# Quantco/tabmat

Measured on AMD Instinct MI355X. Metric: SplitMatrix.sandwich GFLOP/s + effective HBM GB/s, 10M×1k mixed, higher is better.
Workload: dtype f64; 1 GPU; SplitMatrix.sandwich: dense128 + csr512@5% + cats(256,96,32), 10000000 rows/GPU, p=1024, float64 (BASELINE configs[3]); rows_per_gpu=10000000, p=1024, launch=eager, collective=none

## Files before the change

include/tabmat_hip.h:

```cpp
#ifndef TABMAT_HIP_H
#define TABMAT_HIP_H

#include <stddef.h>
#include <stdint.h>

#ifdef __cplusplus
extern "C" {
#endif

#define TM_OK 0
#define TM_EINVAL (-1)
#define TM_ENOMEM (-2)
#define TM_EUNSUPPORTED (-3)

int tm_version(void);
const char *tm_last_error(void);
int tm_device_count(int *count);
int tm_set_device(int device);
int tm_device_info(char *name, int name_len, int *compute_units, int64_t *hbm_bytes);
int tm_malloc(void **ptr, size_t bytes);
int tm_free(void *ptr);
int tm_memcpy_h2d(void *dst, const void *h_src, size_t bytes, void *stream);
int tm_memcpy_d2h(void *h_dst, const void *src, size_t bytes, void *stream);
int tm_memset(void *dst, int value, size_t bytes, void *stream);
// ... 60 lines not shown

int tm_dense_sandwich_matvec_f32(const float *X, int64_t n, int64_t m, const float *u, const float *dm,
                                 const float *t_add, const float *center, const float *shift, float *g, float *w,
                                 void *stream);
int tm_dense_sandwich_matvec_f64(const double *X, int64_t n, int64_t m, const double *u, const double *dm,
                                 const double *t_add, const double *center, const double *shift, double *g,
                                 double *w, void *stream);

int tm_dense_sandwich_bf16x3_f32(const float *X, int64_t n, int64_t m, const float *d, float *out,
                                 void *stream);

int tm_dense_matvec_f32(const float *X, int64_t n, int64_t m, int order_f, const float *v,
                        const int32_t *rows, int64_t n_rows, const int32_t *cols,
                        int64_t n_cols, float *out, void *stream);
int tm_dense_matvec_f64(const double *X, int64_t n, int64_t m, int order_f, const double *v,
                        const int32_t *rows, int64_t n_rows, const int32_t *cols,
                        int64_t n_cols, double *out, void *stream);

int tm_dense_rmatvec_f32(const float *X, int64_t n, int64_t m, int order_f, const float *v,
                         const int32_t *rows, int64_t n_rows, const int32_t *cols,
                         int64_t n_cols, float *out, void *stream);
int tm_dense_rmatvec_f64(const double *X, int64_t n, int64_t m, int order_f, const double *v,
                         const int32_t *rows, int64_t n_rows, const int32_t *cols,
                         int64_t n_cols, double *out, void *stream);

int tm_dense_col_sq_dev_f32(const float *X, int64_t n, int64_t m, int order_f, const float *w,
                            const float *shift, float *out, void *stream);
int tm_dense_col_sq_dev_f64(const double *X, int64_t n, int64_t m, int order_f, const double *w,
                            const double *shift, double *out, void *stream);


int tm_sparse_sandwich_f32(const float *csr_data, const int32_t *csr_indices,
                           const int64_t *csr_indptr, int64_t n, int64_t m, const float *d,
                           const int32_t *rows, int64_t n_rows, const int32_t *cols,
                           int64_t n_cols, float *out, void *stream);
int tm_sparse_sandwich_f64(const double *csr_data, const int32_t *csr_indices,
                           const int64_t *csr_indptr, int64_t n, int64_t m, const double *d,
                           const int32_t *rows, int64_t n_rows, const int32_t *cols,
                           int64_t n_cols, double *out, void *stream);

int tm_sparse_chunk_cols(void);
int tm_sparse_sandwich_chunked_f32(const float *cm_data, const int32_t *cm_indices,
                                   const int32_t *cptr, int64_t n, int64_t m, int64_t nnz,
                                   const float *d, float *out, void *stream);
int tm_sparse_sandwich_chunked_f64(const double *cm_data, const int32_t *cm_indices,
                                   const int32_t *cptr, int64_t n, int64_t m, int64_t nnz,
                                   const double *d, double *out, void *stream);

int tm_sparse_sandwich_pairs_f32(const int32_t *cm_rec, const int32_t *cptr, int64_t n, int64_t m, int64_t nnz,
                                 const float *d, float *out, void *stream);
int tm_sparse_sandwich_pairs_f64(const int32_t *cm_rec, const int32_t *cptr, int64_t n, int64_t m, int64_t nnz,
                                 const double *d, double *out, void *stream);

int tm_sparse_sandwich_pairs_pk_f32(const int32_t *cm_rec_pk, const int32_t *cptr, int64_t n, int64_t m, int64_t nnz,
                                    const float *d, float *out, void *stream);
int tm_sparse_sandwich_pairs_pk_f64(const int32_t *cm_rec_pk, const int32_t *cptr, int64_t n, int64_t m, int64_t nnz,
                                    const double *d, double *out, void *stream);

int tm_sparse_sandwich_blocks_f32(const float *cm_data, const int32_t *cm_indices, const int32_t *cptr,
                                  int64_t n, int64_t m, int64_t nnz, const int32_t *blocks,
                                  const int32_t *wg_tab, int n_wg, int max_nb, const float *d, float *out,
                                  void *stream);
int tm_sparse_sandwich_blocks_f64(const double *cm_data, const int32_t *cm_indices, const int32_t *cptr,
                                  int64_t n, int64_t m, int64_t nnz, const int32_t *blocks,
                                  const int32_t *wg_tab, int n_wg, int max_nb, const double *d, double *out,
                                  void *stream);

int tm_sparse_sandwich_blocks_u8_f32(const float *cm_data, const uint8_t *cm_col8, const int32_t *cptr,
                                     int64_t n, int64_t m, int64_t nnz, const int32_t *blocks,
                                     const int32_t *wg_tab, int n_wg, int max_nb, const float *d, float *out,
                                     void *stream);
int tm_sparse_sandwich_blocks_u8_f64(const double *cm_data, const uint8_t *cm_col8, const int32_t *cptr,
                                     int64_t n, int64_t m, int64_t nnz, const int32_t *blocks,
                                     const int32_t *wg_tab, int n_wg, int max_nb, const double *d, double *out,
                                     void *stream);
int tm_sparse_sandwich_blocks_p12_f32(const float *cm_data, const uint8_t *cm_col8, const int32_t *cptr,
                                      int64_t n, int64_t m, int64_t nnz, const int32_t *blocks12,
                                      const int32_t *wg_tab, int n_wg, int max_nb, const float *d, float *out,
                                      void *stream);
int tm_sparse_sandwich_blocks_p12_f64(const double *cm_data, const uint8_t *cm_col8, const int32_t *cptr,
                                      int64_t n, int64_t m, int64_t nnz, const int32_t *blocks12,
                                      const int32_t *wg_tab, int n_wg, int max_nb, const double *d, double *out,
                                      void *stream);

int tm_csr_dense_sandwich_f32(const float *csr_data, const int32_t *csr_indices,
                              const int64_t *csr_indptr, int64_t n, int64_t m, const float *B,
                              int64_t r, int order_f, const float *d, const int32_t *rows,
                              int64_t n_rows, const int32_t *A_cols, int64_t nA,
                              const int32_t *B_cols, int64_t nB, float *out, void *stream);
int tm_csr_dense_sandwich_f64(const double *csr_data, const int32_t *csr_indices,
                              const int64_t *csr_indptr, int64_t n, int64_t m, const double *B,
                              int64_t r, int order_f, const double *d, const int32_t *rows,
                              int64_t n_rows, const int32_t *A_cols, int64_t nA,
                              const int32_t *B_cols, int64_t nB, double *out, void *stream);

int tm_slab_rows(void);
int tm_slab_group_cols(void);
int tm_csr_dense_sandwich_slab_f32(const float *vals, const uint32_t *koff, const uint16_t *cnt,
                                   const int64_t *gptr, int64_t n, int64_t m, const float *B,
                                   int64_t r, int order_f, const float *d, float *out, void *stream);
int tm_csr_dense_sandwich_slab_f64(const double *vals, const uint32_t *koff, const uint16_t *cnt,
                                   const int64_t *gptr, int64_t n, int64_t m, const double *B,
                                   int64_t r, int order_f, const double *d, double *out, void *stream);

int tm_csr_dense_sandwich_ell_f32(const float *vals, const uint32_t *koff, const int64_t *gptr,
                                  int64_t n, int64_t m, const float *B, int64_t r, const float *d,
                                  float *out, void *stream);
int tm_csr_dense_sandwich_ell_f64(const double *vals, const uint32_t *koff, const int64_t *gptr,
                                  int64_t n, int64_t m, const double *B, int64_t r, const double *d,
                                  double *out, void *stream);

int tm_ellw_rows(void);
int tm_ellw_group_cols(void);
int tm_csr_dense_sandwich_ellw_f32(const float *vals, const uint32_t *koff, const int64_t *gptr,
                                   int64_t n, int64_t m, const float *B, int64_t r, const float *d,
                                   float *out, void *stream);
int tm_csr_dense_sandwich_ellw_f64(const double *vals, const uint32_t *koff, const int64_t *gptr,
                                   int64_t n, int64_t m, const double *B, int64_t r, const double *d,
                                   double *out, void *stream);

int tm_lg_rows(void);
int tm_lg_group_cols(void);
int tm_lg_row_bytes(int elem_size);
int tm_csr_dense_sandwich_lg_f32(const float *vals, const uint32_t *koff, const int64_t *xptr,
                                 const float *xvals, const uint32_t *xkoff, int64_t n, int64_t m,
                                 const float *B, int64_t r, const float *d, int unconditional,
                                 float *out, void *stream);
int tm_csr_dense_sandwich_lg_f64(const double *vals, const uint32_t *koff, const int64_t *xptr,
                                 const double *xvals, const uint32_t *xkoff, int64_t n, int64_t m,
                                 const double *B, int64_t r, const double *d, int unconditional,
                                 double *out, void *stream);

int tm_csr_dense_sandwich_lg_xtd_f32(const float *vals, const uint32_t *koff, const int64_t *xptr,
                                     const float *xvals, const uint32_t *xkoff, int64_t n, int64_t m,
                                     const float *B, int64_t r, const float *d, int unconditional,
                                     float *out, float *colsum, void *stream);
int tm_csr_dense_sandwich_lg_xtd_f64(const double *vals, const uint32_t *koff, const int64_t *xptr,
                                     const double *xvals, const uint32_t *xkoff, int64_t n, int64_t m,
                                     const double *B, int64_t r, const double *d, int unconditional,
                                     double *out, double *colsum, void *stream);

int tm_csr_dense_sandwich_lgc_f32(const float *cvals, const uint32_t *cmap, const int64_t *crec,
                                  const uint32_t *xkoff, int64_t n, int64_t m, const float *B, int64_t r,
                                  const float *d, int unconditional, float *out, float *colsum, void *stream);
int tm_csr_dense_sandwich_lgc_f64(const double *cvals, const uint32_t *cmap, const int64_t *crec,
                                  const uint32_t *xkoff, int64_t n, int64_t m, const double *B, int64_t r,
                                  const double *d, int unconditional, double *out, double *colsum,
                                  void *stream);

int tm_ent_rows(void);
int tm_ent_group_cols(void);
int tm_ent_batch_slots(void);
int tm_csr_dense_sandwich_ent_f32(const float *vals, const uint16_t *meta, const uint32_t *bstart, int64_t n,
                                  int64_t m, const float *B, int64_t r, const float *d, float *out,
                                  float *colsum, void *stream);
int tm_csr_dense_sandwich_ent_f64(const double *vals, const uint16_t *meta, const uint32_t *bstart, int64_t n,
                                  int64_t m, const double *B, int64_t r, const double *d, double *out,
                                  double *colsum, void *stream);


int tm_index_narrow_i64(const int64_t *src, int64_t count, int64_t limit, int32_t *dst, int32_t *bad, void *stream);
int tm_index_widen_i32(const int32_t *src, int64_t count, int64_t *dst, void *stream);

int tm_csr_matvec_f32(const float *csr_data, const int32_t *csr_indices,
                      const int64_t *csr_indptr, int64_t n, int64_t m, const float *v,
                      const int32_t *rows, int64_t n_rows, const int32_t *cols, int64_t n_cols,
                      float *out, void *stream);
int tm_csr_matvec_f64(const double *csr_data, const int32_t *csr_indices,
                      const int64_t *csr_indptr, int64_t n, int64_t m, const double *v,
                      const int32_t *rows, int64_t n_rows, const int32_t *cols, int64_t n_cols,
                      double *out, void *stream);

int tm_csr_matvec_u16_f32(const float *csr_data, const uint16_t *csr_indices16, const int64_t *csr_indptr,
                          int64_t n, int64_t m, const float *v, float *out, void *stream);
int tm_csr_matvec_u16_f64(const double *csr_data, const uint16_t *csr_indices16, const int64_t *csr_indptr,
                          int64_t n, int64_t m, const double *v, double *out, void *stream);

int tm_csr_rmatvec_u16_f32(const float *csr_data, const uint16_t *csr_indices16, const int64_t *csr_indptr,
                           int64_t n, int64_t m, const float *v, float *out, void *stream);
int tm_csr_rmatvec_u16_f64(const double *csr_data, const uint16_t *csr_indices16, const int64_t *csr_indptr,
                           int64_t n, int64_t m, const double *v, double *out, void *stream);

int tm_csr_rmatvec_f32(const float *csr_data, const int32_t *csr_indices,
                       const int64_t *csr_indptr, int64_t n, int64_t m, const float *v,
                       const int32_t *rows, int64_t n_rows, const int32_t *cols, int64_t n_cols,
                       float *out, void *stream);
int tm_csr_rmatvec_f64(const double *csr_data, const int32_t *csr_indices,
                       const int64_t *csr_indptr, int64_t n, int64_t m, const double *v,
                       const int32_t *rows, int64_t n_rows, const int32_t *cols, int64_t n_cols,
                       double *out, void *stream);

int tm_csr_col_sq_f32(const float *csr_data, const int32_t *csr_indices, const int64_t *csr_indptr,
                      int64_t n, int64_t m, const float *w, float *out, void *stream);
int tm_csr_col_sq_f64(const double *csr_data, const int32_t *csr_indices,
                      const int64_t *csr_indptr, int64_t n, int64_t m, const double *w,
                      double *out, void *stream);

int tm_index_check_i64(void *stream, int32_t *h_bad);
int tm_sparse_sandwich_i64_f32(const float *csr_data, const int64_t *csr_indices, const int64_t *csr_indptr,
                               int64_t n, int64_t m, int64_t nnz, const float *d, const int32_t *rows,
                               int64_t n_rows, const int32_t *cols, int64_t n_cols, float *out, void *stream);
int tm_sparse_sandwich_i64_f64(const double *csr_data, const int64_t *csr_indices, const int64_t *csr_indptr,
                               int64_t n, int64_t m, int64_t nnz, const double *d, const int32_t *rows,
                               int64_t n_rows, const int32_t *cols, int64_t n_cols, double *out, void *stream);
int tm_csr_dense_sandwich_i64_f32(const float *csr_data, const int64_t *csr_indices, const int64_t *csr_indptr,
                                  int64_t n, int64_t m, int64_t nnz, const float *B, int64_t r, int order_f,
                                  const float *d, const int32_t *rows, int64_t n_rows, const int32_t *A_cols,
                                  int64_t nA, const int32_t *B_cols, int64_t nB, float *out, void *stream);
int tm_csr_dense_sandwich_i64_f64(const double *csr_data, const int64_t *csr_indices, const int64_t *csr_indptr,
                                  int64_t n, int64_t m, int64_t nnz, const double *B, int64_t r, int order_f,
                                  const double *d, const int32_t *rows, int64_t n_rows, const int32_t *A_cols,
                                  int64_t nA, const int32_t *B_cols, int64_t nB, double *out, void *stream);
int tm_csr_matvec_i64_f32(const float *csr_data, const int64_t *csr_indices, const int64_t *csr_indptr, int64_t n,
                          int64_t m, int64_t nnz, const float *v, const int32_t *rows, int64_t n_rows,
                          const int32_t *cols, int64_t n_cols, float *out, void *stream);
int tm_csr_matvec_i64_f64(const double *csr_data, const int64_t *csr_indices, const int64_t *csr_indptr, int64_t n,
                          int64_t m, int64_t nnz, const double *v, const int32_t *rows, int64_t n_rows,
                          const int32_t *cols, int64_t n_cols, double *out, void *stream);
int tm_csr_rmatvec_i64_f32(const float *csr_data, const int64_t *csr_indices, const int64_t *csr_indptr, int64_t n,
                           int64_t m, int64_t nnz, const float *v, const int32_t *rows, int64_t n_rows,
                           const int32_t *cols, int64_t n_cols, float *out, void *stream);
int tm_csr_rmatvec_i64_f64(const double *csr_data, const int64_t *csr_indices, const int64_t *csr_indptr, int64_t n,
                           int64_t m, int64_t nnz, const double *v, const int32_t *rows, int64_t n_rows,
                           const int32_t *cols, int64_t n_cols, double *out, void *stream);
int tm_csr_col_sq_i64_f32(const float *csr_data, const int64_t *csr_indices, const int64_t *csr_indptr, int64_t n,
                          int64_t m, int64_t nnz, const float *w, float *out, void *stream);
int tm_csr_col_sq_i64_f64(const double *csr_data, const int64_t *csr_indices, const int64_t *csr_indptr, int64_t n,
                          int64_t m, int64_t nnz, const double *w, double *out, void *stream);


int tm_cat_transpose_matvec_f32(const int32_t *codes, int64_t n, int64_t n_cols, int drop_first,
                                const float *v, const int32_t *rows, int64_t n_rows,
                                const int32_t *cols, int64_t n_cols_sel, float *out,
                                void *stream);
int tm_cat_transpose_matvec_f64(const int32_t *codes, int64_t n, int64_t n_cols, int drop_first,
                                const double *v, const int32_t *rows, int64_t n_rows,
                                const int32_t *cols, int64_t n_cols_sel, double *out,
                                void *stream);

int tm_cat_matvec_f32(const int32_t *codes, int64_t n, int64_t n_cols, int drop_first,
                      const float *v, const int32_t *cols, int64_t n_cols_sel, float *out,
                      void *stream);
int tm_cat_matvec_f64(const int32_t *codes, int64_t n, int64_t n_cols, int drop_first,
                      const double *v, const int32_t *cols, int64_t n_cols_sel, double *out,
                      void *stream);

int tm_cat_matvec_assign_f32(const int32_t *codes, int64_t n, int64_t n_cols, int drop_first,
                             const float *v, const int32_t *cols, int64_t n_cols_sel, float *out,
                             void *stream);
int tm_cat_matvec_assign_f64(const int32_t *codes, int64_t n, int64_t n_cols, int drop_first,
                             const double *v, const int32_t *cols, int64_t n_cols_sel, double *out,
                             void *stream);

int tm_cat_cat_sandwich_f32(const int32_t *i_codes, const int32_t *j_codes, int64_t n,
                            const float *d, const int32_t *rows, int64_t n_rows, int64_t i_ncol,
                            int64_t j_ncol, int i_drop_first, int j_drop_first, float *out,
                            void *stream);
int tm_cat_cat_sandwich_f64(const int32_t *i_codes, const int32_t *j_codes, int64_t n,
                            const double *d, const int32_t *rows, int64_t n_rows, int64_t i_ncol,
                            int64_t j_ncol, int i_drop_first, int j_drop_first, double *out,
                            void *stream);

int tm_cat_cat_sandwich_atomic_f32(const int32_t *i_codes, const int32_t *j_codes, int64_t n,
                                   const float *d, const int32_t *rows, int64_t n_rows, int64_t i_ncol,
                                   int64_t j_ncol, int i_drop_first, int j_drop_first, float *out,
                                   void *stream);
int tm_cat_cat_sandwich_atomic_f64(const int32_t *i_codes, const int32_t *j_codes, int64_t n,
                                   const double *d, const int32_t *rows, int64_t n_rows, int64_t i_ncol,
                                   int64_t j_ncol, int i_drop_first, int j_drop_first, double *out,
                                   void *stream);

int tm_cat_cat_sandwich_sorted_f32(const int32_t *ci_sorted, const int32_t *cj_sorted, const int32_t *perm,
                                   const int64_t *lptr, int64_t n_sorted, const float *d, int64_t i_ncol,
                                   int64_t j_ncol, float *out, void *stream);
int tm_cat_cat_sandwich_sorted_f64(const int32_t *ci_sorted, const int32_t *cj_sorted, const int32_t *perm,
                                   const int64_t *lptr, int64_t n_sorted, const double *d, int64_t i_ncol,
                                   int64_t j_ncol, double *out, void *stream);

int tm_cat_dense_sandwich_f32(const int32_t *codes, int64_t n, int64_t i_ncol, int drop_first,
                              const float *d, const int32_t *rows, int64_t n_rows, const float *M,
                              int64_t M_ncol, int order_f, const int32_t *j_cols, int64_t n_j,
                              float *out, void *stream);
int tm_cat_dense_sandwich_f64(const int32_t *codes, int64_t n, int64_t i_ncol, int drop_first,
                              const double *d, const int32_t *rows, int64_t n_rows,
                              const double *M, int64_t M_ncol, int order_f, const int32_t *j_cols,
                              int64_t n_j, double *out, void *stream);

int tm_cat_sparse_sandwich_f32(const int32_t *codes, int64_t n, int64_t i_ncol, int drop_first,
                               const float *csr_data, const int32_t *csr_indices,
                               const int64_t *csr_indptr, int64_t s_ncol, const float *d,
                               const int32_t *rows, int64_t n_rows, const int32_t *cols,
                               int64_t n_cols, float *out, void *stream);
int tm_cat_sparse_sandwich_f64(const int32_t *codes, int64_t n, int64_t i_ncol, int drop_first,
                               const double *csr_data, const int32_t *csr_indices,
                               const int64_t *csr_indptr, int64_t s_ncol, const double *d,
                               const int32_t *rows, int64_t n_rows, const int32_t *cols,
                               int64_t n_cols, double *out, void *stream);

int tm_multi_cat_dense_sandwich_f32(const void *const *h_codes, const int64_t *h_ncols,
                                    const int32_t *h_drop_first, int n_cats, int64_t n,
                                    const float *d, const float *M, int64_t M_ncol, int order_f,
                                    float *out, void *stream);
int tm_multi_cat_dense_sandwich_f64(const void *const *h_codes, const int64_t *h_ncols,
                                    const int32_t *h_drop_first, int n_cats, int64_t n,
                                    const double *d, const double *M, int64_t M_ncol, int order_f,
                                    double *out, void *stream);
int tm_multi_cat_dense_sandwich_rows_f32(const void *const *h_codes, const int64_t *h_ncols,
                                         const int32_t *h_drop_first, int n_cats, int64_t n,
                                         const float *d, const float *M, int64_t M_ncol,
                                         const int32_t *rows, int64_t n_rows, float *out,
                                         void *stream);
int tm_multi_cat_dense_sandwich_rows_f64(const void *const *h_codes, const int64_t *h_ncols,
                                         const int32_t *h_drop_first, int n_cats, int64_t n,
                                         const double *d, const double *M, int64_t M_ncol,
                                         const int32_t *rows, int64_t n_rows, double *out,
                                         void *stream);
int tm_multi_cat_sparse_sandwich_rows_f32(const void *const *h_codes, const int64_t *h_ncols,
                                          const int32_t *h_drop_first, int n_cats,
                                          const float *cm_data, const int32_t *cm_indices,
                                          const int32_t *row_ranges, const int32_t *rows,
                                          int64_t n_sel, int64_t m, const float *d_sel, float *out,
                                          void *stream);
int tm_multi_cat_sparse_sandwich_rows_f64(const void *const *h_codes, const int64_t *h_ncols,
                                          const int32_t *h_drop_first, int n_cats,
                                          const double *cm_data, const int32_t *cm_indices,
                                          const int32_t *row_ranges, const int32_t *rows,
                                          int64_t n_sel, int64_t m, const double *d_sel, double *out,
                                          void *stream);
int tm_multi_cat_sparse_sandwich_rows_u8_f32(const void *const *h_codes, const int64_t *h_ncols,
                                             const int32_t *h_drop_first, int n_cats,
                                             const float *cm_data, const uint8_t *cm_col8,
                                             const int32_t *row_ranges, const int32_t *rows,
                                             int64_t n_sel, int64_t m, const float *d_sel, float *out,
                                             void *stream);
int tm_multi_cat_sparse_sandwich_rows_u8_f64(const void *const *h_codes, const int64_t *h_ncols,
                                             const int32_t *h_drop_first, int n_cats,
                                             const double *cm_data, const uint8_t *cm_col8,
                                             const int32_t *row_ranges, const int32_t *rows,
                                             int64_t n_sel, int64_t m, const double *d_sel, double *out,
                                             void *stream);
int tm_multi_cat_sparse_sandwich_ent_f32(const void *const *h_codes, const int64_t *h_ncols,
                                         const int32_t *h_drop_first, int n_cats, int64_t n, const float *d,
                                         const float *vals, const uint16_t *meta, const uint32_t *bstart,
                                         int64_t n_slots, int64_t mk, float *out, void *stream);
int tm_multi_cat_sparse_sandwich_ent_f64(const void *const *h_codes, const int64_t *h_ncols,
                                         const int32_t *h_drop_first, int n_cats, int64_t n, const double *d,
                                         const double *vals, const uint16_t *meta, const uint32_t *bstart,
                                         int64_t n_slots, int64_t mk, double *out, void *stream);
int tm_multi_cat_pack_codes(const void *const *h_codes, const int64_t *h_ncols, const int32_t *h_drop_first, int n_cats,
                            int64_t n, uint32_t *packed, void *stream);
int tm_multi_cat_sparse_sandwich_entp_f32(const void *const *h_codes, const int64_t *h_ncols,
                                          const int32_t *h_drop_first, int n_cats, int64_t n, const float *d,
                                          const float *vals, const uint16_t *meta, const uint32_t *bstart,
                                          int64_t n_slots, int64_t mk, const uint32_t *packed, float *out, void *stream);
int tm_multi_cat_sparse_sandwich_entp_f64(const void *const *h_codes, const int64_t *h_ncols,
                                          const int32_t *h_drop_first, int n_cats, int64_t n, const double *d,
                                          const double *vals, const uint16_t *meta, const uint32_t *bstart,
                                          int64_t n_slots, int64_t mk, const uint32_t *packed, double *out, void *stream);

int tm_multi_cat_sparse_sandwich_slab_f32(const void *const *h_codes, const int64_t *h_ncols,
                                          const int32_t *h_drop_first, int n_cats, int64_t n,
                                          const float *d, const float *vals, const uint32_t *koff,
                                          const uint8_t *ecol, const int64_t *gptr, int64_t m,
                                          float *out, void *stream);
int tm_multi_cat_sparse_sandwich_slab_f64(const void *const *h_codes, const int64_t *h_ncols,
                                          const int32_t *h_drop_first, int n_cats, int64_t n,
                                          const double *d, const double *vals, const uint32_t *koff,
                                          const uint8_t *ecol, const int64_t *gptr, int64_t m,
                                          double *out, void *stream);

int tm_multi_cat_pairs_max_bins(void);
int tm_multi_cat_pairs_max_slots(void);
int tm_multi_cat_pairs_row_words(void);
int tm_multi_cat_pairs_f32(const int64_t *cat_tab, int64_t n, const float *d, const int32_t *rows,
                           int64_t n_rows, const int32_t *bundles, int n_bundles,
                           const int32_t *wg_map, int n_wg, int slots, int64_t bins,
                           const int64_t *desc, int64_t n_pairs, const int64_t *pos, double *tables,
                           double *out, int64_t p, void *stream);
int tm_multi_cat_pairs_f64(const int64_t *cat_tab, int64_t n, const double *d, const int32_t *rows,
                           int64_t n_rows, const int32_t *bundles, int n_bundles,
                           const int32_t *wg_map, int n_wg, int slots, int64_t bins,
                           const int64_t *desc, int64_t n_pairs, const int64_t *pos, double *tables,
                           double *out, int64_t p, void *stream);

int tm_multi_cat_matvec_f32(const int64_t *cat_tab, int n_cats, const int64_t *pos, const float *v,
                            int64_t n, float *out, void *stream);
int tm_multi_cat_matvec_f64(const int64_t *cat_tab, int n_cats, const int64_t *pos, const double *v,
                            int64_t n, double *out, void *stream);

int tm_csr_densify_cols_f32(const float *data, const int32_t *indices, const int64_t *indptr, int64_t n,
                            const int32_t *colmap, float *T, int64_t ld, void *stream);
int tm_csr_densify_cols_f64(const double *data, const int32_t *indices, const int64_t *indptr, int64_t n,
                            const int32_t *colmap, double *T, int64_t ld, void *stream);
int tm_csc_densify_cols_f32(const int32_t *rows, const float *vals, const int64_t *seg, const int32_t *tcol,
                            int64_t n_sel, int64_t max_len, float *T, int64_t ld, void *stream);
int tm_csc_densify_cols_f64(const int32_t *rows, const double *vals, const int64_t *seg, const int32_t *tcol,
                            int64_t n_sel, int64_t max_len, double *T, int64_t ld, void *stream);
int tm_dense_gather_cols_f32(const float *X, int64_t n, int64_t m, int order_f, const int32_t *cols,
                             int64_t n_sel, float *T, int64_t ld, int64_t t0, void *stream);
int tm_dense_gather_cols_f64(const double *X, int64_t n, int64_t m, int order_f, const int32_t *cols,
                             int64_t n_sel, double *T, int64_t ld, int64_t t0, void *stream);

int tm_scatter_block_f32(const float *src, int64_t nr, int64_t nc, const int64_t *ri,
                         const int64_t *ci, double *out, int64_t p, int mirror, int diag,
                         void *stream);
int tm_scatter_block_f64(const double *src, int64_t nr, int64_t nc, const int64_t *ri,
                         const int64_t *ci, double *out, int64_t p, int mirror, int diag,
                         void *stream);

int tm_sparse_sandwich_chunked_rows_f32(const float *cm_data, const int32_t *cm_indices,
                                        const int32_t *row_ranges, int64_t n_sel, int64_t m,
                                        int64_t nnz, const float *d_sel, float *out, void *stream);
int tm_sparse_sandwich_chunked_rows_f64(const double *cm_data, const int32_t *cm_indices,
                                        const int32_t *row_ranges, int64_t n_sel, int64_t m,
                                        int64_t nnz, const double *d_sel, double *out, void *stream);

int tm_sparse_sandwich_chunked_u8_f32(const float *cm_data, const uint8_t *cm_col8, const int32_t *cptr, int64_t n,
                                      int64_t m, int64_t nnz, const float *d, float *out, void *stream);
int tm_sparse_sandwich_chunked_u8_f64(const double *cm_data, const uint8_t *cm_col8, const int32_t *cptr, int64_t n,
                                      int64_t m, int64_t nnz, const double *d, double *out, void *stream);
int tm_sparse_sandwich_chunked_rows_u8_f32(const float *cm_data, const uint8_t *cm_col8, const int32_t *row_ranges,
                                           int64_t n_sel, int64_t m, int64_t nnz, const float *d_sel, float *out,
                                           void *stream);
int tm_sparse_sandwich_chunked_rows_u8_f64(const double *cm_data, const uint8_t *cm_col8, const int32_t *row_ranges,
                                           int64_t n_sel, int64_t m, int64_t nnz, const double *d_sel, double *out,
                                           void *stream);
int tm_sparse_sandwich_direct_f32(const float *csr_data, const int32_t *csr_indices,
                                  const int64_t *csr_indptr, int64_t n, int64_t m, const float *d,
                                  float *out, void *stream);
int tm_sparse_sandwich_direct_f64(const double *csr_data, const int32_t *csr_indices,
                                  const int64_t *csr_indptr, int64_t n, int64_t m, const double *d,
                                  double *out, void *stream);
int tm_csr_dense_sandwich_rows_f32(const float *cm_data, const int32_t *cm_indices,
                                   const int32_t *row_ranges, int64_t n_sel, const int32_t *rows,
                                   const float *d_sel, int64_t n, int64_t m, const float *B, int64_t r,
                                   int order_f, float *out, void *stream);
int tm_csr_dense_sandwich_rows_f64(const double *cm_data, const int32_t *cm_indices,
                                   const int32_t *row_ranges, int64_t n_sel, const int32_t *rows,
                                   const double *d_sel, int64_t n, int64_t m, const double *B, int64_t r,
                                   int order_f, double *out, void *stream);
int tm_csr_dense_sandwich_rows_u8_f32(const float *cm_data, const uint8_t *cm_col8,
// ... 82 lines not shown
```

tabmat_amd/csrc/cat.hip:

```cpp
#include <algorithm>

#include "common.hpp"
#include "reduce.hpp"

namespace tmh {

__global__ void fill_i32_kernel(int32_t *p, int64_t n, int32_t v) {
    int64_t i = (int64_t)blockIdx.x * blockDim.x + threadIdx.x;
    if (i < n) p[i] = v;
}

__global__ void scatter_iota_i32_kernel(int32_t *map, const int32_t *cols, int64_t n_cols) {
    int64_t i = (int64_t)blockIdx.x * blockDim.x + threadIdx.x;
    if (i < n_cols) map[cols[i]] = (int32_t)i;
}

int build_col_map(int32_t *map, int64_t m, const int32_t *cols, int64_t n_cols, hipStream_t st) {
    if (m > 0) {
        hipLaunchKernelGGL(fill_i32_kernel, dim3((unsigned)ceil_div(m, 256)), dim3(256), 0, st, map,
                           m, -1);
        TM_LAUNCH_CHECK();
    }
    if (n_cols > 0) {
        hipLaunchKernelGGL(scatter_iota_i32_kernel, dim3((unsigned)ceil_div(n_cols, 256)),
// ... 710 lines not shown
                sc[c * MCW_RS + lr] = R.dk != F(0) ? R.code[c] : -1;
        }
        __builtin_amdgcn_wave_barrier();
#pragma unroll
        for (int i = 0; i < NI; ++i) {
            const int row = 4 * i + q;
            const F dk = sd[row];
            int off[NC];
#pragma unroll
            for (int c = 0; c < NC; ++c) off[c] = sc[c * MCW_RS + row];
            vec_t x = R.x[i];
#pragma unroll
            for (int v = 0; v < VEC; ++v) x[v] *= dk;
#pragma unroll
            for (int c = 0; c < NC; ++c) {
                if (jok && off[c] >= 0) {
                    lds_acc_t *dst = reinterpret_cast<lds_acc_t *>(smem_raw + off[c]) + jl;
#pragma unroll
                    for (int v = 0; v < VEC; ++v) atomic_add(dst + 16 * v, (lds_acc_t)x[v]);
                }
            }
        }
    };
    Regs ra, rb;
    int64_t k0 = t0 + (int64_t)wave * MCW_RS;
    if (k0 < t1) load(k0, ra);
    for (; k0 < t1; k0 += 2 * step) {
        const bool more = k0 + step < t1;
        if (more) load(k0 + step, rb);
        process(ra);
        if (more) {
            if (k0 + 2 * step < t1) load(k0 + 2 * step, ra);
            process(rb);
        }
    }
    __syncthreads();
    if (threadIdx.x == 0) wg_log_end(wglog, t_begin, WG_CAT_DENSE);
    F *dst = ws + ((int64_t)blockIdx.y * gridDim.x + blockIdx.x) * stride;
    for (int b = threadIdx.x; b < nel; b += blockDim.x) {
        const int c = b % TJ;
        dst[b] = (F)tile[(b / TJ) * TJ + (c / VEC) + 16 * (c % VEC)];
    }
}

template <typename F, int TJ>
__global__ __launch_bounds__(1024) void multi_cat_dense_f_kernel(
    CatSet cs, const F *__restrict__ d, const F *__restrict__ M, int64_t n, int64_t m,
    int64_t rows_per_block, F *__restrict__ ws, int64_t stride) {
    extern __shared__ __attribute__((aligned(16))) unsigned char smem_raw[];
    lds_acc_t *tile = reinterpret_cast<lds_acc_t *>(smem_raw);
    const int nel = cs.total * TJ;
    for (int b = threadIdx.x; b < nel; b += blockDim.x) tile[b] = 0.0;
    __syncthreads();
    const int64_t j0 = (int64_t)blockIdx.y * TJ;
    const int64_t t0 = (int64_t)blockIdx.x * rows_per_block;
    const int64_t t1 = min(t0 + rows_per_block, n);
    for (int64_t k = t0 + threadIdx.x; k < t1; k += blockDim.x) {
        const F dk = d[k];
        int col[MAX_CATS];
#pragma unroll
        for (int c = 0; c < MAX_CATS; ++c)
            col[c] = c < cs.n_cats ? cs.codes[c][k] - cs.drop[c] : -1;
        for (int jl = 0; jl < TJ && j0 + jl < m; ++jl) {
            const F x = dk * M[(j0 + jl) * n + k];
#pragma unroll
            for (int c = 0; c < MAX_CATS; ++c)
                if (col[c] >= 0) atomic_add(&tile[(cs.off[c] + col[c]) * TJ + jl], (lds_acc_t)x);
        }
    }
    __syncthreads();
    F *dst = ws + ((int64_t)blockIdx.y * gridDim.x + blockIdx.x) * stride;
    for (int b = threadIdx.x; b < nel; b += blockDim.x) dst[b] = (F)tile[b];
}

template <typename F>
__global__ void multi_cat_untile_kernel(const F *__restrict__ tmp, int64_t total, int64_t m,
                                        int TJ, F *__restrict__ out) {
    const int64_t e = (int64_t)blockIdx.x * blockDim.x + threadIdx.x;
    if (e >= total * m) return;
    const int64_t a = e / m, j = e % m;
    out[e] = tmp[((j / TJ) * total + a) * TJ + (j % TJ)];
}

template <typename F, bool STAGE>
__global__ __launch_bounds__(1024) void multi_cat_sparse_kernel(
    CatSet cs, const F *__restrict__ d, const F *__restrict__ vals,
    const unsigned *__restrict__ koff, const unsigned char *__restrict__ ecol,
    const int64_t *__restrict__ gptr, int n_groups, int64_t n_slabs, int64_t slabs_per_block,
    int slab_rows, int group_cols, int64_t n, F *__restrict__ ws, int64_t stride) {
    extern __shared__ __attribute__((aligned(16))) unsigned char smem_raw[];
    lds_acc_t *tile = reinterpret_cast<lds_acc_t *>(smem_raw);
    const int tstr = group_cols + 1;
    const int nel = cs.total * tstr;
    for (int b = threadIdx.x; b < nel; b += blockDim.x) tile[b] = 0.0;
    const int g = blockIdx.y;
    const int lane = threadIdx.x & 63;
    const int wave = threadIdx.x >> 6, nwave = blockDim.x >> 6;
    F *sd = reinterpret_cast<F *>(smem_raw + (((size_t)nel * sizeof(lds_acc_t) + 15) / 16) * 16) +
            (size_t)wave * slab_rows;
    int32_t *sc = reinterpret_cast<int32_t *>(
                      reinterpret_cast<F *>(smem_raw + (((size_t)nel * sizeof(lds_acc_t) + 15) / 16) * 16) +
                      (size_t)nwave * slab_rows) +
                  (size_t)wave * cs.n_cats * slab_rows;
    __syncthreads();
    const int64_t s0 = (int64_t)blockIdx.x * slabs_per_block;
    const int64_t s1 = min(s0 + slabs_per_block, n_slabs);
    const unsigned rowb = 64u * (unsigned)sizeof(F);
    int64_t nb = 0, ne = 0;
    if (s0 + wave < s1) {
        nb = gptr[(s0 + wave) * n_groups + g];
        ne = gptr[(s0 + wave) * n_groups + g + 1];
    }
    for (int64_t s = s0 + wave; s < s1; s += nwave) {
        const int64_t base = nb, end = ne;
        if (s + nwave < s1) {
            nb = gptr[(s + nwave) * n_groups + g];
            ne = gptr[(s + nwave) * n_groups + g + 1];
        }
        if (STAGE) {
            __builtin_amdgcn_wave_barrier();
            for (int r = lane; r < slab_rows; r += 64) {
                const int64_t k = min(s * slab_rows + r, n - 1);
                sd[r] = d[k];
                for (int c = 0; c < cs.n_cats; ++c) sc[c * slab_rows + r] = cs.codes[c][k] - cs.drop[c];
            }
            __builtin_amdgcn_wave_barrier();
        }
        for (int64_t e0 = base + lane; e0 < end; e0 += 128) {
            const int64_t e1 = e0 + 64;
            const bool ok1 = e1 < end;
            const unsigned ko0 = koff[e0];
            const unsigned ko1 = ok1 ? koff[e1] : 0u;
            const F v0 = vals[e0];
            const F v1 = ok1 ? vals[e1] : F(0);
            const int ec0 = ecol[e0];
            const int ec1 = ok1 ? ecol[e1] : 0;
            const int r0 = (int)(ko0 / rowb), r1 = (int)(ko1 / rowb);
            const int64_t k0 = s * slab_rows + r0;
            const int64_t k1 = s * slab_rows + r1;
            const F d0 = STAGE ? sd[r0] : d[k0];
            const F d1 = ok1 ? (STAGE ? sd[r1] : d[k1]) : F(0);
            const F x0 = d0 != F(0) ? d0 * v0 : F(0);
            const F x1 = d1 != F(0) ? d1 * v1 : F(0);
#pragma unroll 1
            for (int c = 0; c < cs.n_cats; ++c) {
                const int c0 = STAGE ? sc[c * slab_rows + r0] : cs.codes[c][k0] - cs.drop[c];
                const int c1 = ok1 ? (STAGE ? sc[c * slab_rows + r1] : cs.codes[c][k1] - cs.drop[c])
                                   : -1;
                if (c0 >= 0) atomic_add(&tile[(cs.off[c] + c0) * tstr + ec0], (lds_acc_t)x0);
                if (c1 >= 0) atomic_add(&tile[(cs.off[c] + c1) * tstr + ec1], (lds_acc_t)x1);
            }
        }
    }
    __syncthreads();
    F *dst = ws + ((int64_t)blockIdx.y * gridDim.x + blockIdx.x) * stride;
    for (int b = threadIdx.x; b < cs.total * group_cols; b += blockDim.x)
        dst[b] = (F)tile[(b / group_cols) * tstr + (b % group_cols)];
}

template <typename F, int NC>
__global__ __launch_bounds__(1024) void multi_cat_sparse_pf_kernel(
    CatSet cs, const F *__restrict__ d, const F *__restrict__ vals,
    const unsigned *__restrict__ koff, const unsigned char *__restrict__ ecol,
    const int64_t *__restrict__ gptr, int n_groups, int64_t n_slabs, int64_t slabs_per_block,
    int group_cols, int64_t n, F *__restrict__ ws, int64_t stride, WgLogBuf *__restrict__ wglog) {
    const unsigned long long t_begin = wg_log_begin(wglog);
// ... 322 lines not shown
            }
        }
    }
    __syncthreads();
    F *dst = ws + ((int64_t)blockIdx.y * gridDim.x + blockIdx.x) * stride;
    for (int b = threadIdx.x; b < cs.total * GC; b += blockDim.x)
        dst[b] = (F)tile[(b / GC) * TSTR + (b % GC)];
}

template <typename F, typename IX>
__global__ __launch_bounds__(1024) void multi_cat_sparse_rows_kernel(
    CatSet cs, const F *__restrict__ cm_data, const IX *__restrict__ cm_ind,
    const int32_t *__restrict__ ranges, const int32_t *__restrict__ rows, const F *__restrict__ d_sel,
    int64_t n_sel, int64_t rows_per_block, F *__restrict__ ws, int64_t stride) {
    constexpr int GC = 32;
    extern __shared__ __attribute__((aligned(16))) unsigned char smem_raw[];
    lds_acc_t *tile = reinterpret_cast<lds_acc_t *>(smem_raw);
    constexpr int tstr = GC + 1;
    const int nel = cs.total * tstr;
    for (int b = threadIdx.x; b < nel; b += blockDim.x) tile[b] = 0.0;
    __syncthreads();
    const int g = blockIdx.y;
    const int ch = g >> 2;
    const int lane = threadIdx.x & 63, wave = threadIdx.x >> 6, nwave = blockDim.x >> 6;
    const int lr = lane >> 3, lt = lane & 7;
    const int64_t t0 = (int64_t)blockIdx.x * rows_per_block;
    const int64_t t1 = min(t0 + rows_per_block, n_sel);
    const int32_t *rg = ranges + (int64_t)ch * n_sel * 2;
    for (int64_t k0 = t0 + wave * 8; k0 < t1; k0 += (int64_t)nwave * 8) {
        const int64_t k = k0 + lr;
        if (k >= t1) continue;
        const F dk = d_sel[k];
        if (dk == F(0)) continue;
        const int e0 = rg[2 * k], e1 = rg[2 * k + 1];
        if (e0 >= e1) continue;
        const int64_t row = rows[k];
        int off[MAX_CATS];
#pragma unroll
        for (int c = 0; c < MAX_CATS; ++c) {
            off[c] = -1;
            if (c < cs.n_cats) {
                const int col = cs.codes[c][row] - cs.drop[c];
                off[c] = col >= 0 ? (cs.off[c] + col) * tstr : -1;
            }
        }
        for (int e = e0 + lt; e < e1; e += 8) {
            const int col = (int)cm_ind[e] - (sizeof(IX) == 1 ? (g & 3) : g) * GC;
            if (col < 0 || col >= GC) continue;
            const lds_acc_t x = (lds_acc_t)(dk * cm_data[e]);
#pragma unroll
            for (int c = 0; c < MAX_CATS; ++c)
                if (off[c] >= 0) atomic_add(&tile[off[c] + col], x);
        }
    }
    __syncthreads();
    F *dst = ws + ((int64_t)blockIdx.y * gridDim.x + blockIdx.x) * stride;
    for (int b = threadIdx.x; b < cs.total * GC; b += blockDim.x)
        dst[b] = (F)tile[(b / GC) * tstr + (b % GC)];
}

static int make_catset(const void *const *h_codes, const int64_t *h_ncols, const int32_t *h_drop,
                       int n_cats, CatSet *cs) {
    if (n_cats < 1 || n_cats > MAX_CATS) {
        set_error("multi-cat call supports 1..%d categoricals, got %d", MAX_CATS, n_cats);
        return TM_EINVAL;
    }
    int off = 0;
    for (int c = 0; c < MAX_CATS; ++c) {
        cs->codes[c] = c < n_cats ? reinterpret_cast<const int32_t *>(h_codes[c]) : nullptr;
        cs->ncol[c] = c < n_cats ? (int)h_ncols[c] : 0;
        cs->drop[c] = c < n_cats ? h_drop[c] : 0;
        cs->off[c] = off;
        off += cs->ncol[c];
    }
    cs->n_cats = n_cats;
    cs->total = off;
    return TM_OK;
}

template <typename F>
static int run_multi_cat_dense(const void *const *h_codes, const int64_t *h_ncols,
                               const int32_t *h_drop, int n_cats, int64_t n, const F *d, const F *M,
                               int64_t m, int order_f, F *out, hipStream_t st,
                               const int32_t *rows = nullptr, int64_t n_rows = 0) {
    CatSet cs;
    int rc = make_catset(h_codes, h_ncols, h_drop, n_cats, &cs);
    if (rc) return rc;
    const int64_t total = (int64_t)cs.total * m;
    if (total == 0) return TM_OK;
    if (rows != nullptr) n = n_rows;
    if (n == 0) {
        TM_HIP(hipMemsetAsync(out, 0, sizeof(F) * (size_t)total, st));
        return TM_OK;
    }
    {
        constexpr int VEC = MCW_VEC;
        constexpr int TJW = 16 * VEC;
        const size_t tile_b = ((sizeof(lds_acc_t) * (size_t)cs.total * TJW + 15) / 16) * 16;
        const size_t lds_w = tile_b + (size_t)16 * MCW_RS * (sizeof(F) + (size_t)n_cats * sizeof(int));
        if (!order_f && n_cats <= 8 && m >= VEC && m % VEC == 0 &&
            (reinterpret_cast<uintptr_t>(M) & 15) == 0 && lds_w <= 150 * 1024 &&
            (int64_t)cs.total * TJW * (int64_t)sizeof(lds_acc_t) < (1ll << 30)) {
            const int64_t n_parts = ceil_div(m, TJW);
            const int64_t stride = (int64_t)cs.total * TJW;
            int64_t nblk = std::max<int64_t>(1, tune("catdense_rounds", 1) * NUM_CU / n_parts);
            nblk = std::min<int64_t>(nblk, std::max<int64_t>(1, ceil_div(n, 4096)));
            const int64_t rpb = ceil_div(ceil_div(n, nblk), MCW_RS) * MCW_RS;
            nblk = ceil_div(n, rpb);
            const size_t tmp_bytes = ((sizeof(F) * (size_t)(n_parts * stride) + 255) / 256) * 256;
            void *wsv = nullptr;
            rc = get_workspace(tmp_bytes + sizeof(F) * (size_t)(n_parts * nblk * stride) + 256, &wsv, st);
            if (rc) return rc;
            F *tmp = reinterpret_cast<F *>(wsv);
            F *ws = reinterpret_cast<F *>(reinterpret_cast<char *>(wsv) + tmp_bytes);
            auto gow = [&](auto kern) -> int {
                TM_HIP(hipFuncSetAttribute(reinterpret_cast<const void *>(kern),
                                           hipFuncAttributeMaxDynamicSharedMemorySize, (int)lds_w));
                prof_begin(st);
                const int nw_dflt = (sizeof(F) == 8 && tile_b > 64 * 1024) ? 8 : 16;
                const int nw = (int)std::min<int64_t>(16, std::max<int64_t>(4, tune("catdense_waves", nw_dflt)));
                hipLaunchKernelGGL(kern, dim3((unsigned)nblk, (unsigned)n_parts), dim3(nw * 64), lds_w, st,
                                   cs, d, M, n, m, rpb, ws, stride, rows, wg_log_ptr());
                prof_end(st);
                TM_LAUNCH_CHECK();
                return TM_OK;
            };
            if (n_cats == 1) rc = gow(&multi_cat_dense_wide_kernel<F, 1>);
            else if (n_cats == 2) rc = gow(&multi_cat_dense_wide_kernel<F, 2>);
            else if (n_cats == 3) rc = gow(&multi_cat_dense_wide_kernel<F, 3>);
            else if (n_cats == 4) rc = gow(&multi_cat_dense_wide_kernel<F, 4>);
            else if (n_cats == 5) rc = gow(&multi_cat_dense_wide_kernel<F, 5>);
            else if (n_cats == 6) rc = gow(&multi_cat_dense_wide_kernel<F, 6>);
            else if (n_cats == 7) rc = gow(&multi_cat_dense_wide_kernel<F, 7>);
            else rc = gow(&multi_cat_dense_wide_kernel<F, 8>);
            if (rc) return rc;
            rc = launch_reduce_partials<F>(ws, stride, (int)nblk, (int)n_parts, tmp, n_parts * stride,
                                           false, st);
            if (rc) return rc;
            hipLaunchKernelGGL((multi_cat_untile_kernel<F>), dim3((unsigned)ceil_div(total, 256)),
                               dim3(256), 0, st, tmp, (int64_t)cs.total, m, TJW, out);
            TM_LAUNCH_CHECK();
            return TM_OK;
        }
    }
    if (rows != nullptr) {
        set_error("multi_cat_dense: the row-list form needs the wide-load path");
        return TM_EUNSUPPORTED;
    }
    int TJ = 64;
    while (TJ > 1 && sizeof(lds_acc_t) * (size_t)cs.total * TJ > HIST_LDS_MAX) TJ >>= 1;
    while (TJ > 1 && TJ / 2 >= m) TJ >>= 1;
    if (sizeof(lds_acc_t) * (size_t)cs.total * TJ > HIST_LDS_MAX) {
        set_error("multi_cat_dense: %d stacked categories exceed the LDS tile", cs.total);
        return TM_EUNSUPPORTED;
    }
    const int64_t n_parts = ceil_div(m, TJ);
    const int64_t stride = (int64_t)cs.total * TJ;
    const size_t lds = sizeof(lds_acc_t) * (size_t)stride;
    int64_t nblk = std::max<int64_t>(1, NUM_CU / n_parts);
    nblk = std::min<int64_t>(nblk, std::max<int64_t>(1, ceil_div(n, 4096)));
    const int64_t rpb = ceil_div(n, nblk);
    nblk = ceil_div(n, rpb);
    const size_t tmp_bytes = ((sizeof(F) * (size_t)(n_parts * stride) + 255) / 256) * 256;
    void *wsv = nullptr;
    rc = get_workspace(tmp_bytes + sizeof(F) * (size_t)(n_parts * nblk * stride) + 256, &wsv, st);
    if (rc) return rc;
    F *tmp = reinterpret_cast<F *>(wsv);
    F *ws = reinterpret_cast<F *>(reinterpret_cast<char *>(wsv) + tmp_bytes);
    auto go = [&](auto kern) -> int {
        if (lds > 48 * 1024)
            TM_HIP(hipFuncSetAttribute(reinterpret_cast<const void *>(kern),
                                       hipFuncAttributeMaxDynamicSharedMemorySize, (int)lds));
        prof_begin(st);
        hipLaunchKernelGGL(kern, dim3((unsigned)nblk, (unsigned)n_parts), dim3(1024), lds, st, cs, d,
                           M, n, m, rpb, ws, stride);
        prof_end(st);
        TM_LAUNCH_CHECK();
        return TM_OK;
    };
#define TM_MCD_CASE(V)                                                                       \
    case V:                                                                                  \
        if (order_f) rc = go(&multi_cat_dense_f_kernel<F, V>);                               \
        else if (n_cats == 1) rc = go(&multi_cat_dense_c_kernel<F, V, 1>);                   \
        else if (n_cats == 2) rc = go(&multi_cat_dense_c_kernel<F, V, 2>);                   \
        else if (n_cats == 3) rc = go(&multi_cat_dense_c_kernel<F, V, 3>);                   \
        else if (n_cats == 4) rc = go(&multi_cat_dense_c_kernel<F, V, 4>);                   \
        else rc = go(&multi_cat_dense_c_kernel<F, V, 0>);                                    \
        break;
    switch (TJ) {
        TM_MCD_CASE(64)
        TM_MCD_CASE(32)
        TM_MCD_CASE(16)
        TM_MCD_CASE(8)
        TM_MCD_CASE(4)
        TM_MCD_CASE(2)
        TM_MCD_CASE(1)
        default:
            rc = TM_EINVAL;
    }
#undef TM_MCD_CASE
    if (rc) return rc;
    rc = launch_reduce_partials<F>(ws, stride, (int)nblk, (int)n_parts, tmp, n_parts * stride, false,
                                   st);
    if (rc) return rc;
    hipLaunchKernelGGL((multi_cat_untile_kernel<F>), dim3((unsigned)ceil_div(total, 256)),
                       dim3(256), 0, st, tmp, (int64_t)cs.total, m, TJ, out);
    TM_LAUNCH_CHECK();
    return TM_OK;
}

template <typename F, typename IX>
static int run_multi_cat_sparse_rows(const void *const *h_codes, const int64_t *h_ncols,
                                     const int32_t *h_drop, int n_cats, const F *cm_data,
                                     const IX *cm_ind, const int32_t *ranges, const int32_t *rows,
                                     int64_t n_sel, int64_t m, const F *d_sel, F *out, hipStream_t st);

template <typename F>
static int run_multi_cat_sparse(const void *const *h_codes, const int64_t *h_ncols,
                                const int32_t *h_drop, int n_cats, int64_t n, const F *d,
                                const F *vals, const unsigned *koff, const unsigned char *ecol,
                                const int64_t *gptr, int64_t m, int slab_rows, int group_cols,
                                F *out, hipStream_t st) {
    CatSet cs;
    int rc = make_catset(h_codes, h_ncols, h_drop, n_cats, &cs);
    if (rc) return rc;
    const int64_t total = (int64_t)cs.total * m;
// ... 4 lines not shown
    }
    const int64_t stride = (int64_t)cs.total * group_cols;
    const size_t tile_bytes = ((sizeof(lds_acc_t) * (size_t)cs.total * (group_cols + 1) + 15) / 16) * 16;
    if (tile_bytes > HIST_LDS_MAX) {
        set_error("multi_cat_sparse: %d stacked categories exceed the LDS tile", cs.total);
        return TM_EUNSUPPORTED;
    }
    const int nw = (int)std::min<int64_t>(16, std::max<int64_t>(4, tune("catsparse_waves", 16)));
    const size_t stage_bytes = (size_t)nw * slab_rows * (sizeof(F) + sizeof(int32_t) * (size_t)n_cats);
    const bool stage = tile_bytes + stage_bytes <= 150 * 1024;
    const size_t lds = tile_bytes + (stage ? stage_bytes : 0);
    const int n_groups = (int)ceil_div(m, group_cols);
    const int64_t n_slabs = ceil_div(n, slab_rows);
    int64_t nblk = std::max<int64_t>(1, tune("catsparse_rounds", 1) * NUM_CU / n_groups);
    nblk = std::min<int64_t>(nblk, n_slabs);
    const int64_t spb = ceil_div(n_slabs, nblk);
    nblk = ceil_div(n_slabs, spb);
    const size_t tmp_bytes = ((sizeof(F) * (size_t)(n_groups * stride) + 255) / 256) * 256;
    void *wsv = nullptr;
    rc = get_workspace(tmp_bytes + sizeof(F) * (size_t)((int64_t)n_groups * nblk * stride) + 256,
                       &wsv, st);
    if (rc) return rc;
    F *tmp = reinterpret_cast<F *>(wsv);
    F *ws = reinterpret_cast<F *>(reinterpret_cast<char *>(wsv) + tmp_bytes);
    if (stage && n_cats <= 8 && slab_rows == 128) {
        auto kpf = n_cats == 1   ? &multi_cat_sparse_pf_kernel<F, 1>
                   : n_cats == 2 ? &multi_cat_sparse_pf_kernel<F, 2>
                   : n_cats == 3 ? &multi_cat_sparse_pf_kernel<F, 3>
                   : n_cats == 4 ? &multi_cat_sparse_pf_kernel<F, 4>
                   : n_cats == 5 ? &multi_cat_sparse_pf_kernel<F, 5>
                   : n_cats == 6 ? &multi_cat_sparse_pf_kernel<F, 6>
                   : n_cats == 7 ? &multi_cat_sparse_pf_kernel<F, 7>
                                 : &multi_cat_sparse_pf_kernel<F, 8>;
        if (lds > 48 * 1024)
            TM_HIP(hipFuncSetAttribute(reinterpret_cast<const void *>(kpf),
                                       hipFuncAttributeMaxDynamicSharedMemorySize, (int)lds));
        prof_begin(st);
        hipLaunchKernelGGL(kpf, dim3((unsigned)nblk, (unsigned)n_groups), dim3(nw * 64), lds, st, cs, d,
                           vals, koff, ecol, gptr, n_groups, n_slabs, spb, group_cols, n, ws, stride,
                           wg_log_ptr());
        prof_end(st);
        TM_LAUNCH_CHECK();
    } else {
        auto kern = stage ? &multi_cat_sparse_kernel<F, true> : &multi_cat_sparse_kernel<F, false>;
        if (lds > 48 * 1024)
            TM_HIP(hipFuncSetAttribute(reinterpret_cast<const void *>(kern),
                                       hipFuncAttributeMaxDynamicSharedMemorySize, (int)lds));
        prof_begin(st);
        hipLaunchKernelGGL(kern, dim3((unsigned)nblk, (unsigned)n_groups), dim3(nw * 64), lds, st, cs,
                           d, vals, koff, ecol, gptr, n_groups, n_slabs, spb, slab_rows, group_cols,
                           n, ws, stride);
        prof_end(st);
        TM_LAUNCH_CHECK();
    }
    rc = launch_reduce_partials<F>(ws, stride, (int)nblk, n_groups, tmp,
                                   (int64_t)n_groups * stride, false, st);
    if (rc) return rc;
    hipLaunchKernelGGL((multi_cat_untile_kernel<F>), dim3((unsigned)ceil_div(total, 256)),
                       dim3(256), 0, st, tmp, (int64_t)cs.total, m, group_cols, out);
    TM_LAUNCH_CHECK();
    return TM_OK;
}

__global__ __launch_bounds__(256) void multi_cat_pack_codes_kernel(CatSet cs, int64_t n, unsigned *__restrict__ out) {
    for (int64_t r = (int64_t)blockIdx.x * blockDim.x + threadIdx.x; r < n; r += (int64_t)gridDim.x * blockDim.x) {
        unsigned pk = 0u;
#pragma unroll
        for (int c = 0; c < 3; ++c) {
            unsigned f = 1023u;
            if (c < cs.n_cats) {
                const int col = cs.codes[c][r] - cs.drop[c];
                if (col >= 0 && col < cs.ncol[c]) f = (unsigned)(cs.off[c] + col);
            }
            pk |= f << (10 * c);
        }
        out[r] = pk;
    }
}

template <typename F>
static int run_multi_cat_sparse_ent(const void *const *h_codes, const int64_t *h_ncols, const int32_t *h_drop,
                                    int n_cats, int64_t n, const F *d, const F *vals, const unsigned short *meta,
                                    const unsigned *bstart, int64_t mk, F *out, hipStream_t st,
                                    const unsigned *packed = nullptr, int64_t n_slots = 0) {
    CatSet cs;
    int rc = make_catset(h_codes, h_ncols, h_drop, n_cats, &cs);
    if (rc) return rc;
    const int64_t total = (int64_t)cs.total * mk;
    if (total == 0) return TM_OK;
    if (n == 0) {
        TM_HIP(hipMemsetAsync(out, 0, sizeof(F) * (size_t)total, st));
        return TM_OK;
    }
    TM_REQUIRE(mk % 16 == 0 && n_cats >= 1 && n_cats <= 8, "kernel columns in groups of 16, 1 .. 8 categoricals");
    TM_REQUIRE(n < (1ll << 28), "at most 2^28 - 1 rows per block");
    constexpr int GC = 32;
    const int64_t stride = (int64_t)cs.total * GC;
    const size_t lds = ((sizeof(lds_acc_t) * (size_t)cs.total * (GC + 1) + 15) / 16) * 16;
    if (lds > HIST_LDS_MAX) {
        set_error("multi_cat_sparse_ent: %d stacked categories exceed the LDS tile", cs.total);
        return TM_EUNSUPPORTED;
    }
    const int nw = (int)std::min<int64_t>(16, std::max<int64_t>(4, tune("catsparse_waves", 16)));
    const int n_groups = (int)(mk / 16);
    const int n_pairs = (n_groups + 1) / 2;
    const int64_t n_slabs = ceil_div(n, 64);
    int64_t nblk = std::max<int64_t>(1, tune("catsparse_rounds", 1) * NUM_CU / n_pairs);
    nblk = std::min<int64_t>(nblk, n_slabs);
    const int64_t spb = ceil_div(n_slabs, nblk);
    nblk = ceil_div(n_slabs, spb);
    const size_t tmp_bytes = ((sizeof(F) * (size_t)(n_pairs * stride) + 255) / 256) * 256;
    void *wsv = nullptr;
    rc = get_workspace(tmp_bytes + sizeof(F) * (size_t)((int64_t)n_pairs * nblk * stride) + 256, &wsv, st);
    if (rc) return rc;
    F *tmp = reinterpret_cast<F *>(wsv);
    F *ws = reinterpret_cast<F *>(reinterpret_cast<char *>(wsv) + tmp_bytes);
    auto kern = n_cats == 1   ? &multi_cat_sparse_ent_kernel<F, 1>
                : n_cats == 2 ? &multi_cat_sparse_ent_kernel<F, 2>
                : n_cats == 3 ? &multi_cat_sparse_ent_kernel<F, 3>
                : n_cats == 4 ? &multi_cat_sparse_ent_kernel<F, 4>
                : n_cats == 5 ? &multi_cat_sparse_ent_kernel<F, 5>
                : n_cats == 6 ? &multi_cat_sparse_ent_kernel<F, 6>
                : n_cats == 7 ? &multi_cat_sparse_ent_kernel<F, 7>
                              : &multi_cat_sparse_ent_kernel<F, 8>;
    TM_REQUIRE(packed == nullptr || (n_cats <= 3 && cs.total < 1023), "packed codes: at most 3 categoricals, 1022 levels");
    const int ncw = packed != nullptr ? 1 : n_cats;
    const size_t lds_staged = lds + (size_t)nw * 64 * (sizeof(F) + 4 * (size_t)ncw);
    const double fill = (double)n_slots / ((double)std::max(n_groups, 1) * (double)n_slabs);
    if (tune("catsparse_staged", 1) != 0 && lds_staged <= 156 * 1024 &&
        fill >= (double)tune("catsparse_staged_fill", 44)) {
        using KS = void (*)(CatSet, const F *, const F *, const unsigned short *, const unsigned *, int, int64_t, int64_t,
                            int64_t, F *, int64_t, const unsigned *, int);
        KS ks = nullptr;
        if (packed != nullptr) {
            ks = n_cats == 1 ? &multi_cat_sparse_ent_staged_kernel<F, 1, true>
                 : n_cats == 2 ? &multi_cat_sparse_ent_staged_kernel<F, 2, true>
                               : &multi_cat_sparse_ent_staged_kernel<F, 3, true>;
        } else {
            ks = n_cats == 1   ? &multi_cat_sparse_ent_staged_kernel<F, 1, false>
                 : n_cats == 2 ? &multi_cat_sparse_ent_staged_kernel<F, 2, false>
                 : n_cats == 3 ? &multi_cat_sparse_ent_staged_kernel<F, 3, false>
                 : n_cats == 4 ? &multi_cat_sparse_ent_staged_kernel<F, 4, false>
                 : n_cats == 5 ? &multi_cat_sparse_ent_staged_kernel<F, 5, false>
                 : n_cats == 6 ? &multi_cat_sparse_ent_staged_kernel<F, 6, false>
                 : n_cats == 7 ? &multi_cat_sparse_ent_staged_kernel<F, 7, false>
                               : &multi_cat_sparse_ent_staged_kernel<F, 8, false>;
        }
        if (lds_staged > 48 * 1024)
            TM_HIP(hipFuncSetAttribute(reinterpret_cast<const void *>(ks),
                                       hipFuncAttributeMaxDynamicSharedMemorySize, (int)lds_staged));
        prof_begin(st);
        hipLaunchKernelGGL(ks, dim3((unsigned)nblk, (unsigned)n_pairs), dim3(nw * 64), lds_staged, st, cs, d, vals,
                           meta, bstart, n_groups, n, n_slabs, spb, ws, stride, packed, (int)lds);
        prof_end(st);
        TM_LAUNCH_CHECK();
    } else {
        if (lds > 48 * 1024)
            TM_HIP(hipFuncSetAttribute(reinterpret_cast<const void *>(kern),
                                       hipFuncAttributeMaxDynamicSharedMemorySize, (int)lds));
        prof_begin(st);
        hipLaunchKernelGGL(kern, dim3((unsigned)nblk, (unsigned)n_pairs), dim3(nw * 64), lds, st, cs, d, vals, meta,
                           bstart, n_groups, n, n_slabs, spb, ws, stride, packed);
        prof_end(st);
        TM_LAUNCH_CHECK();
    }
    rc = launch_reduce_partials<F>(ws, stride, (int)nblk, n_pairs, tmp, (int64_t)n_pairs * stride, false, st);
    if (rc) return rc;
    hipLaunchKernelGGL((multi_cat_untile_kernel<F>), dim3((unsigned)ceil_div(total, 256)), dim3(256), 0, st, tmp,
                       (int64_t)cs.total, mk, GC, out);
    TM_LAUNCH_CHECK();
    return TM_OK;
}

}

using namespace tmh;

#define TM_CHECK_COMMON(nn) \
    TM_REQUIRE((nn) >= 0, "negative size")

extern "C" {

int tm_cat_transpose_matvec_f32(const int32_t *codes, int64_t n, int64_t n_cols, int drop_first,
                                const float *v, const int32_t *rows, int64_t n_rows,
                                const int32_t *cols, int64_t n_cols_sel, float *out, void *stream) {
    TM_CHECK_COMMON(n);
    return run_cat_tmv<float>(codes, n, n_cols, drop_first, v, rows, n_rows, cols, n_cols_sel, out,
                              as_stream(stream));
}
int tm_cat_transpose_matvec_f64(const int32_t *codes, int64_t n, int64_t n_cols, int drop_first,
                                const double *v, const int32_t *rows, int64_t n_rows,
                                const int32_t *cols, int64_t n_cols_sel, double *out,
                                void *stream) {
    TM_CHECK_COMMON(n);
    return run_cat_tmv<double>(codes, n, n_cols, drop_first, v, rows, n_rows, cols, n_cols_sel,
                               out, as_stream(stream));
}

int tm_cat_matvec_f32(const int32_t *codes, int64_t n, int64_t n_cols, int drop_first,
                      const float *v, const int32_t *cols, int64_t n_cols_sel, float *out,
                      void *stream) {
    TM_CHECK_COMMON(n);
    return run_cat_matvec<float>(codes, n, n_cols, drop_first, v, cols, n_cols_sel, out,
                                 as_stream(stream));
}
int tm_cat_matvec_f64(const int32_t *codes, int64_t n, int64_t n_cols, int drop_first,
                      const double *v, const int32_t *cols, int64_t n_cols_sel, double *out,
                      void *stream) {
    TM_CHECK_COMMON(n);
    return run_cat_matvec<double>(codes, n, n_cols, drop_first, v, cols, n_cols_sel, out,
                                  as_stream(stream));
}

int tm_cat_matvec_assign_f32(const int32_t *codes, int64_t n, int64_t n_cols, int drop_first,
                             const float *v, const int32_t *cols, int64_t n_cols_sel, float *out,
                             void *stream) {
    TM_CHECK_COMMON(n);
    return run_cat_matvec<float>(codes, n, n_cols, drop_first, v, cols, n_cols_sel, out,
                                 as_stream(stream), true);
}
int tm_cat_matvec_assign_f64(const int32_t *codes, int64_t n, int64_t n_cols, int drop_first,
                             const double *v, const int32_t *cols, int64_t n_cols_sel, double *out,
                             void *stream) {
    TM_CHECK_COMMON(n);
    return run_cat_matvec<double>(codes, n, n_cols, drop_first, v, cols, n_cols_sel, out,
                                  as_stream(stream), true);
}

int tm_cat_cat_sandwich_f32(const int32_t *i_codes, const int32_t *j_codes, int64_t n,
                            const float *d, const int32_t *rows, int64_t n_rows, int64_t i_ncol,
                            int64_t j_ncol, int i_drop_first, int j_drop_first, float *out,
                            void *stream) {
    TM_CHECK_COMMON(n);
    return run_hist<float, true>(i_codes, j_codes, d, rows, rows ? n_rows : n, i_drop_first,
                                 j_drop_first, i_ncol, j_ncol, nullptr, out, false,
                                 as_stream(stream));
}
int tm_cat_cat_sandwich_f64(const int32_t *i_codes, const int32_t *j_codes, int64_t n,
                            const double *d, const int32_t *rows, int64_t n_rows, int64_t i_ncol,
                            int64_t j_ncol, int i_drop_first, int j_drop_first, double *out,
                            void *stream) {
    TM_CHECK_COMMON(n);
    return run_hist<double, true>(i_codes, j_codes, d, rows, rows ? n_rows : n, i_drop_first,
                                  j_drop_first, i_ncol, j_ncol, nullptr, out, false,
                                  as_stream(stream));
}

int tm_cat_cat_sandwich_atomic_f32(const int32_t *i_codes, const int32_t *j_codes, int64_t n,
// ... 55 lines not shown
    TM_CHECK_COMMON(n);
    return run_cat_sparse<float>(codes, n, i_ncol, drop_first, csr_data, csr_indices, csr_indptr,
                                 s_ncol, d, rows, n_rows, cols, n_cols, out, as_stream(stream));
}
int tm_cat_sparse_sandwich_f64(const int32_t *codes, int64_t n, int64_t i_ncol, int drop_first,
                               const double *csr_data, const int32_t *csr_indices,
                               const int64_t *csr_indptr, int64_t s_ncol, const double *d,
                               const int32_t *rows, int64_t n_rows, const int32_t *cols,
                               int64_t n_cols, double *out, void *stream) {
    TM_CHECK_COMMON(n);
    return run_cat_sparse<double>(codes, n, i_ncol, drop_first, csr_data, csr_indices, csr_indptr,
                                  s_ncol, d, rows, n_rows, cols, n_cols, out, as_stream(stream));
}

int tm_multi_cat_dense_sandwich_f32(const void *const *h_codes, const int64_t *h_ncols,
                                    const int32_t *h_drop_first, int n_cats, int64_t n,
                                    const float *d, const float *M, int64_t M_ncol, int order_f,
                                    float *out, void *stream) {
    return run_multi_cat_dense<float>(h_codes, h_ncols, h_drop_first, n_cats, n, d, M, M_ncol,
                                      order_f, out, as_stream(stream));
}
int tm_multi_cat_dense_sandwich_f64(const void *const *h_codes, const int64_t *h_ncols,
                                    const int32_t *h_drop_first, int n_cats, int64_t n,
                                    const double *d, const double *M, int64_t M_ncol, int order_f,
                                    double *out, void *stream) {
    return run_multi_cat_dense<double>(h_codes, h_ncols, h_drop_first, n_cats, n, d, M, M_ncol,
                                       order_f, out, as_stream(stream));
}
int tm_multi_cat_dense_sandwich_rows_f32(const void *const *h_codes, const int64_t *h_ncols,
                                         const int32_t *h_drop_first, int n_cats, int64_t n,
                                         const float *d, const float *M, int64_t M_ncol,
                                         const int32_t *rows, int64_t n_rows, float *out,
                                         void *stream) {
    return run_multi_cat_dense<float>(h_codes, h_ncols, h_drop_first, n_cats, n, d, M, M_ncol, 0, out,
                                      as_stream(stream), rows, n_rows);
}
int tm_multi_cat_dense_sandwich_rows_f64(const void *const *h_codes, const int64_t *h_ncols,
                                         const int32_t *h_drop_first, int n_cats, int64_t n,
                                         const double *d, const double *M, int64_t M_ncol,
                                         const int32_t *rows, int64_t n_rows, double *out,
                                         void *stream) {
    return run_multi_cat_dense<double>(h_codes, h_ncols, h_drop_first, n_cats, n, d, M, M_ncol, 0, out,
                                       as_stream(stream), rows, n_rows);
}
int tm_multi_cat_sparse_sandwich_ent_f32(const void *const *h_codes, const int64_t *h_ncols,
                                         const int32_t *h_drop_first, int n_cats, int64_t n, const float *d,
                                         const float *vals, const uint16_t *meta, const uint32_t *bstart,
                                         int64_t n_slots, int64_t mk, float *out, void *stream) {
    return run_multi_cat_sparse_ent<float>(h_codes, h_ncols, h_drop_first, n_cats, n, d, vals, meta, bstart, mk,
                                           out, as_stream(stream), nullptr, n_slots);
}
int tm_multi_cat_sparse_sandwich_ent_f64(const void *const *h_codes, const int64_t *h_ncols,
                                         const int32_t *h_drop_first, int n_cats, int64_t n, const double *d,
                                         const double *vals, const uint16_t *meta, const uint32_t *bstart,
                                         int64_t n_slots, int64_t mk, double *out, void *stream) {
    return run_multi_cat_sparse_ent<double>(h_codes, h_ncols, h_drop_first, n_cats, n, d, vals, meta, bstart, mk,
                                            out, as_stream(stream), nullptr, n_slots);
}
int tm_multi_cat_pack_codes(const void *const *h_codes, const int64_t *h_ncols, const int32_t *h_drop_first, int n_cats,
                            int64_t n, uint32_t *packed, void *stream) {
    CatSet cs;
    int rc = make_catset(h_codes, h_ncols, h_drop_first, n_cats, &cs);
    if (rc) return rc;
    TM_REQUIRE(n_cats <= 3 && cs.total < 1023, "packed codes: at most 3 categoricals, 1022 stacked levels");
    if (n == 0) return TM_OK;
    hipLaunchKernelGGL(multi_cat_pack_codes_kernel, dim3((unsigned)std::min<int64_t>(4 * NUM_CU, ceil_div(n, 256))),
                       dim3(256), 0, as_stream(stream), cs, n, packed);
    TM_LAUNCH_CHECK();
    return TM_OK;
}
int tm_multi_cat_sparse_sandwich_entp_f32(const void *const *h_codes, const int64_t *h_ncols,
                                          const int32_t *h_drop_first, int n_cats, int64_t n, const float *d,
                                          const float *vals, const uint16_t *meta, const uint32_t *bstart,
                                          int64_t n_slots, int64_t mk, const uint32_t *packed, float *out, void *stream) {
    return run_multi_cat_sparse_ent<float>(h_codes, h_ncols, h_drop_first, n_cats, n, d, vals, meta, bstart, mk, out,
                                           as_stream(stream), packed, n_slots);
}
int tm_multi_cat_sparse_sandwich_entp_f64(const void *const *h_codes, const int64_t *h_ncols,
                                          const int32_t *h_drop_first, int n_cats, int64_t n, const double *d,
                                          const double *vals, const uint16_t *meta, const uint32_t *bstart,
                                          int64_t n_slots, int64_t mk, const uint32_t *packed, double *out, void *stream) {
    return run_multi_cat_sparse_ent<double>(h_codes, h_ncols, h_drop_first, n_cats, n, d, vals, meta, bstart, mk,
                                            out, as_stream(stream), packed, n_slots);
}
int tm_multi_cat_sparse_sandwich_slab_f32(const void *const *h_codes, const int64_t *h_ncols,
                                          const int32_t *h_drop_first, int n_cats, int64_t n,
                                          const float *d, const float *vals, const uint32_t *koff,
                                          const uint8_t *ecol, const int64_t *gptr, int64_t m,
                                          float *out, void *stream) {
    return run_multi_cat_sparse<float>(h_codes, h_ncols, h_drop_first, n_cats, n, d, vals, koff,
                                       ecol, gptr, m, tm_slab_rows(), tm_slab_group_cols(), out,
                                       as_stream(stream));
}
int tm_multi_cat_sparse_sandwich_slab_f64(const void *const *h_codes, const int64_t *h_ncols,
                                          const int32_t *h_drop_first, int n_cats, int64_t n,
                                          const double *d, const double *vals, const uint32_t *koff,
                                          const uint8_t *ecol, const int64_t *gptr, int64_t m,
                                          double *out, void *stream) {
    return run_multi_cat_sparse<double>(h_codes, h_ncols, h_drop_first, n_cats, n, d, vals, koff,
                                        ecol, gptr, m, tm_slab_rows(), tm_slab_group_cols(), out,
                                        as_stream(stream));
}

}

namespace tmh {
template <typename F, typename IX>
static int run_multi_cat_sparse_rows(const void *const *h_codes, const int64_t *h_ncols,
                                     const int32_t *h_drop, int n_cats, const F *cm_data,
                                     const IX *cm_ind, const int32_t *ranges, const int32_t *rows,
                                     int64_t n_sel, int64_t m, const F *d_sel, F *out, hipStream_t st) {
    CatSet cs;
    int rc = make_catset(h_codes, h_ncols, h_drop, n_cats, &cs);
    if (rc) return rc;
    const int64_t total = (int64_t)cs.total * m;
    if (total == 0) return TM_OK;
    if (n_sel == 0) {
        TM_HIP(hipMemsetAsync(out, 0, sizeof(F) * (size_t)total, st));
        return TM_OK;
    }
    constexpr int GC = 32;
    const size_t lds = ((sizeof(lds_acc_t) * (size_t)cs.total * (GC + 1) + 15) / 16) * 16;
    if (lds > HIST_LDS_MAX) {
        set_error("multi_cat_sparse_rows: %d stacked categories exceed the LDS tile", cs.total);
        return TM_EUNSUPPORTED;
    }
    const int n_groups = (int)ceil_div(m, GC);
    const int64_t stride = (int64_t)cs.total * GC;
    int64_t nblk = std::max<int64_t>(1, tune("catsparse_rounds", 1) * NUM_CU / n_groups);
    nblk = std::min<int64_t>(nblk, std::max<int64_t>(1, ceil_div(n_sel, 2048)));
    const int64_t rpb = ceil_div(n_sel, nblk);
    nblk = ceil_div(n_sel, rpb);
    const size_t tmp_bytes = ((sizeof(F) * (size_t)(n_groups * stride) + 255) / 256) * 256;
    void *wsv = nullptr;
    rc = get_workspace(tmp_bytes + sizeof(F) * (size_t)((int64_t)n_groups * nblk * stride) + 256, &wsv, st);
    if (rc) return rc;
    F *tmp = reinterpret_cast<F *>(wsv);
    F *ws = reinterpret_cast<F *>(reinterpret_cast<char *>(wsv) + tmp_bytes);
    auto kern = &multi_cat_sparse_rows_kernel<F, IX>;
    if (lds > 48 * 1024)
        TM_HIP(hipFuncSetAttribute(reinterpret_cast<const void *>(kern),
                                   hipFuncAttributeMaxDynamicSharedMemorySize, (int)lds));
    prof_begin(st);
    hipLaunchKernelGGL(kern, dim3((unsigned)nblk, (unsigned)n_groups), dim3(1024), lds, st, cs, cm_data,
                       cm_ind, ranges, rows, d_sel, n_sel, rpb, ws, stride);
    prof_end(st);
    TM_LAUNCH_CHECK();
    rc = launch_reduce_partials<F>(ws, stride, (int)nblk, n_groups, tmp, (int64_t)n_groups * stride, false, st);
    if (rc) return rc;
    hipLaunchKernelGGL((multi_cat_untile_kernel<F>), dim3((unsigned)ceil_div(total, 256)), dim3(256), 0,
                       st, tmp, (int64_t)cs.total, m, GC, out);
    TM_LAUNCH_CHECK();
    return TM_OK;
}
}

extern "C" {
int tm_multi_cat_sparse_sandwich_rows_f32(const void *const *h_codes, const int64_t *h_ncols,
                                          const int32_t *h_drop_first, int n_cats,
                                          const float *cm_data, const int32_t *cm_indices,
                                          const int32_t *row_ranges, const int32_t *rows,
                                          int64_t n_sel, int64_t m, const float *d_sel, float *out,
                                          void *stream) {
    return tmh::run_multi_cat_sparse_rows<float, int32_t>(h_codes, h_ncols, h_drop_first, n_cats, cm_data,
                                                 cm_indices, row_ranges, rows, n_sel, m, d_sel, out,
                                                 tmh::as_stream(stream));
// ... 33 lines not shown
```

tabmat_amd/csrc/reduce.hpp:

```cpp
#pragma once
#include "common.hpp"

namespace tmh {

template <typename F, bool ACCUMULATE, int NW>
__global__ __launch_bounds__(NW * 64) void reduce_partials_kernel(const F *__restrict__ ws,
                                                                  int64_t stride, int nb,
                                                                  F *__restrict__ out,
                                                                  int64_t out_elems) {
    __shared__ double red[NW][64];
    const int lane = threadIdx.x & 63;
    const int wave = threadIdx.x >> 6;
    const int64_t e = (int64_t)blockIdx.x * 64 + lane;
    const int part = blockIdx.y;
    double acc = 0.0;
    if (e < stride) {
        const F *p = ws + ((int64_t)part * nb) * stride + e;
        for (int b = wave; b < nb; b += NW) acc += (double)p[(int64_t)b * stride];
    }
    red[wave][lane] = acc;
    __syncthreads();
    if (wave == 0 && e < stride) {
        const int64_t o = (int64_t)part * stride + e;
        if (o < out_elems) {
            double s = 0.0;
#pragma unroll
            for (int w = 0; w < NW; w += 4)
                s += (red[w][lane] + red[w + 1][lane]) + (red[w + 2][lane] + red[w + 3][lane]);
            if (ACCUMULATE)
                out[o] += (F)s;
            else
                out[o] = (F)s;
        }
    }
}

template <typename F>
inline int launch_reduce_partials(const F *ws, int64_t stride, int nb, int n_parts, F *out,
                                  int64_t out_elems, bool accumulate, hipStream_t st) {
    dim3 grid((unsigned)ceil_div(stride, 64), (unsigned)n_parts);
    const bool small = (int64_t)grid.x * grid.y < 1024 && nb > 16;
    if (small) {
        if (accumulate)
            hipLaunchKernelGGL((reduce_partials_kernel<F, true, 16>), grid, dim3(1024), 0, st, ws,
                               stride, nb, out, out_elems);
        else
            hipLaunchKernelGGL((reduce_partials_kernel<F, false, 16>), grid, dim3(1024), 0, st, ws,
                               stride, nb, out, out_elems);
    } else if (accumulate) {
        hipLaunchKernelGGL((reduce_partials_kernel<F, true, 4>), grid, dim3(256), 0, st, ws, stride,
                           nb, out, out_elems);
    } else {
        hipLaunchKernelGGL((reduce_partials_kernel<F, false, 4>), grid, dim3(256), 0, st, ws, stride,
                           nb, out, out_elems);
    }
    TM_LAUNCH_CHECK();
    return TM_OK;
}

__global__ void fill_i32_kernel(int32_t *p, int64_t n, int32_t v);
__global__ void scatter_iota_i32_kernel(int32_t *map, const int32_t *cols, int64_t n_cols);

int build_col_map(int32_t *map, int64_t m, const int32_t *cols, int64_t n_cols, hipStream_t st);

}
```

tabmat_amd/csrc/sparse_blocks.hip:

```cpp
#include <algorithm>

#include "common.hpp"
#include "reduce.hpp"

namespace tmh {

constexpr int KB_WAVES = 16;
constexpr int KB_TS = 128;

template <typename F>
__global__ void blocks_assemble_kernel(const F *__restrict__ tiles, int n_out, F *__restrict__ out) {
    const int j = blockIdx.x * blockDim.x + threadIdx.x;
    const int i = blockIdx.y;
    if (i >= n_out || j >= n_out) return;
    const int hi = max(i, j), lo = min(i, j);
    const int I = hi / KB_TS, J = lo / KB_TS;
    const int part = I * (I + 1) / 2 + J;
    out[(int64_t)i * n_out + j] = tiles[(int64_t)part * KB_TS * KB_TS + (hi % KB_TS) * KB_TS + (lo % KB_TS)];
}

constexpr int KB_FLAG_REP_A = 1 << 16;
constexpr int KB_FLAG_REP_B = 1 << 17;

template <typename F, bool U8, bool D12 = false>
__global__ __launch_bounds__(KB_WAVES * 64) void sparse_sandwich_blocks_kernel(
    const F *__restrict__ data, const int32_t *__restrict__ ind, const int32_t *__restrict__ cptr,
    int64_t n, int64_t nnz1, const int32_t *__restrict__ blocks, const int4 *__restrict__ wg_tab,
    const F *__restrict__ d, int max_nb, F *__restrict__ ws, WgLogBuf *__restrict__ wglog) {
    constexpr int TS = KB_TS;
    const unsigned long long t_begin = wg_log_begin(wglog);
    extern __shared__ __attribute__((aligned(16))) unsigned char smem_raw[];
    lds_acc_t *tile = reinterpret_cast<lds_acc_t *>(smem_raw);
    const int4 w = wg_tab[2 * blockIdx.x], x = wg_tab[2 * blockIdx.x + 1];
    const int part = __builtin_amdgcn_readfirstlane(w.x), slot = __builtin_amdgcn_readfirstlane(w.y);
    const int b0 = __builtin_amdgcn_readfirstlane(w.z), b1 = __builtin_amdgcn_readfirstlane(w.w);
    const int bfull = __builtin_amdgcn_readfirstlane(x.x);
    int wfull = __builtin_amdgcn_readfirstlane(x.y);
    {
        const int nwv = (int)(blockDim.x >> 6);
        if (nwv != KB_WAVES) {
            wfull = (wfull * nwv + KB_WAVES / 2) / KB_WAVES;
            if (bfull > b0) wfull = max(wfull, 1);
            if (b1 > bfull) wfull = min(wfull, nwv - 1);
            if (bfull == b0) wfull = 0;
            if (b1 == bfull) wfull = nwv;
        }
    }
    int I = (int)((sqrtf(8.0f * (float)part + 1.0f) - 1.0f) * 0.5f);
    while ((I + 1) * (I + 2) / 2 <= part) ++I;
    while (I * (I + 1) / 2 > part) --I;
    const int J = part - I * (I + 1) / 2;
    const int i0 = I * TS, j0 = J * TS;
    for (int b = threadIdx.x; b < TS * TS; b += blockDim.x) tile[b] = 0.0;
    __syncthreads();

    const int lane = threadIdx.x & 63;
    const int wave = __builtin_amdgcn_readfirstlane(threadIdx.x >> 6);
    const int lr = lane >> 3, lt = lane & 7;
    if (b1 > b0) {
        const int row_first = __builtin_amdgcn_readfirstlane(x.z), row_last = __builtin_amdgcn_readfirstlane(x.w);
        const int32_t *cpA = cptr + (int64_t)I * (n + 1), *cpB = cptr + (int64_t)J * (n + 1);
        const int baseA = __builtin_amdgcn_readfirstlane(cpA[row_first]);
        const int baseB = __builtin_amdgcn_readfirstlane(cpB[row_first]);
        const unsigned spanA1 = (unsigned)max(__builtin_amdgcn_readfirstlane(cpA[row_last + 1]) - baseA - 1, 0);
        const unsigned spanB1 = (unsigned)max(__builtin_amdgcn_readfirstlane(cpB[row_last + 1]) - baseB - 1, 0);
        const F *dataA = data + min((int64_t)baseA, nnz1), *dataB = data + min((int64_t)baseB, nnz1);
        const int32_t *indA = ind + min((int64_t)baseA, nnz1), *indB = ind + min((int64_t)baseB, nnz1);
        const unsigned char *ind8 = reinterpret_cast<const unsigned char *>(ind);
        const unsigned char *ind8A = ind8 + min((int64_t)baseA, nnz1), *ind8B = ind8 + min((int64_t)baseB, nnz1);
        const int i0c = U8 ? 0 : i0, j0c = U8 ? 0 : j0;
        const unsigned nrow1 = (unsigned)max(n - 1, (int64_t)0);
        auto ldi = [](const int32_t *base, unsigned i) {
            return *reinterpret_cast<const int32_t *>(reinterpret_cast<const char *>(base) + (i << 2));
        };
        auto ldf = [](const F *base, unsigned i) {
            return *reinterpret_cast<const F *>(reinterpret_cast<const char *>(base) + (i * (unsigned)sizeof(F)));
        };
        constexpr int SH = 3;
        constexpr int BIGKEY = 0x7ffffff0;
        char *const tile_bytes = reinterpret_cast<char *>(tile);
        auto add_pair = [&](int kb, int la, int ba, F prod) {
            if (kb <= la)
                atomic_add(reinterpret_cast<lds_acc_t *>(tile_bytes + (unsigned)(kb ^ ba)), (lds_acc_t)prod);
        };

        auto run_list = [&](auto diag_c, auto full_c, int s0, int s1, int w0, int nw) {
            constexpr bool DIAG = decltype(diag_c)::value;
            constexpr bool FULL = decltype(full_c)::value;
            constexpr int offmask = DIAG ? 0 : 0x70000000;
            const int nseg = s1 - s0;
            if (nseg <= 0) return;
            constexpr int DW = D12 ? 3 : 4;
            const int32_t *blk = blocks + (int64_t)s0 * DW;
            struct Dsc { int4 q; bool valid; };
            struct Grp { int nA, nB, ta, tb; F d, va, vb; int ca, cb; };
            auto load_desc = [&](int g) {
                Dsc r;
                const int k = g + lr;
                r.valid = k < nseg;
                const unsigned kc = (unsigned)min(k, nseg - 1);
                if constexpr (D12) {
                    const int32_t *b = reinterpret_cast<const int32_t *>(reinterpret_cast<const char *>(blk) + kc * 12u);
// ... 18 lines not shown
                const unsigned iA = min((unsigned)(sd.q.x - baseA) + min((unsigned)e.ta, (unsigned)max(e.nA - 1, 0)), spanA1);
                const unsigned iB = min((unsigned)(sd.q.y - baseB) + min((unsigned)e.tb, (unsigned)max(e.nB - 1, 0)), spanB1);
#ifdef KB_ABL_WRAP
                const unsigned iAw = iA & (unsigned)(KB_ABL_WRAP), iBw = iB & (unsigned)(KB_ABL_WRAP);
                e.ca = ldi(indA, min(iAw, spanA1));
                e.va = ldf(dataA, min(iAw, spanA1));
                e.cb = ldi(indB, min(iBw, spanB1));
                e.vb = ldf(dataB, min(iBw, spanB1));
                return e;
#endif
                e.ca = U8 ? (int)ind8A[iA] : ldi(indA, iA);
                e.va = ldf(dataA, iA);
                e.cb = U8 ? (int)ind8B[iB] : ldi(indB, iB);
                e.vb = ldf(dataB, iB);
                return e;
            };
            auto process = [&](const Grp &cur) {
                __builtin_amdgcn_s_setprio(1);
                const int colA = cur.ta < cur.nA ? cur.ca - i0c : -1;
                const int colB = cur.tb < cur.nB ? cur.cb - j0c : -1;
                const int la = (colA < 0 ? -8 : colA << SH) | offmask;
                const int ba = (int)(((unsigned)colA << (7 + SH)) | ((colA & 15) << (3 + SH)));
                const int kb = colB < 0 ? BIGKEY : colB << SH;
                const F av = cur.va * cur.d, vb = cur.vb;
                add_pair(kb, la, ba, av * vb);
                add_pair(dpp_xor_i32<1>(kb), la, ba, av * dpp_xor<1>(vb));
                add_pair(dpp_xor_i32<2>(kb), la, ba, av * dpp_xor<2>(vb));
                add_pair(dpp_xor_i32<3>(kb), la, ba, av * dpp_xor<3>(vb));
#ifndef KB_ABL_HALFSTEPS
                if constexpr (FULL) {
                    const int kb4 = dpp_xor_i32<4>(kb);
                    const F vb4 = dpp_xor<4>(vb);
                    add_pair(kb4, la, ba, av * vb4);
                    add_pair(dpp_xor_i32<1>(kb4), la, ba, av * dpp_xor<1>(vb4));
                    add_pair(dpp_xor_i32<2>(kb4), la, ba, av * dpp_xor<2>(vb4));
                    add_pair(dpp_xor_i32<3>(kb4), la, ba, av * dpp_xor<3>(vb4));
                }
#endif
                __builtin_amdgcn_s_setprio(0);
            };
            const int gstep = nw * 8;
            const int gw = (wave - w0) * 8;
            Grp ea[2], eb[2];
            Dsc ps[2];
            ea[0] = load_entries(load_desc(gw));
            ea[1] = load_entries(load_desc(gw + gstep));
            ps[0] = load_desc(gw + 2 * gstep);
            ps[1] = load_desc(gw + 3 * gstep);
            for (int g = gw; g < nseg; g += 4 * gstep) {
                eb[0] = load_entries(ps[0]);
                eb[1] = load_entries(ps[1]);
                ps[0] = load_desc(g + 4 * gstep);
                ps[1] = load_desc(g + 5 * gstep);
                process(ea[0]);
                if (g + gstep < nseg) process(ea[1]);
                if (g + 2 * gstep >= nseg) break;
                ea[0] = load_entries(ps[0]);
                ea[1] = load_entries(ps[1]);
                ps[0] = load_desc(g + 6 * gstep);
                ps[1] = load_desc(g + 7 * gstep);
                process(eb[0]);
                if (g + 3 * gstep < nseg) process(eb[1]);
            }
        };
        auto run_tile = [&](auto diag_c) {
            if (wave < wfull) run_list(diag_c, std::true_type{}, b0, bfull, 0, wfull);
            else run_list(diag_c, std::false_type{}, bfull, b1, wfull, (int)(blockDim.x >> 6) - wfull);
        };
        if (I == J) run_tile(std::true_type{});
        else run_tile(std::false_type{});
    }
    __syncthreads();
    if (threadIdx.x == 0) wg_log_end(wglog, t_begin, WG_K2);
    F *dst = ws + ((int64_t)part * max_nb + slot) * (TS * TS);
    for (int b = threadIdx.x; b < TS * TS; b += blockDim.x) {
        const int r = b / TS, c = b % TS;
        dst[b] = (F)tile[r * TS + (c ^ ((r & 15) << 3))];
    }
}

template <typename F, bool U8 = false, bool D12 = false>
static int run_sparse_sandwich_blocks(const F *data, const int32_t *ind, const int32_t *cptr, int64_t n,
                                      int64_t m, int64_t nnz, const int32_t *blocks, const int32_t *wg_tab,
                                      int n_wg, int max_nb, const F *d, F *out, hipStream_t st) {
    if (m == 0) return TM_OK;
    if (n == 0 || nnz == 0 || n_wg == 0) {
        TM_HIP(hipMemsetAsync(out, 0, sizeof(F) * (size_t)(m * m), st));
        return TM_OK;
    }
    constexpr int TS = KB_TS;
    const int nchunk = (int)ceil_div(m, TS);
    const int n_parts = nchunk * (nchunk + 1) / 2;
    TM_REQUIRE(nnz < (1ll << 31) && n < (1ll << 29), "sparse block too large for the block-list sandwich");
    TM_REQUIRE(!D12 || n < (1ll << 24), "12-byte block descriptors hold 24 bits of row");
    TM_REQUIRE(max_nb >= 1 && n_wg >= 1, "empty workgroup table");
    const size_t lds = sizeof(lds_acc_t) * (size_t)(TS * TS);
    const size_t tmp_bytes = (sizeof(F) * (size_t)n_parts * TS * TS + 255) / 256 * 256;
    const size_t ws_bytes = sizeof(F) * (size_t)n_parts * (size_t)max_nb * TS * TS;
    void *wsv = nullptr;
    int rc = get_workspace(tmp_bytes + ws_bytes + 256, &wsv, st);
    if (rc) return rc;
    F *tmp = reinterpret_cast<F *>(wsv);
    F *ws = reinterpret_cast<F *>(reinterpret_cast<char *>(wsv) + tmp_bytes);
    TM_HIP(hipMemsetAsync(ws, 0, ws_bytes, st));
    auto kern = &sparse_sandwich_blocks_kernel<F, U8, D12>;
    TM_HIP(hipFuncSetAttribute(reinterpret_cast<const void *>(kern),
                               hipFuncAttributeMaxDynamicSharedMemorySize, (int)lds));
    prof_begin(st);
    const int kb_waves = (int)std::min<int64_t>(KB_WAVES, std::max<int64_t>(2, tune("k2b_waves", KB_WAVES)));
    hipLaunchKernelGGL(kern, dim3((unsigned)n_wg), dim3(kb_waves * 64), lds, st, data, ind, cptr, n, nnz - 1,
                       blocks, reinterpret_cast<const int4 *>(wg_tab), d,
                       max_nb, ws, wg_log_ptr());
    prof_end(st);
    TM_LAUNCH_CHECK();
    rc = launch_reduce_partials<F>(ws, (int64_t)TS * TS, max_nb, n_parts, tmp, (int64_t)n_parts * TS * TS,
                                   false, st);
    if (rc) return rc;
    hipLaunchKernelGGL((blocks_assemble_kernel<F>), dim3((unsigned)ceil_div(m, 64), (unsigned)m), dim3(64),
                       0, st, tmp, (int)m, out);
    TM_LAUNCH_CHECK();
    return TM_OK;
}

}

extern "C" {

int tm_sparse_sandwich_blocks_f32(const float *cm_data, const int32_t *cm_indices, const int32_t *cptr,
                                  int64_t n, int64_t m, int64_t nnz, const int32_t *blocks,
                                  const int32_t *wg_tab, int n_wg, int max_nb, const float *d, float *out,
                                  void *stream) {
    return tmh::run_sparse_sandwich_blocks<float>(cm_data, cm_indices, cptr, n, m, nnz, blocks, wg_tab, n_wg,
                                                  max_nb, d, out, tmh::as_stream(stream));
}
int tm_sparse_sandwich_blocks_f64(const double *cm_data, const int32_t *cm_indices, const int32_t *cptr,
                                  int64_t n, int64_t m, int64_t nnz, const int32_t *blocks,
                                  const int32_t *wg_tab, int n_wg, int max_nb, const double *d, double *out,
                                  void *stream) {
    return tmh::run_sparse_sandwich_blocks<double>(cm_data, cm_indices, cptr, n, m, nnz, blocks, wg_tab, n_wg,
                                                   max_nb, d, out, tmh::as_stream(stream));
}

int tm_sparse_sandwich_blocks_u8_f32(const float *cm_data, const uint8_t *cm_col8, const int32_t *cptr,
                                     int64_t n, int64_t m, int64_t nnz, const int32_t *blocks,
                                     const int32_t *wg_tab, int n_wg, int max_nb, const float *d, float *out,
                                     void *stream) {
    return tmh::run_sparse_sandwich_blocks<float, true>(cm_data, reinterpret_cast<const int32_t *>(cm_col8), cptr, n, m,
                                                        nnz, blocks, wg_tab, n_wg, max_nb, d, out,
                                                        tmh::as_stream(stream));
}
int tm_sparse_sandwich_blocks_u8_f64(const double *cm_data, const uint8_t *cm_col8, const int32_t *cptr,
                                     int64_t n, int64_t m, int64_t nnz, const int32_t *blocks,
                                     const int32_t *wg_tab, int n_wg, int max_nb, const double *d, double *out,
                                     void *stream) {
    return tmh::run_sparse_sandwich_blocks<double, true>(cm_data, reinterpret_cast<const int32_t *>(cm_col8), cptr, n, m,
                                                         nnz, blocks, wg_tab, n_wg, max_nb, d, out,
                                                         tmh::as_stream(stream));
}

int tm_sparse_sandwich_blocks_p12_f32(const float *cm_data, const uint8_t *cm_col8, const int32_t *cptr,
                                      int64_t n, int64_t m, int64_t nnz, const int32_t *blocks12,
                                      const int32_t *wg_tab, int n_wg, int max_nb, const float *d, float *out,
                                      void *stream) {
    return tmh::run_sparse_sandwich_blocks<float, true, true>(cm_data, reinterpret_cast<const int32_t *>(cm_col8), cptr,
                                                              n, m, nnz, blocks12, wg_tab, n_wg, max_nb, d, out,
                                                              tmh::as_stream(stream));
}
int tm_sparse_sandwich_blocks_p12_f64(const double *cm_data, const uint8_t *cm_col8, const int32_t *cptr,
                                      int64_t n, int64_t m, int64_t nnz, const int32_t *blocks12,
                                      const int32_t *wg_tab, int n_wg, int max_nb, const double *d, double *out,
                                      void *stream) {
    return tmh::run_sparse_sandwich_blocks<double, true, true>(cm_data, reinterpret_cast<const int32_t *>(cm_col8), cptr,
                                                               n, m, nnz, blocks12, wg_tab, n_wg, max_nb, d, out,
                                                               tmh::as_stream(stream));
}

}
```

tabmat_amd/csrc/sparse_ent.hip:

```cpp
#include "common.hpp"
#include "reduce.hpp"

namespace tmh {

constexpr int EN_R = 64;
constexpr int EN_C = 16;
constexpr int EN_NW = 16;
constexpr int EN_THREADS = EN_NW * 64;
constexpr int EN_W = 128;
constexpr int EN_B = 16;
constexpr int EN_SB = 64;

template <typename F>
struct EnLds {
    static constexpr int ROWB = EN_W * (int)sizeof(F);
    static constexpr int SLABB = EN_R * ROWB;
    static constexpr int SCR_OFF = ROWB + 2 * SLABB;
    static constexpr int CS_OFF = SCR_OFF + EN_NW * EN_SB * 16;
    static constexpr int TOTAL = CS_OFF + EN_NW * EN_C * (int)sizeof(double);
};

constexpr int EN_CVGPR = 24;
#define EN_LD "40"

// ... 252 lines not shown
            e = enext;
        }
        if (q != 3) enext = scratch[(q + 1) * EN_B + l16];
        EN_TICK(pt_a)
        const int slab = __builtin_amdgcn_readlane((int)e[3], 1);
        while (w < slab) end_slab();
        if (ncopied == 0 && w + 1 < ns) {
            issue_pieces((w & 1) ^ 1, 0, NV);

            ncopied = NV;
            psince += NV;
            lsince = 0;
        }
        EN_TICK(pt_p)
        F a;
        if constexpr (sizeof(F) == 8) a = __hiloint2double((int)e[1], (int)e[0]);
        else a = __uint_as_float(e[0]);
#if defined(EN_ABL_NOBATCH)
        asm volatile("" ::"v"(a), "v"(e[2]), "v"(e[3]));
#else
        const unsigned live = (unsigned)__builtin_amdgcn_ballot_w64(a != F(0)) & 0xffffu;
        const int nq = live ? ((31 - __builtin_clz(live)) >> 2) + 1 : 0;
        unsigned p0 = (unsigned)__builtin_amdgcn_readlane((int)e[3], 0);
        unsigned p1 = (unsigned)__builtin_amdgcn_readlane((int)e[3], 4);
        unsigned p2 = (unsigned)__builtin_amdgcn_readlane((int)e[3], 8);
        unsigned p3 = (unsigned)__builtin_amdgcn_readlane((int)e[3], 12);
        if (nq == 4) en_batch_asm<16, F>(p0, p1, p2, p3, a, e[2], lane_off);
        else if (nq == 3) en_batch_asm<12, F>(p0, p1, p2, p3, a, e[2], lane_off);
        else if (nq == 2) en_batch_asm<8, F>(p0, p1, p2, p3, a, e[2], lane_off);
        else if (nq == 1) en_batch_asm<4, F>(p0, p1, p2, p3, a, e[2], lane_off);
#endif
        EN_TICK(pt_x)
#if defined(EN_PROF)
        ++pt_n;
#endif
    }
    while (w < ns) end_slab();
    wait_loads(std::integral_constant<int, 0>{});
#if defined(EN_PROF)
    if (prof != nullptr && lane == 0) {
        long long *o = prof + (((int64_t)blockIdx.z * gridDim.y + blockIdx.y) * gridDim.x + blockIdx.x) * (EN_NW * 8) + wave * 8;
        o[0] = pt_a; o[1] = pt_p; o[2] = pt_x; o[3] = pt_b; o[4] = pt_bar; o[5] = pt_n; o[6] = clock64() - pt_start; o[7] = ns;
    }
#endif

    if (active) {
        F *dst = ws + (((int64_t)blockIdx.y * gridDim.x + blockIdx.x) * n_groups + group) * (EN_C * EN_W);
        static_for<EN_C>([&](auto jc) {
            constexpr int j = decltype(jc)::value;
            if constexpr (sizeof(F) == 8) {
                const u4 o = u4{en_read_acc<4 * j>(), en_read_acc<4 * j + 1>(), en_read_acc<4 * j + 2>(),
                                en_read_acc<4 * j + 3>()};
                *reinterpret_cast<u4 *>(dst + j * EN_W + 2 * lane) = o;
            } else {
                typedef unsigned u2 __attribute__((ext_vector_type(2)));
                const u2 o = u2{en_read_acc<2 * j>(), en_read_acc<2 * j + 1>()};
                *reinterpret_cast<u2 *>(dst + j * EN_W + 2 * lane) = o;
            }
        });
        if constexpr (CSUM) {
            if (blockIdx.y == 0 && lane < EN_C)
                ws_csum[(int64_t)blockIdx.x * (n_groups * EN_C) + group * EN_C + lane] = (F)cs_lds[lane];
        }
    }
}

template <typename F>
__global__ void en_untile_kernel(const F *__restrict__ tmp, int64_t m, int64_t nB, F *__restrict__ out) {
    const int64_t e = (int64_t)blockIdx.x * blockDim.x + threadIdx.x;
    if (e >= m * nB) return;
    const int64_t i = e / nB, j = e % nB;
    out[e] = tmp[((j / EN_W) * m + i) * EN_W + (j % EN_W)];
}

template <typename F>
__global__ void en_csum_kernel(const F *__restrict__ part, int nblk, int64_t m, F *__restrict__ csum) {
    const int64_t c = (int64_t)blockIdx.x * blockDim.x + threadIdx.x;
    if (c >= m) return;
    double a = 0.0;
    for (int b = 0; b < nblk; ++b) a += (double)part[(int64_t)b * m + c];
    csum[c] = (F)a;
}

template <typename F>
static int run_csr_dense_ent(const F *vals, const uint16_t *meta, const uint32_t *bstart, int64_t n, int64_t m,
                             const F *B, int64_t r, const F *d, F *out, F *colsum, hipStream_t st) {
    const int64_t nB = r;
    const int64_t total = m * nB;
    if (total == 0) return TM_OK;
    constexpr int VEC = 16 / (int)sizeof(F);
    if ((reinterpret_cast<uintptr_t>(B) & 15) != 0 || r % VEC != 0 || nB < VEC) {
        set_error("tm_csr_dense_sandwich_ent: B must be C-ordered with 16-byte aligned rows");
        return TM_EUNSUPPORTED;
    }
    if (m % EN_C != 0) {
        set_error("tm_csr_dense_sandwich_ent: m must be a multiple of tm_ent_group_cols()");
        return TM_EINVAL;
    }
    if (n >= (1ll << 28)) {
        set_error("tm_csr_dense_sandwich_ent: at most 2^28 - 1 rows per block (work in row parts)");
        return TM_EUNSUPPORTED;
    }
    const int64_t n_slabs = ceil_div(n, EN_R);
    const int n_groups = (int)(m / EN_C);
    const int n_parts = (int)ceil_div(nB, EN_W);
    const int nz = (int)ceil_div(n_groups, EN_NW);
    const bool want_csum = colsum != nullptr;
    if (n_slabs == 0) {
        TM_HIP(hipMemsetAsync(out, 0, sizeof(F) * (size_t)total, st));
        if (want_csum) TM_HIP(hipMemsetAsync(colsum, 0, sizeof(F) * (size_t)m, st));
        return TM_OK;
    }
    int64_t nblk = std::max<int64_t>(1, tune("ent_rounds", 1) * NUM_CU / ((int64_t)n_parts * nz));
    nblk = std::min<int64_t>(nblk, n_slabs);
    const int64_t spb = ceil_div(n_slabs, nblk);
    nblk = ceil_div(n_slabs, spb);
    const int64_t stride = m * EN_W;
    const size_t tmp_bytes = (sizeof(F) * (size_t)(n_parts * stride) + 255) / 256 * 256;
    const size_t part_bytes = (sizeof(F) * (size_t)((int64_t)n_parts * nblk * stride) + 255) / 256 * 256;
    const size_t csum_bytes = ((want_csum ? sizeof(F) * (size_t)(nblk * m) : 0) + 255) / 256 * 256 + 256;
    void *wsv = nullptr;
    int rc = get_workspace(tmp_bytes + part_bytes + csum_bytes + 256, &wsv, st);
    if (rc) return rc;
    F *tmp = reinterpret_cast<F *>(wsv);
    F *ws = reinterpret_cast<F *>(reinterpret_cast<char *>(wsv) + tmp_bytes);
    F *ws_csum = reinterpret_cast<F *>(reinterpret_cast<char *>(wsv) + tmp_bytes + part_bytes);
    const size_t lds = (size_t)EnLds<F>::TOTAL;
    auto kern = want_csum ? &csr_dense_ent_kernel<F, true> : &csr_dense_ent_kernel<F, false>;
    TM_HIP(hipFuncSetAttribute(reinterpret_cast<const void *>(kern),
                               hipFuncAttributeMaxDynamicSharedMemorySize, (int)lds));
    prof_begin(st);
    hipLaunchKernelGGL(kern, dim3((unsigned)nblk, (unsigned)n_parts, (unsigned)nz), dim3(EN_THREADS), lds, st,
                       vals, meta, bstart, n_groups, n_slabs, spb, B, n, r, (int)nB, d, ws, ws_csum,
                       reinterpret_cast<long long *>((uintptr_t)tune("ent_prof", 0)));
    prof_end(st);
    TM_LAUNCH_CHECK();
    rc = launch_reduce_partials<F>(ws, stride, (int)nblk, n_parts, tmp, n_parts * stride, false, st);
    if (rc) return rc;
    hipLaunchKernelGGL((en_untile_kernel<F>), dim3((unsigned)ceil_div(total, 256)), dim3(256), 0, st, tmp, m,
                       nB, out);
    TM_LAUNCH_CHECK();
    if (want_csum) {
        hipLaunchKernelGGL((en_csum_kernel<F>), dim3((unsigned)ceil_div(m, 256)), dim3(256), 0, st, ws_csum,
                           (int)nblk, m, colsum);
        TM_LAUNCH_CHECK();
    }
    return TM_OK;
}

}

extern "C" {
int tm_ent_rows(void) { return tmh::EN_R; }
int tm_ent_group_cols(void) { return tmh::EN_C; }
int tm_ent_batch_slots(void) { return tmh::EN_B; }

int tm_csr_dense_sandwich_ent_f32(const float *vals, const uint16_t *meta, const uint32_t *bstart, int64_t n,
                                  int64_t m, const float *B, int64_t r, const float *d, float *out,
                                  float *colsum, void *stream) {
    return tmh::run_csr_dense_ent<float>(vals, meta, bstart, n, m, B, r, d, out, colsum, tmh::as_stream(stream));
}
int tm_csr_dense_sandwich_ent_f64(const double *vals, const uint16_t *meta, const uint32_t *bstart, int64_t n,
                                  int64_t m, const double *B, int64_t r, const double *d, double *out,
                                  double *colsum, void *stream) {
    return tmh::run_csr_dense_ent<double>(vals, meta, bstart, n, m, B, r, d, out, colsum, tmh::as_stream(stream));
}
}
```

tabmat_amd/ext/sparse.py:

```python
from __future__ import annotations

import os


from .. import _device as D
from .._lib import call
from ._types import CsrDev, DenseDev, SlabCsc, SlabEll, SlabEnt, SlabLg


def _csr_args(A: CsrDev):
    return (D.p(A.data), D.p(A.indices), D.p(A.indptr), A.n, A.m)


def sparse_sandwich(A: CsrDev, d, rows, cols):
    m = A.m if cols is None else D.nlen(cols)
    out = D.zeros((m, m), A.dtype)
    if m == 0 or (rows is not None and D.nlen(rows) == 0):
        return out
    D.same_float("sparse_sandwich", A.data, d)
    call(f"tm_sparse_sandwich_{D.fsuf(A.data)}", *_csr_args(A), D.p(d), D.p(rows), D.nlen(rows),
         D.p(cols), D.nlen(cols), D.p(out), D.stream_ptr())
    return out


# ... 55 lines not shown

def csr_matvec_multi(X: CsrDev, V, rows, cols, transpose):
    K = int(V.shape[1])
    n_cols = X.m if cols is None else D.nlen(cols)
    n_rows = X.n if rows is None else D.nlen(rows)
    out = D.zeros((n_cols if transpose else n_rows, K), X.dtype)
    if K == 0 or n_rows == 0 or n_cols == 0:
        return out
    D.same_float("csr_matvec_multi", X.data, V)
    Vc = V.contiguous()
    fn = "tm_csr_rmatvec_multi_" if transpose else "tm_csr_matvec_multi_"
    call(fn + D.fsuf(X.data), *_csr_args(X), D.p(Vc), K, D.p(rows), D.nlen(rows), D.p(cols),
         D.nlen(cols), D.p(out), D.stream_ptr())
    return out


def csr_dense_sandwich_slab(A: SlabCsc, B: DenseDev, d):
    assert B.n == A.n
    out = D.zeros((A.m, B.m), A.vals.dtype)
    if A.m == 0 or B.m == 0 or A.n == 0:
        return out
    D.same_float("csr_dense_sandwich_slab", A.vals, B.buf, d)
    call(f"tm_csr_dense_sandwich_slab_{D.fsuf(A.vals)}", D.p(A.vals), D.p(A.koff), D.p(A.cnt),
         D.p(A.gptr), A.n, A.m, D.p(B.buf), B.m, B.order_f, D.p(d), D.p(out), D.stream_ptr())
    return out


def ell_supported(B: DenseDev) -> bool:
    vec = 16 // B.buf.element_size()
    return (not B.order_f) and B.m % vec == 0 and B.m >= vec and B.buf.data_ptr() % 16 == 0


def csr_dense_sandwich_ell(A: SlabEll, B: DenseDev, d):
    assert B.n == A.n and ell_supported(B)
    if A.m == 0 or B.m == 0 or A.n == 0:
        return D.zeros((A.m, B.m), A.vals.dtype)
    out = D.zeros((A.mk, B.m), A.vals.dtype)
    D.same_float("csr_dense_sandwich_ell", A.vals, B.buf, d)
    fn = "tm_csr_dense_sandwich_ellw_" if A.wide else "tm_csr_dense_sandwich_ell_"
    call(fn + D.fsuf(A.vals), D.p(A.vals), D.p(A.koff), D.p(A.gptr),
         A.n, A.mk, D.p(B.buf), B.m, D.p(d), D.p(out), D.stream_ptr())
    return out[A.inv]


def csr_dense_sandwich_lg(A: SlabLg, B: DenseDev, d, unc=None, want_colsum=False):
    assert B.n == A.n and ell_supported(B)
    dt = A.dtype
    if A.m == 0 or B.m == 0 or A.n == 0:
        z = D.zeros((A.m, B.m), dt)
        return (z, D.zeros((A.m,), dt)) if want_colsum else z
    out = D.out_buf((A.mk, B.m), dt)
    u = int(A.unc if unc is None else unc)
    cs = D.out_buf((A.mk,), dt) if want_colsum else None
    if A.cvals is not None:
        D.same_float("csr_dense_sandwich_lg", A.cvals, B.buf, d)
        call("tm_csr_dense_sandwich_lgc_" + D.fsuf(A.cvals), D.p(A.cvals), D.p(A.cmap), D.p(A.crec),
             D.p(A.xkoff), A.n, A.mk, D.p(B.buf), B.m, D.p(d), u, D.p(out), D.p(cs), D.stream_ptr())
    elif want_colsum:
        D.same_float("csr_dense_sandwich_lg", A.vals, B.buf, d)
        call("tm_csr_dense_sandwich_lg_xtd_" + D.fsuf(A.vals), D.p(A.vals), D.p(A.koff), D.p(A.xptr),
             D.p(A.xvals), D.p(A.xkoff), A.n, A.mk, D.p(B.buf), B.m, D.p(d), u, D.p(out), D.p(cs),
             D.stream_ptr())
    else:
        D.same_float("csr_dense_sandwich_lg", A.vals, B.buf, d)
        call("tm_csr_dense_sandwich_lg_" + D.fsuf(A.vals), D.p(A.vals), D.p(A.koff), D.p(A.xptr),
             D.p(A.xvals), D.p(A.xkoff), A.n, A.mk, D.p(B.buf), B.m, D.p(d), u, D.p(out), D.stream_ptr())
    return (out[A.inv], cs[A.inv]) if want_colsum else out[A.inv]


def csr_dense_sandwich_ent(A: SlabEnt, B: DenseDev, d, want_colsum=False):
    assert B.n == A.n and ell_supported(B)
    dt = A.dtype
    if A.m == 0 or B.m == 0 or A.n == 0:
        z = D.zeros((A.m, B.m), dt)
        return (z, D.zeros((A.m,), dt)) if want_colsum else z
    out = D.out_buf((A.mk, B.m), dt)
    cs = D.out_buf((A.mk,), dt) if want_colsum else None
    D.same_float("csr_dense_sandwich_ent", A.vals, B.buf, d)
    call("tm_csr_dense_sandwich_ent_" + D.fsuf(A.vals), D.p(A.vals), D.p(A.meta), D.p(A.bstart), A.n, A.mk,
         D.p(B.buf), B.m, D.p(d), D.p(out), D.p(cs), D.stream_ptr())
    return (out[A.inv], cs[A.inv]) if want_colsum else out[A.inv]


def _row_table(A: CsrDev, rows, d, as_set: bool):
    import weakref

    import torch

    cm_data, cm_c8, cptr = A.chunk_major()
    cached = getattr(A, "_row_table", None)
    stamp = (rows.data_ptr(), rows._version, int(rows.numel()))
    if cached is not None and cached[0]() is rows and cached[4] == stamp:
        _, r64, dup, tabs, _ = cached
    else:
        r64 = torch.sort(rows.to(torch.int64)).values
        dup = bool((r64[1:] == r64[:-1]).any().item()) if r64.numel() > 1 else False
        tabs = {}
        A._row_table = (weakref.ref(rows), r64, dup, tabs, stamp)
    key = bool(as_set and dup)
    if key not in tabs:
        rr = torch.unique_consecutive(r64) if key else r64
        tabs[key] = (rr, torch.stack([cptr[:, rr], cptr[:, rr + 1]], dim=2).contiguous())
    rr, ranges = tabs[key]
    return cm_data, cm_c8, ranges, rr.to(torch.int32).contiguous(), d[rr].contiguous()


def sparse_sandwich_rows(A: CsrDev, d, rows):
    out = D.zeros((A.m, A.m), A.dtype)
    if A.m == 0 or D.nlen(rows) == 0 or A.data.numel() == 0:
        return out
    D.same_float("sparse_sandwich_rows", A.data, d)
    cm_data, cm_c8, ranges, r32, d_sel = _row_table(A, rows, d, True)
    cols = cm_c8 if K2B_U8 else A.chunk_cols32()
    call(f"tm_sparse_sandwich_chunked_rows_{'u8_' if K2B_U8 else ''}{D.fsuf(A.data)}", D.p(cm_data),
         D.p(cols), D.p(ranges),
         int(r32.numel()), A.m, int(cm_data.numel()), D.p(d_sel), D.p(out), D.stream_ptr())
    return out


def csr_dense_sandwich_rows(A: CsrDev, B: DenseDev, d, rows):
    out = D.zeros((A.m, B.m), A.dtype)
    if A.m == 0 or B.m == 0 or D.nlen(rows) == 0 or A.data.numel() == 0:
        return out
    D.same_float("csr_dense_sandwich_rows", A.data, B.buf, d)
    cm_data, cm_c8, ranges, r32, d_sel = _row_table(A, rows, d, False)
    call(f"tm_csr_dense_sandwich_rows_u8_{D.fsuf(A.data)}", D.p(cm_data), D.p(cm_c8), D.p(ranges),
         int(r32.numel()), D.p(r32), D.p(d_sel), A.n, A.m, D.p(B.buf), B.m, B.order_f, D.p(out),
         D.stream_ptr())
    return out


def sparse_sandwich_chunked(A: CsrDev, d):
    if A.m == 0 or A.n == 0:
        return D.zeros((A.m, A.m), A.dtype)
    out = D.out_buf((A.m, A.m), A.dtype)
    D.same_float("sparse_sandwich_chunked", A.data, d)
    cm_data, cm_c8, cptr = A.chunk_major()
    cols = cm_c8 if K2B_U8 else A.chunk_cols32()
    call(f"tm_sparse_sandwich_chunked_{'u8_' if K2B_U8 else ''}{D.fsuf(A.data)}", D.p(cm_data),
         D.p(cols), D.p(cptr),
         A.n, A.m, int(cm_data.numel()), D.p(d), D.p(out), D.stream_ptr())
    return out


K2_BLOCKS = True


def blocks_sandwich_pays(A: CsrDev) -> bool:
    import torch

    if not K2_BLOCKS or A.n == 0 or A.m == 0 or A.n >= 2**29:
        return False
    nnz = int(A.data.numel())
    nch = -(-A.m // 128)
    if not (0 < nnz < 2**31) or nnz / (A.n * nch) <= 4.5 or nch > 32:
        return False
    est = 16 * 2 * A.n * nch * (nch + 1) // 2
    return est * 3 < torch.cuda.mem_get_info(A.data.device)[0] or bool(getattr(A, "_pb", None))


K2B_U8 = os.environ.get("TABMAT_AMD_K2B_U8", "1") == "1"


def sparse_sandwich_blocks(A: CsrDev, d):
    if A.m == 0 or A.n == 0:
        return D.zeros((A.m, A.m), A.dtype)
    out = D.out_buf((A.m, A.m), A.dtype)
    D.same_float("sparse_sandwich_blocks", A.data, d)
    cm_data, cm_c8, cptr = A.chunk_major()
    blocks, wg_tab, max_nb = A.pair_blocks(d12=None if K2B_U8 else False)
    if int(blocks.shape[1]) == 3:
        call(f"tm_sparse_sandwich_blocks_p12_{D.fsuf(A.data)}", D.p(cm_data), D.p(cm_c8), D.p(cptr), A.n, A.m,
             int(cm_data.numel()), D.p(blocks), D.p(wg_tab), int(wg_tab.shape[0]), int(max_nb), D.p(d),
             D.p(out), D.stream_ptr())
        return out
    if K2B_U8:
        call(f"tm_sparse_sandwich_blocks_u8_{D.fsuf(A.data)}", D.p(cm_data), D.p(cm_c8), D.p(cptr), A.n, A.m,
             int(cm_data.numel()), D.p(blocks), D.p(wg_tab), int(wg_tab.shape[0]), int(max_nb), D.p(d),
             D.p(out), D.stream_ptr())
        return out
    cm_ind = A.chunk_cols32()
    call(f"tm_sparse_sandwich_blocks_{D.fsuf(A.data)}", D.p(cm_data), D.p(cm_ind), D.p(cptr), A.n, A.m,
         int(cm_data.numel()), D.p(blocks), D.p(wg_tab), int(wg_tab.shape[0]), int(max_nb), D.p(d),
         D.p(out), D.stream_ptr())
    return out


def sparse_sandwich_pairs(A: CsrDev, d):
    if A.m == 0 or A.n == 0:
        return D.zeros((A.m, A.m), A.dtype)
    out = D.out_buf((A.m, A.m), A.dtype)
    D.same_float("sparse_sandwich_pairs", A.data, d)
    _, _, cptr = A.chunk_major()
    if K2_PAIRS_PACKED and A.n < 2**25:
        rec = A.chunk_records_packed()
        call(f"tm_sparse_sandwich_pairs_pk_{D.fsuf(A.data)}", D.p(rec), D.p(cptr), A.n, A.m, int(A.data.numel()), D.p(d),
             D.p(out), D.stream_ptr())
        return out
    rec = A.chunk_records()
    call(f"tm_sparse_sandwich_pairs_{D.fsuf(A.data)}", D.p(rec), D.p(cptr), A.n, A.m, int(rec.shape[0]), D.p(d),
         D.p(out), D.stream_ptr())
    return out


def csc_dense_sandwich_sorted(A: CsrDev, B: DenseDev, d):
    if A.m == 0 or B.m == 0:
        return D.zeros((A.m, B.m), A.dtype)
    rows, vals, bstart, n_blocks, col_bptr = A.csc_blocks()
    out = D.out_buf((A.m, B.m), A.dtype)
    D.same_float("csc_dense_sandwich_sorted", vals, B.buf, d)
    call(f"tm_csc_dense_sandwich_sorted_{D.fsuf(vals)}", D.p(rows), D.p(vals), D.p(bstart),
         int(n_blocks), D.p(col_bptr), A.m, D.p(d), D.p(B.buf), B.m, D.p(out), D.stream_ptr())
    return out


def sparse_sandwich_direct(A: CsrDev, d):
    if A.m == 0 or A.n == 0:
        return D.zeros((A.m, A.m), A.dtype)
    out = D.out_buf((A.m, A.m), A.dtype)
    D.same_float("sparse_sandwich_direct", A.data, d)
    call(f"tm_sparse_sandwich_direct_{D.fsuf(A.data)}", D.p(A.data), D.p(A.indices), D.p(A.indptr),
         A.n, A.m, D.p(d), D.p(out), D.stream_ptr())
    return out


def direct_sandwich_pays(A: CsrDev) -> bool:
    nnz, n, m = int(A.data.numel()), A.n, A.m
    if n == 0 or nnz == 0 or m <= 1024:
        return False
    nch = (m + 127) // 128
    per_row = nnz / n
    pairs = n * per_row * (per_row + 1.0) / 2.0 * 1.3
    if nch > 32:
        return pairs / 15e9 < n * (nch * (nch + 1) / 2) * 0.3e-9
    if per_row / nch > 0.6:
        return False
    return pairs / 15e9 < n * (nch * (nch + 1) / 2) * 15e-12


K2_PAIRS = "auto"
K2_PAIRS_PACKED = os.environ.get("TABMAT_AMD_K2_PAIRS_PACKED", "1") == "1"
K2_PAIRS_MAX_M = 16384
K2_PAIRS_MAX_NNZ = 2**31 - 4 * 16 * 64


def pairs_sandwich_pays(A: CsrDev) -> bool:
    if K2_PAIRS != "auto":
        return K2_PAIRS == "1" and A.m <= K2_PAIRS_MAX_M and 0 < int(A.data.numel()) < K2_PAIRS_MAX_NNZ
    nnz, n, m = int(A.data.numel()), A.n, A.m
    if n == 0 or nnz == 0 or m <= 512 or m > K2_PAIRS_MAX_M or nnz >= K2_PAIRS_MAX_NNZ:
        return False
    nch = (m + 127) // 128
    parts = nch * (nch + 1) / 2
    per_row = nnz / n
    k = per_row / nch
    pairs = n * per_row * (per_row + 2.0) / 2.0
    pk = 0.75 if (K2_PAIRS_PACKED and n < 2**25) else 1.0
    t_pairs = (nnz * (nch + 1) / 2.0 * 2.3e-12 * pk * min(6.0, max(1.0, (1.6 / k) ** 0.8)) + pairs * 2.7e-12 * pk
               + min(parts, 768) * 0.8e-6 + max(0.0, parts - 768) * 0.1e-6)
    t_direct = pairs / 21e9
    if nch > 32:
        t_tiled = n * parts * 0.3e-9
    else:
        t_tiled = pairs * 1.15e-12 if k > 4.5 else n * parts * 17e-12 + pairs * 0.8e-12
    return t_pairs < 0.9 * min(t_direct, t_tiled)


def transpose_square_dot_weights(A: CsrDev, weights):
    out = D.zeros((A.m,), A.dtype)
    if A.n == 0 or A.m == 0 or A.data.numel() == 0:
# ... 18 lines not shown
```

tabmat_amd/ext/split.py:

```python
from __future__ import annotations

import ctypes as C

import numpy as np

from .. import _device as D
from .._lib import call
from ._types import CsrDev, DenseDev, SlabCsc


def sandwich_cat_dense(i_indices, i_ncol, d, mat_j: DenseDev, rows, j_cols, drop_first=False):
    n_j = mat_j.m if j_cols is None else D.nlen(j_cols)
    res = D.zeros((i_ncol, n_j), mat_j.dtype)
    n_rows = i_indices.numel() if rows is None else D.nlen(rows)
    if d.numel() == 0 or n_rows == 0 or n_j == 0 or i_ncol == 0:
        return res
    D.same_float("sandwich_cat_dense", mat_j.buf, d)
    call(f"tm_cat_dense_sandwich_{D.fsuf(mat_j.buf)}", D.p(i_indices), i_indices.numel(), i_ncol,
         int(drop_first), D.p(d), D.p(rows), D.nlen(rows), D.p(mat_j.buf), mat_j.m, mat_j.order_f,
         D.p(j_cols), D.nlen(j_cols), D.p(res), D.stream_ptr())
    return res


def sandwich_cat_cat(i_indices, j_indices, i_ncol, j_ncol, d, rows, i_drop_first=False,
# ... 262 lines not shown
        order = np.argsort(b, kind="stable").astype(np.int32)
        ends = np.cumsum(np.bincount(b, minlength=n_blocks))
        starts = np.concatenate([[0], ends[:-1]])
        return ([order[s:e] for s, e in zip(starts, ends)],
                [loc[order[s:e]] for s, e in zip(starts, ends)], len(cols))
    next_idx = [0] * n_blocks
    sub_idx = [[] for _ in range(n_blocks)]
    sub_cols = [[] for _ in range(n_blocks)]
    for i, c in enumerate(cols.tolist()):
        for j in range(n_blocks):
            ind = self.indices[j]
            k = next_idx[j]
            while k < len(ind) and ind[k] < c:
                k += 1
            next_idx[j] = k
            if k < len(ind) and ind[k] == c:
                sub_idx[j].append(i)
                sub_cols[j].append(k)
                next_idx[j] = k + 1
                break
    return (
        [np.array(s, dtype=np.int32) for s in sub_idx],
        [np.array(s, dtype=np.int32) for s in sub_cols],
        len(cols),
    )


def is_sorted(a) -> bool:
    a = np.asarray(a)
    return bool(np.all(a[1:] >= a[:-1]))


MAX_FUSED_CATS = 16


def _cat_args(cats):
    n = len(cats)
    codes = (C.c_void_p * n)(*[c[0].data_ptr() for c in cats])
    ncols = (C.c_int64 * n)(*[int(c[1]) for c in cats])
    drop = (C.c_int32 * n)(*[int(bool(c[2])) for c in cats])
    return codes, ncols, drop, n


def multi_cat_dense_wide_ok(cats, mat_j: DenseDev) -> bool:
    fb = mat_j.buf.element_size()
    vec = 2
    total = sum(int(c[1]) for c in cats)
    tile = (total * 16 * vec * 8 + 15) // 16 * 16
    lds = tile + 16 * 32 * (fb + 4 * len(cats))
    return (not mat_j.order_f and 1 <= len(cats) <= 8 and mat_j.m >= vec and mat_j.m % vec == 0
            and mat_j.buf.data_ptr() % 16 == 0 and lds <= 150 * 1024)


def multi_cat_dense_tile_ok(cats, mat_j: DenseDev) -> bool:
    total = sum(int(c[1]) for c in cats)
    m = mat_j.m
    if total == 0 or m == 0 or not 1 <= len(cats) <= 16:
        return False
    tj = 64
    while tj > 1 and 8 * total * tj > 128 * 1024:
        tj >>= 1
    while tj > 1 and tj // 2 >= m:
        tj >>= 1
    return 8 * total * tj <= 128 * 1024 and (m + tj - 1) // tj <= 2


def multi_cat_dense_sandwich(cats, d, mat_j: DenseDev, rows=None):
    total = sum(int(c[1]) for c in cats)
    if total == 0 or mat_j.m == 0 or mat_j.n == 0 or (rows is not None and D.nlen(rows) == 0):
        return D.zeros((total, mat_j.m), mat_j.dtype)
    res = D.out_buf((total, mat_j.m), mat_j.dtype)
    codes, ncols, drop, n = _cat_args(cats)
    if rows is not None:
        D.same_float("multi_cat_dense_sandwich", mat_j.buf, d)
        call(f"tm_multi_cat_dense_sandwich_rows_{D.fsuf(mat_j.buf)}", codes, ncols, drop, n, mat_j.n,
             D.p(d), D.p(mat_j.buf), mat_j.m, D.p(rows), D.nlen(rows), D.p(res), D.stream_ptr())
        return res
    D.same_float("multi_cat_dense_sandwich", mat_j.buf, d)
    call(f"tm_multi_cat_dense_sandwich_{D.fsuf(mat_j.buf)}", codes, ncols, drop, n, mat_j.n,
         D.p(d), D.p(mat_j.buf), mat_j.m, mat_j.order_f, D.p(res), D.stream_ptr())
    return res


def multi_cat_sparse_sandwich(cats, d, S: SlabCsc):
    total = sum(int(c[1]) for c in cats)
    if total == 0 or S.m == 0 or S.n == 0:
        return D.zeros((total, S.m), S.vals.dtype)
    res = D.out_buf((total, S.m), S.vals.dtype)
    codes, ncols, drop, n = _cat_args(cats)
    D.same_float("multi_cat_sparse_sandwich", S.vals, d)
    call(f"tm_multi_cat_sparse_sandwich_slab_{D.fsuf(S.vals)}", codes, ncols, drop, n, S.n, D.p(d),
         D.p(S.vals), D.p(S.koff), D.p(S.ecol), D.p(S.gptr), S.m, D.p(res), D.stream_ptr())
    return res


PACKED_CODES = True


def pack_codes(cats):
    import torch

    total = sum(int(c[1]) for c in cats)
    if not PACKED_CODES or len(cats) > 3 or total >= 1023 or len(cats) == 0:
        return None
    codes, ncols, drop, n = _cat_args(cats)
    nrow = int(cats[0][0].numel())
    out = torch.empty((nrow,), dtype=torch.int32, device=cats[0][0].device)
    call("tm_multi_cat_pack_codes", codes, ncols, drop, n, nrow, D.p(out), D.stream_ptr())
    return out


def multi_cat_sparse_sandwich_ent(cats, d, E, packed=None):
    total = sum(int(c[1]) for c in cats)
    if total == 0 or E.m == 0 or E.n == 0:
        return D.zeros((total, E.m), E.vals.dtype)
    res = D.out_buf((total, E.mk), E.vals.dtype)
    codes, ncols, drop, n = _cat_args(cats)
    D.same_float("multi_cat_sparse_sandwich_ent", E.vals, d)
    if packed is not None:
        call(f"tm_multi_cat_sparse_sandwich_entp_{D.fsuf(E.vals)}", codes, ncols, drop, n, E.n, D.p(d),
             D.p(E.vals), D.p(E.meta), D.p(E.bstart), E.n_slots(), E.mk, D.p(packed), D.p(res), D.stream_ptr())
        return res[:, E.inv]
    call(f"tm_multi_cat_sparse_sandwich_ent_{D.fsuf(E.vals)}", codes, ncols, drop, n, E.n, D.p(d),
         D.p(E.vals), D.p(E.meta), D.p(E.bstart), E.n_slots(), E.mk, D.p(res), D.stream_ptr())
    return res[:, E.inv]


def multi_cat_sparse_sandwich_rows(cats, d, A, rows):
    from . import sparse as xs

    total = sum(int(c[1]) for c in cats)
    if total == 0 or A.m == 0 or D.nlen(rows) == 0 or A.data.numel() == 0:
        return D.zeros((total, A.m), A.data.dtype)
    res = D.out_buf((total, A.m), A.data.dtype)
    codes, ncols, drop, n = _cat_args(cats)
    D.same_float("multi_cat_sparse_sandwich_rows", A.data, d)
    cm_data, cm_c8, ranges, r32, d_sel = xs._row_table(A, rows, d, False)
    call(f"tm_multi_cat_sparse_sandwich_rows_u8_{D.fsuf(A.data)}", codes, ncols, drop, n, D.p(cm_data),
         D.p(cm_c8), D.p(ranges), D.p(r32), int(r32.numel()), A.m, D.p(d_sel), D.p(res), D.stream_ptr())
    return res
```

tabmat_amd/sparse_matrix.py:

```python
from __future__ import annotations

import os

import numpy as np
import torch
from scipy import sparse as sps

from . import _device as D
from .ext import sparse as xs
from .ext._types import CsrDev, SlabCsc, SlabEll, SlabEnt, SlabLg
from .matrix_base import MatrixBase
from .util import (
    check_indexer,
    check_matvec_dimensions,
    check_matvec_out_shape,
    check_sandwich_compatible,
    check_transpose_matvec_out_shape,
    normalize_index,
    device_row_index,
    selects_all_columns,
)


ELL_MAX_PAD = 8.0
# ... 229 lines not shown
                r = None
                if rows is not None:
                    r64 = rows.to(torch.int64)
                    sel = r64[(r64 >= a) & (r64 < b)]
                    if sel.numel() == 0:
                        continue
                    r = (sel - a).to(torch.int32)
                res = part._sandwich_dev(d[a:b], r, cols)
                out = res if out is None else out + res
            if out is None:
                k = self.shape[1] if cols is None else D.nlen(cols)
                out = D.zeros((k, k), d.dtype)
            return out
        A = self._dev()
        from . import categorical_matrix as _cm

        if _cm.DETERMINISTIC and A.data.numel() > 0 and self.shape[0] > 0:
            res = self._sandwich_deterministic(d, rows, cols)
            if res is not None:
                return res
            import warnings

            warnings.warn("TABMAT_AMD_DETERMINISTIC=1: this sparse block has no entry twin, its self sandwich "
                          "falls back to the LDS-atomic kernels and is NOT bit-reproducible from run to run",
                          RuntimeWarning, stacklevel=3)
        if getattr(self, "_direct_pays", None) is None:
            self._direct_pays = xs.direct_sandwich_pays(A)
        w = D.nlen(cols) if cols is not None else 0
        if (0 < w <= NARROW_COLS and 2 * w < self.shape[1] and self.shape[0] > 0 and A.data.numel() > 0
                and self._narrow_pays(w)
                and self.shape[0] * w * A.data.element_size() * 4 < torch.cuda.mem_get_info()[0]):
            from .ext import dense as xd
            from .ext._types import DenseDev

            rws, vls, bstart, _, col_bptr = A.csc_blocks()
            mx = getattr(self, "_max_col_len", None)
            if mx is None:
                ends = bstart[col_bptr]
                mx = self._max_col_len = int((ends[1:] - ends[:-1]).max().item())
            cd = cols.to(torch.int64)
            seg = torch.stack([bstart[col_bptr[cd]], bstart[col_bptr[cd + 1]]], dim=1).contiguous()
            T = torch.zeros((self.shape[0], w), dtype=A.data.dtype, device=A.data.device)
            xs.csc_densify_cols(rws, vls, seg, torch.arange(w, dtype=torch.int32, device=A.data.device),
                                mx, T)
            return xd.dense_sandwich(DenseDev(T, self.shape[0], w, 0), d, rows, None)
        pp = getattr(self, "_pairs_pay", None)
        if pp is None:
            pp = self._pairs_pay = xs.pairs_sandwich_pays(A)
        if pp and (rows is None or D.nlen(rows) > 0.3 * self.shape[0]):
            d = D.masked_d(d, rows, as_set=True)
            res = xs.sparse_sandwich_pairs(A, d)
            if cols is not None:
                c64 = cols.to(torch.int64)
                res = res[c64][:, c64].contiguous()
            return res
        pays = getattr(self, "_direct_pays", None)
        if pays is None:
            pays = self._direct_pays = xs.direct_sandwich_pays(A)
        if pays:
            d = D.masked_d(d, rows, as_set=True)
            res = xs.sparse_sandwich_direct(A, d)
            if cols is not None:
                c64 = cols.to(torch.int64)
                res = res[c64][:, c64].contiguous()
            return res
        if A.data.numel() > 0 and A.data.numel() < 2**31 and self.shape[1] <= 128 * 32:
            if rows is not None and 0 < D.nlen(rows) <= ROW_LIST_FRACTION * self.shape[0]:
                res = xs.sparse_sandwich_rows(A, d, rows)
                if cols is not None:
                    c64 = cols.to(torch.int64)
                    res = res[c64][:, c64].contiguous()
                return res
            d = D.masked_d(d, rows, as_set=True)
            bl = getattr(self, "_blocks_pay", None)
            if bl is None:
                bl = self._blocks_pay = xs.blocks_sandwich_pays(A)
            res = xs.sparse_sandwich_blocks(A, d) if bl else xs.sparse_sandwich_chunked(A, d)
            if cols is not None:
                c64 = cols.to(torch.int64)
                res = res[c64][:, c64].contiguous()
            return res
        return xs.sparse_sandwich(A, d, rows, cols)

    def _ent_det(self):
        ent = self._ent()
        if ent is None:
            hit = getattr(self, "_entblk_det", None)
            if hit is None:
                twin = SlabEnt.from_csr(self._dev(), max_pad=None)
                hit = self._entblk_det = twin if twin is not None else False
            ent = hit or None
        return ent

    def _sandwich_deterministic(self, d, rows, cols=None):
        from .ext._types import DenseDev

        ent = self._ent_det()
        if ent is None:
            return None
        n, m = self.shape
        A = self._dev()
        d = D.masked_d(d, rows, as_set=True)
        inv = None
        if cols is None:
            sel = torch.arange(m, dtype=torch.int64, device=d.device)
        else:
            sel, inv = torch.unique(cols.to(torch.int64), return_inverse=True)
            if int(sel.numel()) == int(inv.numel()) and bool((sel == cols.to(torch.int64)).all()):
                inv = None
        k = int(sel.numel())
        out = torch.empty((m, k), dtype=d.dtype, device=d.device)
        W = 128
        for c0 in range(0, k, W):
            w = min(W, k - c0)
            w_pad = (w + 3) // 4 * 4
            colmap = torch.full((m,), -1, dtype=torch.int32, device=d.device)
            colmap[sel[c0:c0 + w]] = torch.arange(w, dtype=torch.int32, device=d.device)
            T = torch.zeros((n, w_pad), dtype=A.data.dtype, device=d.device)
            xs.csr_densify_cols(A, colmap, T)
            res = xs.csr_dense_sandwich_ent(ent, DenseDev(T, n, w_pad, 0), d)
            out[:, c0:c0 + w] = res[:, :w]
            del T
        out = out if cols is None else out[sel]
        low = torch.tril(out)
        full = low + torch.tril(out, -1).T
        if inv is not None:
            full = full.index_select(0, inv).index_select(1, inv)
        return full

    def sandwich(self, d, rows=None, cols=None):
        on_dev = D.is_dev(d)
        if not on_dev:
            d = np.asarray(d)
        check_sandwich_compatible(self, d)
        res = self._sandwich_dev(D.to_dev(d), D.idx_dev(normalize_index(rows, self.shape[0])),
                                 D.idx_dev(normalize_index(cols, self.shape[1])))
        return res if on_dev else D.to_host(res)

    def _cross_sandwich_dev(self, other, d, rows, L_cols, R_cols, colsum_box=None):
        from .categorical_matrix import CategoricalMatrix
        from .dense_matrix import DenseMatrix

        if isinstance(other, DenseMatrix):
            if other.dtype != self.dtype:
                raise TypeError(
                    "self, B and d all need to be of same dtype, either np.float64 or "
                    f"np.float32. This matrix is of type {self.dtype}, B is of type "
                    f"{other.dtype}.")
            Bd = other._dev_c()
            A = self._dev()
            if (rows is not None and 0 < D.nlen(rows) <= ROW_LIST_FRACTION_K3 * self.shape[0]
                    and 0 < A.data.numel() < 2**31 and self.shape[1] <= 128 * 32):
                res = xs.csr_dense_sandwich_rows(A, Bd, d, rows)
                if L_cols is not None:
                    res = res[L_cols.to(torch.int64)]
                if R_cols is not None:
                    res = res[:, R_cols.to(torch.int64)]
                return res
            if self.shape[0] > 0 and self._dev().data.numel() > 0 and (
                    rows is None or self._values_finite()):
                d = D.masked_d(d, rows)
                if (A.data.numel() <= SORTED_K3_NNZ_PER_ROW * self.shape[0] and self.shape[1] >= 1024
                        and xs.ell_supported(Bd)):
                    res = xs.csc_dense_sandwich_sorted(A, Bd, d)
                    if L_cols is not None:
                        res = res[L_cols.to(torch.int64)]
                    if R_cols is not None:
                        res = res[:, R_cols.to(torch.int64)]
                    return res
                wide = Bd.m > 64 and xs.ell_supported(Bd)
                ent = self._ent() if wide else None
                lg = self._lg() if (wide and ent is None) else None
                ell = None
                if ent is None and lg is None and xs.ell_supported(Bd):
                    ell = self._ell(wide=Bd.m > 64)
                if ent is not None and colsum_box is not None:
                    res, cs = xs.csr_dense_sandwich_ent(ent, Bd, d, want_colsum=True)
                    colsum_box.append(cs if L_cols is None else cs[L_cols.to(torch.int64)])
                elif ent is not None:
                    res = xs.csr_dense_sandwich_ent(ent, Bd, d)
                elif lg is not None and colsum_box is not None:
                    res, cs = xs.csr_dense_sandwich_lg(lg, Bd, d, want_colsum=True)
                    colsum_box.append(cs if L_cols is None else cs[L_cols.to(torch.int64)])
                elif lg is not None:
                    res = xs.csr_dense_sandwich_lg(lg, Bd, d)
                elif ell is not None:
                    res = xs.csr_dense_sandwich_ell(ell, Bd, d)
                else:
                    res = xs.csr_dense_sandwich_slab(self._slab(), Bd, d)
                if L_cols is not None:
                    res = res[L_cols.to(torch.int64)]
                if R_cols is not None:
                    res = res[:, R_cols.to(torch.int64)]
                return res
            return xs.csr_dense_sandwich(self._dev(), Bd, d, rows, L_cols, R_cols)
        if isinstance(other, CategoricalMatrix):
            return other._cross_sandwich_dev(self, d, rows, R_cols, L_cols).T
        raise TypeError

    def _cross_sandwich(self, other, d, rows, L_cols=None, R_cols=None):
        on_dev = D.is_dev(d)
        if not on_dev:
            d = np.asarray(d)
        check_sandwich_compatible(self, d)
        res = self._cross_sandwich_dev(
            other, D.to_dev(d), D.idx_dev(normalize_index(rows, self.shape[0])),
            D.idx_dev(normalize_index(L_cols, self.shape[1])),
            D.idx_dev(normalize_index(R_cols, other.shape[1])))
        return res if on_dev else D.to_host(res)

    def sandwich_dense(self, B, d, rows, L_cols, R_cols):
        from .dense_matrix import DenseMatrix

        Bm = B if isinstance(B, DenseMatrix) else DenseMatrix(B)
        return self._cross_sandwich(Bm, d, rows, L_cols, R_cols)

    def _matvec_dev(self, vec, rows, cols, out, transpose):
        fn = xs.csc_rmatvec if transpose else xs.csr_matvec
        return fn(self._dev(), vec, rows, cols, out)

# ... 45 lines not shown
```

tabmat_amd/split_matrix.py:

```python
from __future__ import annotations

import os
import warnings
from collections.abc import Sequence
from typing import Optional, Union

import numpy as np
import torch
from scipy import sparse as sps

from . import _device as D
from .categorical_matrix import CategoricalMatrix
from .dense_matrix import DenseMatrix
from .ext import split as xsplit
from .ext.dense import dense_sandwich_matvec as xd_smv
from .matrix_base import MatrixBase
from .sparse_matrix import SparseMatrix
from .standardized_mat import StandardizedMatrix
from .util import (
    check_matvec_dimensions,
    check_matvec_out_shape,
    check_sandwich_compatible,
    check_transpose_matvec_out_shape,
    collapse_identity,
    normalize_index,
    set_up_rows_or_cols,
)


ROW_LIST_FRACTION_CATSPARSE = 0.04
DIAG_FROM_PAIRS = True
CAT_PAIRS_FUSED = os.environ.get("TABMAT_AMD_CAT_PAIRS", "1") != "0"
FULL_THEN_SELECT = float(os.environ.get("TABMAT_AMD_FULL_THEN_SELECT", "0.5"))
FULL_RESULT_MAX_BYTES = 256 << 20
FULL_UNSELECTED_SHARE = 0.2
FULL_THEN_SELECT_MV = 0.0
NARROW_COLS = int(os.environ.get("TABMAT_AMD_NARROW_COLS", "128"))
from . import categorical_matrix as _cm
from . import sparse_matrix as _spm


class _Centering:
    NARROW_GROUP = 1 << 20

    def __init__(self, vec):
        self.vec = dict(vec)
        self.cs_centered = set()
        self.groups = None

    def get(self, b):
        return self.vec.get(b)


class _Xtv:

    def __init__(self, v):
        self.v = v
        self.out = {}


def as_tabmat(a):
    if isinstance(a, (MatrixBase, StandardizedMatrix)):
        return a
    if sps.issparse(a):
        return SparseMatrix(a.tocsc(copy=False))
    if isinstance(a, np.ndarray):
        return DenseMatrix(a)
    raise ValueError(f"Cannot convert type {type(a)} to Matrix.")


def hstack(tup: Sequence) -> MatrixBase:
    mats = [as_tabmat(a) for a in tup]
    if not mats:
        raise ValueError("Need at least one array to concatenate.")
    if all(isinstance(m, SparseMatrix) for m in mats):
        return SparseMatrix(sps.hstack([m.array_csc for m in mats]))
    if all(isinstance(m, DenseMatrix) for m in mats):
        return DenseMatrix(np.hstack([m.toarray() for m in mats]))
    return SplitMatrix(mats)


def _merge_same_kind(matrices, indices):
    for kind in (DenseMatrix, SparseMatrix):
        which = [i for i, m in enumerate(matrices) if isinstance(m, kind)]
        if len(which) <= 1:
            continue
        gidx = np.concatenate([indices[i] for i in which])
        order = np.argsort(gidx)
        names = np.concatenate([np.array(matrices[i]._colnames, dtype=object) for i in which])
        terms = np.concatenate([np.array(matrices[i]._terms, dtype=object) for i in which])
        if kind is DenseMatrix:
            merged = DenseMatrix(np.hstack([matrices[i].toarray() for i in which])[:, order])
        else:
            merged = SparseMatrix(sps.hstack([matrices[i].array_csc for i in which]).tocsc()[:, order])
        merged._colnames = names[order].tolist()
        merged._terms = terms[order].tolist()
        matrices[which[0]] = merged
        indices[which[0]] = gidx[order]
        drop = set(which[1:])
        matrices = [m for i, m in enumerate(matrices) if i not in drop]
        indices = [x for i, x in enumerate(indices) if i not in drop]
    return matrices, indices


class SplitMatrix(MatrixBase):

    def __init__(self, matrices: Sequence[MatrixBase], indices: Optional[list] = None):
        flat, corrections = [], []
        for mat in matrices:
            if not isinstance(mat, MatrixBase):
                raise ValueError(
                    "Expected all elements of matrices to be subclasses of MatrixBase.")
# ... 225 lines not shown
            xtd[pd] = cs.to(torch.float64)
        if center is not None:
            return out, xtd, cmask, center.groups
        return out, xtd

    FUSED_LEVELS = 496
    FUSED_CATS = 8

    def _cat_groups(self, cat_ids):
        groups, cur, tot = [], [], 0
        for i in cat_ids:
            k = self.matrices[i].shape[1]
            if k > self.FUSED_LEVELS:
                continue
            if cur and (len(cur) == self.FUSED_CATS or tot + k > self.FUSED_LEVELS):
                groups.append(cur)
                cur, tot = [], 0
            cur.append(i)
            tot += k
        if cur:
            groups.append(cur)
        return groups

    def _cat_pairs_plan(self):
        plan = self.__dict__.get("_cp_plan", False)
        if plan is False:
            plan = None
            ids = [i for i, m in enumerate(self.matrices)
                   if isinstance(m, CategoricalMatrix) and m.shape[1] > 0]
            if len(ids) >= 1:
                pos = self._full_dev_indices()
                plan = xsplit.CatPairsPlan([(i, self.matrices[i].shape[1]) for i in ids],
                                           [pos[i] for i in ids])
            self.__dict__["_cp_plan"] = plan
        return plan

    def _cat_hist_plan(self):
        plan = self.__dict__.get("_ch_plan", False)
        if plan is False:
            plan = None
            ids = [i for i, m in enumerate(self.matrices)
                   if isinstance(m, CategoricalMatrix) and m.shape[1] > 0 and m.shape[0] > 0]
            if len(ids) >= 2:
                pos = self._full_dev_indices()
                plan = xsplit.CatPairsPlan([(i, self.matrices[i].shape[1]) for i in ids],
                                           [pos[i] for i in ids], diag_only=True)
            self.__dict__["_ch_plan"] = plan
        return plan

    def _fused_cats(self, mw, cats, cat_ids, d_eff, rows, total, budget, d_rows=None):
        if isinstance(mw, DenseMatrix) and xsplit.multi_cat_dense_wide_ok(cats, mw._dev_c()):
            if rows is not None and D.nlen(rows) <= 0.5 * self.shape[0]:
                return xsplit.multi_cat_dense_sandwich(cats, d_rows, mw._dev_c(), rows)
            return xsplit.multi_cat_dense_sandwich(cats, d_eff, mw._dev_c())
        if isinstance(mw, DenseMatrix) and xsplit.multi_cat_dense_tile_ok(cats, mw._dev_c()):
            return xsplit.multi_cat_dense_sandwich(cats, d_eff, mw._dev_c())
        if isinstance(mw, DenseMatrix):
            if xsplit.cat_dense_sorted_ok(mw._dev_c()):
                return None
            from .ext import sparse as xs

            oh, inv = self._onehot_slab(cat_ids)
            return xs.csr_dense_sandwich_slab(oh, mw._dev_c(), d_eff)[inv]
        if (isinstance(mw, SparseMatrix) and total * 33 <= budget and rows is not None
                and 0 < D.nlen(rows) <= ROW_LIST_FRACTION_CATSPARSE * self.shape[0]
                and 0 < mw._dev().data.numel() < 2**31):
            return xsplit.multi_cat_sparse_sandwich_rows(cats, d_rows, mw._dev(), rows)
        if (isinstance(mw, SparseMatrix) and total * 33 <= budget
                and mw._dev().data.numel() > 0 and (rows is None or mw._values_finite())):
            ent = None
            if len(cats) <= 8 and (getattr(mw, "_entblk", None) or any(
                    isinstance(mo, DenseMatrix) and mo.shape[1] > 64 and mo.dtype == mw.dtype
                    for mo in self.matrices)):
                ent = mw._ent()
            if ent is not None:
                pk_cache = self.__dict__.setdefault("_packed_codes", {})
                key = tuple(cat_ids)
                if key not in pk_cache:
                    pk_cache[key] = xsplit.pack_codes(cats)
                return xsplit.multi_cat_sparse_sandwich_ent(cats, d_eff, ent, pk_cache[key])
            return xsplit.multi_cat_sparse_sandwich(cats, d_eff, mw._slab())
        return None

    def _parts(self):
        parts = self.__dict__.get("_row_parts", False)
        if parts is False:
            parts = None
            big = [m for m in self.matrices
                   if isinstance(m, SparseMatrix) and m._dev().data.numel() >= _spm.PART_NNZ]
            if big:
                n = self.shape[0]
                lead = max(big, key=lambda m: m._dev().data.numel())
                ptr = lead._dev().indptr
                nnz = int(ptr[-1].item())
                k = -(-nnz // max(1, int(0.8 * _spm.PART_NNZ)))
                while True:
                    targets = torch.arange(1, k, device=ptr.device, dtype=torch.int64) * nnz // k
                    cuts = [0] + torch.searchsorted(ptr, targets).clamp_(0, n).tolist() + [n]
                    cuts = sorted(set(int(c) for c in cuts))
                    ok = all(int((m._dev().indptr[cuts[1:]] - m._dev().indptr[cuts[:-1]]).max().item())
                             < _spm.PART_NNZ for m in big)
                    if ok or k >= n:
                        break
                    k += 1
                parts = [(a, b, self[a:b]) for a, b in zip(cuts[:-1], cuts[1:]) if b > a]
            self.__dict__["_row_parts"] = parts
        return parts

    def _sandwich_parts(self, parts, d, rows, cols_host, colsum, center=None):
        out = None
        for a, b, part in parts:
            r = None
            if rows is not None:
                r64 = rows.to(torch.int64)
                sel = r64[(r64 >= a) & (r64 < b)]
                if sel.numel() == 0:
                    continue
                r = (sel - a).to(torch.int32)
            cs = [None] * len(self.matrices) if colsum is not None else None
            sub_cen = None if center is None else _Centering(center.vec)
            res = part._sandwich_dev(d[a:b], r, cols_host, None, cs, center=sub_cen)
            if sub_cen is not None:
                center.groups = sub_cen.groups
            if sub_cen is not None and colsum is not None:
                dsum = (d[a:b] if r is None else d[a:b][r.to(torch.int64)]).sum(dtype=torch.float64)
                _, sub_p, _ = self._sandwich_plan(cols_host)
                for i in sub_cen.cs_centered:
                    if cs[i] is not None and sub_cen.get(i) is not None:
                        cv = sub_cen.get(i).to(torch.float64)
                        if sub_p[i] is not None:
                            cv = cv[sub_p[i].to(torch.int64)]
                        cs[i] = cs[i].to(torch.float64) + cv * dsum
            out = res if out is None else out + res
            if colsum is not None:
                for i, c in enumerate(cs):
                    if c is None:
                        colsum[i] = False
                    elif colsum[i] is not False:
                        colsum[i] = c if colsum[i] is None else colsum[i] + c
        if colsum is not None:
            for i, c in enumerate(colsum):
                if c is False:
                    colsum[i] = None
        if out is None:
            _, _, n_cols = self._sandwich_plan(cols_host)
            out = D.zeros((n_cols, n_cols), torch.float64)
        return out

    def _full_product_pays(self, sub_h) -> bool:
        p = self.shape[1]
        if p * p * 8 > FULL_RESULT_MAX_BYTES:
            return False
        n = max(self.shape[0], 1)
        tot = unsel = 0.0
        for b, mb in enumerate(self.matrices):
            if isinstance(mb, DenseMatrix):
                wb = float(mb.shape[1])
            elif isinstance(mb, SparseMatrix):
                nnz = mb._devblk.data.numel() if mb._devblk is not None else mb._host().nnz
                wb = max(1.0, float(nnz) / n)
            else:
                wb = 1.0 + mb.shape[1] / 256.0
            tot += wb
            if len(sub_h[b]) == 0:
                unsel += wb
        return unsel <= FULL_UNSELECTED_SHARE * tot
# ... 77 lines not shown
        dm._devblk = DenseDev(T, n, nar["w_pad"], 0)
        sub_cen = None
        if center is not None:
            tc = torch.zeros((nar["w_pad"],), dtype=d.dtype, device=d.device)
            for b, t0, s, idx in nar["parts"]:
                if center.get(b) is not None:
                    tc[t0:t0 + s] = center.get(b)[idx.to(torch.int64)]
            sub_cen = _Centering({0: tc})
        try:
            cs_tmp = [None] * len(tmp.matrices) if colsum is not None else None
            full = tmp._sandwich_dev(d, rows, None, None, cs_tmp, center=sub_cen)
        finally:
            dm._devblk = None
        if colsum is not None:
            if cs_tmp[0] is not None:
                for b, t0, s, _ in nar["parts"]:
                    colsum[b] = cs_tmp[0][t0:t0 + s]
                    if sub_cen is not None and 0 in sub_cen.cs_centered:
                        center.cs_centered.add(b)
            for k, i in enumerate(nar["cat"]):
                if cs_tmp[1 + k] is not None and i in nar["cat_sub"]:
                    colsum[i] = cs_tmp[1 + k][nar["cat_sub"][i]]
        if center is not None:
            g = torch.full_like(nar["sel"], -1, dtype=torch.int32)
            g[nar["sel"] < nar["w_pad"]] = _Centering.NARROW_GROUP
            center.groups = g
        sel = nar["sel"]
        return full.index_select(0, sel).index_select(1, sel)

    def _sandwich_dev(self, d, rows, cols_host, plan=None, colsum=None, center=None, xtv=None):
        if cols_host is not None and len(cols_host) >= FULL_THEN_SELECT * self.shape[1] \
                and len(cols_host) > 0 and self._full_product_pays_cols(cols_host):
            pos_d, sub_d, n_cols = plan if plan is not None else self._sandwich_plan(cols_host)
            cs_full = [None] * len(self.matrices) if colsum is not None else None
            full = self._sandwich_dev(d, rows, None, None, cs_full, center=center, xtv=xtv)
            if colsum is not None:
                for i, c in enumerate(cs_full):
                    if c is not None:
                        colsum[i] = c if sub_d[i] is None else c[sub_d[i].to(torch.int64)]
            cd = self._cols_dev64(cols_host)
            return full.index_select(0, cd).index_select(1, cd)
        parts = self._parts()
        if parts is not None:
            return self._sandwich_parts(parts, d, rows, cols_host, colsum, center)
        if cols_host is not None and plan is None and NARROW_COLS > 0:
            nar = self._narrow_plan(cols_host)
            if nar == "wide":
                cs_full = [None] * len(self.matrices) if colsum is not None else None
                full = self._sandwich_dev(d, rows, None, None, cs_full, center=center, xtv=xtv)
                if colsum is not None:
                    _, sub_sel, _ = self._sandwich_plan(cols_host)
                    for i, c in enumerate(cs_full):
                        if c is not None:
                            colsum[i] = c if sub_sel[i] is None else c[sub_sel[i].to(torch.int64)]
                cd = self._cols_dev64(cols_host)
                return full.index_select(0, cd).index_select(1, cd)
            if nar is not None and d.dtype == D.torch_dtype(self.dtype):
                return self._sandwich_narrow(nar, d, rows, colsum, center)
        pos_d, sub_d, n_cols = plan if plan is not None else self._sandwich_plan(cols_host)
        out = D.zeros((n_cols, n_cols), torch.float64)
        mats = self.matrices
        empty = [sd is not None and D.nlen(sd) == 0 for sd in sub_d]
        done = set()
        return self._sandwich_terms(d, rows, cols_host, colsum, out, pos_d, sub_d, empty, done, center,
                                    xtv if cols_host is None else None)

    def _sandwich_terms(self, d, rows, cols_host, colsum, out, pos_d, sub_d, empty, done, center=None, xtv=None):
        from .ext import dense as xd

        mats = self.matrices
        cat_ids = [i for i, m in enumerate(mats) if isinstance(m, CategoricalMatrix) and not empty[i]
                   and m.shape[1] > 0]
        budget = (128 * 1024) // 8
        groups = self._cat_groups(cat_ids)
        if groups:
            d_eff = D.masked_d(d, rows)
        for grp in groups:
            cats = [(mats[i]._dev(), mats[i].shape[1], mats[i].drop_first) for i in grp]
            total = sum(c[1] for c in cats)
            offs = np.concatenate([[0], np.cumsum([c[1] for c in cats])])
            for w, mw in enumerate(mats):
                if empty[w] or mw.dtype != self.dtype or d.dtype != D.torch_dtype(self.dtype):
                    continue
                stacked = self._fused_cats(mw, cats, grp, d_eff, rows, total, budget, d)
                if stacked is None:
                    continue
                whole = cols_host is None and len(grp) > 1
                if whole:
                    cache = self.__dict__.setdefault("_group_pos", {})
                    gpos = cache.get(tuple(grp))
                    if gpos is None:
                        gpos = cache[tuple(grp)] = torch.cat([pos_d[i] for i in grp])
                    xsplit.scatter_block(stacked.contiguous(), gpos, pos_d[w], out, mirror=True)
                for ci, i in enumerate(grp):
                    res = stacked[int(offs[ci]):int(offs[ci + 1])]
                    if (colsum is not None and colsum[w] is None and not mats[i].drop_first
                            and not mats[i]._has_missings):
                        cs = res.sum(dim=0)
                        colsum[w] = cs if sub_d[w] is None else cs[sub_d[w].to(torch.int64)]
                    if not whole:
                        res = CategoricalMatrix._restrict(res, sub_d[i], sub_d[w])
                        xsplit.scatter_block(res.contiguous(), pos_d[i], pos_d[w], out, mirror=True)
                    done.add((min(i, w), max(i, w)))
        big = [i for i in cat_ids if mats[i].shape[1] > self.FUSED_LEVELS]
        if len(big) >= 2 and len(big) <= 16 and d.dtype == D.torch_dtype(self.dtype):
            cats = [(mats[i]._dev(), mats[i].shape[1], mats[i].drop_first) for i in big]
            offs = np.concatenate([[0], np.cumsum([c[1] for c in cats])])
            d_big = None
            for w, mw in enumerate(mats):
                if (empty[w] or not isinstance(mw, DenseMatrix) or mw.dtype != self.dtype
                        or not xsplit.multi_cat_dense_tile_ok(cats, mw._dev_c())):
                    continue
                if d_big is None:
                    d_big = D.masked_d(d, rows)
                stacked = xsplit.multi_cat_dense_sandwich(cats, d_big, mw._dev_c())
                for ci, i in enumerate(big):
                    res = stacked[int(offs[ci]):int(offs[ci + 1])]
                    if (colsum is not None and colsum[w] is None and not mats[i].drop_first
                            and not mats[i]._has_missings):
                        cs = res.sum(dim=0)
                        colsum[w] = cs if sub_d[w] is None else cs[sub_d[w].to(torch.int64)]
                    res = CategoricalMatrix._restrict(res, sub_d[i], sub_d[w])
                    xsplit.scatter_block(res.contiguous(), pos_d[i], pos_d[w], out, mirror=True)
                    done.add((min(i, w), max(i, w)))
        cat_diag = {}
        diag_scattered = set()
        det = _cm.DETERMINISTIC
        plan = self._cat_pairs_plan() if CAT_PAIRS_FUSED and not det else None
        if (plan is not None and plan.n_pairs > 0
                and d.dtype in (torch.float32, torch.float64)
                and d.dtype == D.torch_dtype(self.dtype)):
            cl = [(mats[i]._dev(), mats[i].shape[1], mats[i].drop_first) for i in plan.cat_ids]
            pos_sel = None if cols_host is None else self._pairs_pos_sel(plan, cols_host)
            tables = xsplit.multi_cat_pairs(plan, cl, d, rows, out, pos=pos_sel)
            for i, j, toff, li, lj, stride in plan.pairs:
                if i == j:
                    if not empty[i]:
                        full = tables[toff:toff + (li - 1) * stride + 1:stride]
                        if sub_d[i] is not None and colsum is not None:
                            full = full[sub_d[i].to(torch.int64)]
                        cat_diag[i] = full.to(d.dtype)
                        diag_scattered.add(i)
                else:
                    done.add((i, j))
        complete = [isinstance(m, CategoricalMatrix) and not m.drop_first and not m._has_missings
                    and sub_d[k] is None and not empty[k] for k, m in enumerate(mats)]
        for i, mi in enumerate(mats):
            if empty[i] or not isinstance(mi, CategoricalMatrix):
                continue
            for j in range(i + 1, len(mats)):
                if empty[j] or not isinstance(mats[j], CategoricalMatrix) or (i, j) in done:
                    continue
                res = mi._cross_sandwich_dev(mats[j], d, rows, sub_d[i], sub_d[j])
                xsplit.scatter_block(res.contiguous(), pos_d[i], pos_d[j], out, mirror=True)
                done.add((i, j))
                if DIAG_FROM_PAIRS and not det and complete[j] and i not in cat_diag:
                    cat_diag[i] = res.sum(dim=1)
                if DIAG_FROM_PAIRS and not det and complete[i] and j not in cat_diag:
                    cat_diag[j] = res.sum(dim=0)
        for i, mi in enumerate(mats):
            if empty[i]:
                continue
            if isinstance(mi, CategoricalMatrix):
                diag = cat_diag[i] if i in cat_diag else mi._sandwich_diag_dev(d, rows, sub_d[i])
                if colsum is not None:
                    colsum[i] = diag
                if i not in diag_scattered:
                    xsplit.scatter_block(diag, pos_d[i], pos_d[i], out, diag=True)
            elif (xtv is not None and colsum is None and center is None and isinstance(mi, DenseMatrix)
                  and sub_d[i] is None and (both := mi._sandwich_xtv_dev(d, xtv.v, rows)) is not None):
                res, xtv.out[i] = both
                xsplit.scatter_block(res, pos_d[i], pos_d[i], out)
            elif (colsum is not None and colsum[i] is None and isinstance(mi, DenseMatrix)
                  and rows is None and sub_d[i] is None
                  and (both := mi._sandwich_xtd_dev(d, cen_i := (center.get(i) if center else None))) is not None):
                res, colsum[i] = both
                if cen_i is not None:
                    center.cs_centered.add(i)
                xsplit.scatter_block(res, pos_d[i], pos_d[i], out)
            elif isinstance(mi, DenseMatrix) and center is not None and center.get(i) is not None:
                res = mi._sandwich_dev(d, rows, sub_d[i], center=center.get(i))
                xsplit.scatter_block(res, pos_d[i], pos_d[i], out)
            else:
                res = mi._sandwich_dev(d, rows, sub_d[i])
                xsplit.scatter_block(res, pos_d[i], pos_d[i], out)
        for i, mi in enumerate(mats):
            if empty[i]:
                continue
            for j in range(i + 1, len(mats)):
                if empty[j] or (i, j) in done:
                    continue
                si, di = (i, j) if isinstance(mi, SparseMatrix) else (j, i)
                if (colsum is not None and colsum[si] is None and isinstance(mats[si], SparseMatrix)
                        and isinstance(mats[di], DenseMatrix)):
                    box = []
                    res = mats[si]._cross_sandwich_dev(mats[di], d, rows, sub_d[si], sub_d[di],
                                                       colsum_box=box)
                    if box:
                        colsum[si] = box[0]
                    if si != i:
                        res = res.T
                else:
                    res = mi._cross_sandwich_dev(mats[j], d, rows, sub_d[i], sub_d[j])
                xsplit.scatter_block(res.contiguous(), pos_d[i], pos_d[j], out, mirror=True)
        return out

    def sandwich_graph(self, d, rows=None, cols=None):
        from .graph import CapturedProduct

        check_sandwich_compatible(self, d)
        rows_d = D.idx_dev(normalize_index(rows, self.shape[0]))
        cols_n = collapse_identity(normalize_index(cols, self.shape[1]), self.shape[1])
        plan = self._sandwich_plan(cols_n)
        return CapturedProduct(lambda dd: self._sandwich_dev(dd, rows_d, cols_n, plan), d)

    def sandwich(self, d, rows=None, cols=None):
        on_dev = D.is_dev(d)
        if not on_dev:
            d = np.asarray(d)
        check_sandwich_compatible(self, d)
        rows_n = normalize_index(rows, self.shape[0])
        cols_n = collapse_identity(normalize_index(cols, self.shape[1]), self.shape[1])
        out = self._sandwich_dev(D.to_dev(d), D.idx_dev(rows_n), cols_n)
        return out if on_dev else D.to_host(out)

    def sandwich_and_transpose_matvec(self, d, v, rows=None, cols=None):
        from .matrix_base import _check_1d

        _check_1d(v)
        d_dev_side, v_dev_side = D.is_dev(d), D.is_dev(v)
        if not d_dev_side:
            d = np.asarray(d)
        if not v_dev_side:
            v = np.asarray(v)
        check_sandwich_compatible(self, d)
        check_matvec_dimensions(self, v, transpose=True)
        rows_n = normalize_index(rows, self.shape[0])
        cols_n = collapse_identity(normalize_index(cols, self.shape[1]), self.shape[1])
        tdt = D.torch_dtype(self.dtype)
        v_dev = D.to_dev(v, tdt)
        acc = None
        if (tdt == torch.float64 and not _cm.DETERMINISTIC
                and (rows_n is None or len(rows_n) < self.shape[0])):
            acc = _Xtv(v_dev)
        H = self._sandwich_dev(D.to_dev(d), D.idx_dev(rows_n), cols_n, xtv=acc)
        g, _ = self._transpose_matvec_dev(v_dev, rows_n, cols_n, done=None if acc is None else acc.out)
        if not v_dev_side:
            g = D.to_host(g)
            if np.issubdtype(v.dtype, np.floating):
                g = g.astype(np.result_type(self.dtype, v.dtype), copy=False)
        return (H if d_dev_side else D.to_host(H)), g

    def sandwich_matvec(self, d, u, rows=None, cols=None):
        from .matrix_base import _smv_args, _smv_compose

        a = _smv_args(self, d, u, rows, cols, h_dtype=np.float64)
        if a.trivial is not None:
            return a.finish(a.trivial)
        tdt = D.torch_dtype(self.dtype)
        res = None
        if (rows is None and cols is None) or self._blocks_finite():
            res = self._smv_dev(a.d_masked(tdt), a.u_full(tdt))
        if res is None:
            return a.finish(_smv_compose(self, a))
        g = res[0]
        if a.cols is not None:
            g = g[self._cols_dev64(a.cols)]
        return a.finish(g)

    def matvec(self, v, cols=None, out=None):
        assert not sps.issparse(v)
        on_dev = D.is_dev(v)
        if not on_dev:
            v = np.asarray(v)
        check_matvec_dimensions(self, v, transpose=False)
        check_matvec_out_shape(self, out)
        if v.ndim > 1 and any(isinstance(m, CategoricalMatrix) for m in self.matrices):
# ... 178 lines not shown
```

Before: 1017 GB/s.

## Fuse partial reduction with scatter into output for sparse and categorical sandwich blocks

Adds reduce-scatter kernels that sum per-block partials and write each element straight into its final position in the p×p output, mirrored, instead of reducing into a temporary tile, untiling, then scattering. New _into entry points cover the sparse blocks path, the sparse×dense ENT cross path and the fused multi-categorical dense/sparse paths, and SplitMatrix routes to them when FINISH_INTO is on. A liveness mask also lets the blocks path skip zeroing the workspace. This removes several intermediate buffers and kernel launches per block, at the cost of extra code paths and stricter preconditions (f64 only, no colsum).

```diff
diff --git a/include/tabmat_hip.h b/include/tabmat_hip.h
--- a/include/tabmat_hip.h
+++ b/include/tabmat_hip.h
@@ -166,6 +166,10 @@
                                       int64_t n, int64_t m, int64_t nnz, const int32_t *blocks12,
                                       const int32_t *wg_tab, int n_wg, int max_nb, const double *d, double *out,
                                       void *stream);
+int tm_sparse_sandwich_blocks_p12_into_f64(const double *cm_data, const uint8_t *cm_col8, const int32_t *cptr,
+                                           int64_t n, int64_t m, int64_t nnz, const int32_t *blocks12,
+                                           const int32_t *wg_tab, int n_wg, int max_nb, const double *d, double *out,
+                                           int64_t p, const int64_t *pos, const uint8_t *slot_live, void *stream);
 
 int tm_csr_dense_sandwich_f32(const float *csr_data, const int32_t *csr_indices,
                               const int64_t *csr_indptr, int64_t n, int64_t m, const float *B,
@@ -241,6 +245,9 @@
 int tm_csr_dense_sandwich_ent_f64(const double *vals, const uint16_t *meta, const uint32_t *bstart, int64_t n,
                                   int64_t m, const double *B, int64_t r, const double *d, double *out,
                                   double *colsum, void *stream);
+int tm_csr_dense_sandwich_ent_into_f64(const double *vals, const uint16_t *meta, const uint32_t *bstart, int64_t n,
+                                       int64_t m, const double *B, int64_t r, const double *d, double *out,
+                                       int64_t p, const int64_t *rpos, const int64_t *cpos, void *stream);
 
 
 int tm_index_narrow_i64(const int64_t *src, int64_t count, int64_t limit, int32_t *dst, int32_t *bad, void *stream);
@@ -389,6 +396,10 @@
                                     const int32_t *h_drop_first, int n_cats, int64_t n,
                                     const double *d, const double *M, int64_t M_ncol, int order_f,
                                     double *out, void *stream);
+int tm_multi_cat_dense_sandwich_into_f64(const void *const *h_codes, const int64_t *h_ncols,
+                                         const int32_t *h_drop_first, int n_cats, int64_t n, const double *d,
+                                         const double *M, int64_t M_ncol, double *out, int64_t p,
+                                         const int64_t *rpos, const int64_t *cpos, void *stream);
 int tm_multi_cat_dense_sandwich_rows_f32(const void *const *h_codes, const int64_t *h_ncols,
                                          const int32_t *h_drop_first, int n_cats, int64_t n,
                                          const float *d, const float *M, int64_t M_ncol,
@@ -441,6 +452,11 @@
                                           const int32_t *h_drop_first, int n_cats, int64_t n, const double *d,
                                           const double *vals, const uint16_t *meta, const uint32_t *bstart,
                                           int64_t n_slots, int64_t mk, const uint32_t *packed, double *out, void *stream);
+int tm_multi_cat_sparse_sandwich_ent_into_f64(const void *const *h_codes, const int64_t *h_ncols,
+                                              const int32_t *h_drop_first, int n_cats, int64_t n, const double *d,
+                                              const double *vals, const uint16_t *meta, const uint32_t *bstart,
+                                              int64_t n_slots, int64_t mk, const uint32_t *packed, double *out,
+                                              int64_t p, const int64_t *rpos, const int64_t *cpos, void *stream);
 
 int tm_multi_cat_sparse_sandwich_slab_f32(const void *const *h_codes, const int64_t *h_ncols,
                                           const int32_t *h_drop_first, int n_cats, int64_t n,
diff --git a/tabmat_amd/csrc/cat.hip b/tabmat_amd/csrc/cat.hip
--- a/tabmat_amd/csrc/cat.hip
+++ b/tabmat_amd/csrc/cat.hip
@@ -816,6 +816,16 @@
     out[e] = tmp[((j / TJ) * total + a) * TJ + (j % TJ)];
 }
 
+struct CatTileMap {
+    int TJ;
+    int64_t m;
+    __device__ bool operator()(int part, int64_t e, int64_t &a, int64_t &j) const {
+        a = e / TJ;
+        j = (int64_t)part * TJ + e % TJ;
+        return j < m;
+    }
+};
+
 template <typename F, bool STAGE>
 __global__ __launch_bounds__(1024) void multi_cat_sparse_kernel(
     CatSet cs, const F *__restrict__ d, const F *__restrict__ vals,
@@ -1304,13 +1314,18 @@
 static int run_multi_cat_dense(const void *const *h_codes, const int64_t *h_ncols,
                                const int32_t *h_drop, int n_cats, int64_t n, const F *d, const F *M,
                                int64_t m, int order_f, F *out, hipStream_t st,
-                               const int32_t *rows = nullptr, int64_t n_rows = 0) {
+                               const int32_t *rows = nullptr, int64_t n_rows = 0, double *pp = nullptr,
+                               int64_t p = 0, const int64_t *rpos = nullptr, const int64_t *cpos = nullptr) {
     CatSet cs;
     int rc = make_catset(h_codes, h_ncols, h_drop, n_cats, &cs);
     if (rc) return rc;
     const int64_t total = (int64_t)cs.total * m;
     if (total == 0) return TM_OK;
     if (rows != nullptr) n = n_rows;
+    if (pp != nullptr && (n == 0 || rows != nullptr)) {
+        set_error("multi_cat_dense_into: needs n > 0 and takes no row list");
+        return TM_EINVAL;
+    }
     if (n == 0) {
         TM_HIP(hipMemsetAsync(out, 0, sizeof(F) * (size_t)total, st));
         return TM_OK;
@@ -1356,6 +1371,9 @@
             else if (n_cats == 7) rc = gow(&multi_cat_dense_wide_kernel<F, 7>);
             else rc = gow(&multi_cat_dense_wide_kernel<F, 8>);
             if (rc) return rc;
+            if (pp != nullptr)
+                return launch_reduce_scatter<F>(ws, stride, (int)nblk, (int)n_parts, CatTileMap{TJW, m}, rpos, cpos,
+                                                pp, p, 1, st);
             rc = launch_reduce_partials<F>(ws, stride, (int)nblk, (int)n_parts, tmp, n_parts * stride,
                                            false, st);
             if (rc) return rc;
@@ -1364,6 +1382,10 @@
             TM_LAUNCH_CHECK();
             return TM_OK;
         }
+    }
+    if (pp != nullptr) {
+        set_error("multi_cat_dense_into: needs the wide-load path (C-ordered, aligned, <= 8 categoricals)");
+        return TM_EUNSUPPORTED;
     }
     if (rows != nullptr) {
         set_error("multi_cat_dense: the row-list form needs the wide-load path");
@@ -1534,12 +1556,17 @@
 static int run_multi_cat_sparse_ent(const void *const *h_codes, const int64_t *h_ncols, const int32_t *h_drop,
                                     int n_cats, int64_t n, const F *d, const F *vals, const unsigned short *meta,
                                     const unsigned *bstart, int64_t mk, F *out, hipStream_t st,
-                                    const unsigned *packed = nullptr, int64_t n_slots = 0) {
+                                    const unsigned *packed = nullptr, int64_t n_slots = 0, double *pp = nullptr,
+                                    int64_t p = 0, const int64_t *rpos = nullptr, const int64_t *cpos = nullptr) {
     CatSet cs;
     int rc = make_catset(h_codes, h_ncols, h_drop, n_cats, &cs);
     if (rc) return rc;
     const int64_t total = (int64_t)cs.total * mk;
     if (total == 0) return TM_OK;
+    if (pp != nullptr && n == 0) {
+        set_error("multi_cat_sparse_ent_into: needs n > 0");
+        return TM_EINVAL;
+    }
     if (n == 0) {
         TM_HIP(hipMemsetAsync(out, 0, sizeof(F) * (size_t)total, st));
         return TM_OK;
@@ -1616,6 +1643,8 @@
         prof_end(st);
         TM_LAUNCH_CHECK();
     }
+    if (pp != nullptr)
+        return launch_reduce_scatter<F>(ws, stride, (int)nblk, n_pairs, CatTileMap{GC, mk}, rpos, cpos, pp, p, 1, st);
     rc = launch_reduce_partials<F>(ws, stride, (int)nblk, n_pairs, tmp, (int64_t)n_pairs * stride, false, st);
     if (rc) return rc;
     hipLaunchKernelGGL((multi_cat_untile_kernel<F>), dim3((unsigned)ceil_div(total, 256)), dim3(256), 0, st, tmp,
@@ -1837,6 +1866,29 @@
                                           int64_t n_slots, int64_t mk, const uint32_t *packed, double *out, void *stream) {
     return run_multi_cat_sparse_ent<double>(h_codes, h_ncols, h_drop_first, n_cats, n, d, vals, meta, bstart, mk,
                                             out, as_stream(stream), packed, n_slots);
+}
+int tm_multi_cat_dense_sandwich_into_f64(const void *const *h_codes, const int64_t *h_ncols,
+                                         const int32_t *h_drop_first, int n_cats, int64_t n, const double *d,
+                                         const double *M, int64_t M_ncol, double *out, int64_t p,
+                                         const int64_t *rpos, const int64_t *cpos, void *stream) {
+    if (out == nullptr || rpos == nullptr || cpos == nullptr) {
+        set_error("tm_multi_cat_dense_sandwich_into_f64: out, rpos and cpos are required");
+        return TM_EINVAL;
+    }
+    return run_multi_cat_dense<double>(h_codes, h_ncols, h_drop_first, n_cats, n, d, M, M_ncol, 0, nullptr,
+                                       as_stream(stream), nullptr, 0, out, p, rpos, cpos);
+}
+int tm_multi_cat_sparse_sandwich_ent_into_f64(const void *const *h_codes, const int64_t *h_ncols,
+                                              const int32_t *h_drop_first, int n_cats, int64_t n, const double *d,
+                                              const double *vals, const uint16_t *meta, const uint32_t *bstart,
+                                              int64_t n_slots, int64_t mk, const uint32_t *packed, double *out,
+                                              int64_t p, const int64_t *rpos, const int64_t *cpos, void *stream) {
+    if (out == nullptr || rpos == nullptr || cpos == nullptr) {
+        set_error("tm_multi_cat_sparse_sandwich_ent_into_f64: out, rpos and cpos are required");
+        return TM_EINVAL;
+    }
+    return run_multi_cat_sparse_ent<double>(h_codes, h_ncols, h_drop_first, n_cats, n, d, vals, meta, bstart, mk,
+                                            nullptr, as_stream(stream), packed, n_slots, out, p, rpos, cpos);
 }
 int tm_multi_cat_sparse_sandwich_slab_f32(const void *const *h_codes, const int64_t *h_ncols,
                                           const int32_t *h_drop_first, int n_cats, int64_t n,
diff --git a/tabmat_amd/csrc/reduce.hpp b/tabmat_amd/csrc/reduce.hpp
--- a/tabmat_amd/csrc/reduce.hpp
+++ b/tabmat_amd/csrc/reduce.hpp
@@ -58,6 +58,64 @@
     return TM_OK;
 }
 
+template <typename F, int NW, typename MAP>
+__global__ __launch_bounds__(NW * 64) void reduce_scatter_kernel(const F *__restrict__ ws, int64_t stride, int nb,
+                                                                 MAP map, const int64_t *__restrict__ rpos,
+                                                                 const int64_t *__restrict__ cpos,
+                                                                 double *__restrict__ out, int64_t p, int mirror,
+                                                                 const uint8_t *__restrict__ live) {
+    __shared__ double red[NW][64];
+    const int lane = threadIdx.x & 63;
+    const int wave = threadIdx.x >> 6;
+    const int64_t e = (int64_t)blockIdx.x * 64 + lane;
+    const int part = blockIdx.y;
+    double acc = 0.0;
+    if (e < stride) {
+        const F *q = ws + ((int64_t)part * nb) * stride + e;
+        if (live == nullptr) {
+            for (int b = wave; b < nb; b += NW) acc += (double)q[(int64_t)b * stride];
+        } else {
+            const uint8_t *lv = live + (int64_t)part * nb;
+            for (int b = wave; b < nb; b += NW) {
+                const uint8_t l = lv[b];
+                const double v = (double)q[(int64_t)b * stride];
+                acc += l ? v : 0.0;
+            }
+        }
+    }
+    red[wave][lane] = acc;
+    __syncthreads();
+    int64_t i, j;
+    if (wave == 0 && e < stride && map(part, e, i, j)) {
+        const int64_t r = rpos[i], c = cpos[j];
+        if (r >= 0 && c >= 0) {
+            double s = 0.0;
+#pragma unroll
+            for (int w = 0; w < NW; w += 4)
+                s += (red[w][lane] + red[w + 1][lane]) + (red[w + 2][lane] + red[w + 3][lane]);
+            const double v = (double)(F)s;
+            out[r * p + c] = v;
+            if (mirror) out[c * p + r] = v;
+        }
+    }
+}
+
+template <typename F, typename MAP>
+inline int launch_reduce_scatter(const F *ws, int64_t stride, int nb, int n_parts, MAP map, const int64_t *rpos,
+                                 const int64_t *cpos, double *out, int64_t p, int mirror, hipStream_t st,
+                                 const uint8_t *live = nullptr) {
+    dim3 grid((unsigned)ceil_div(stride, 64), (unsigned)n_parts);
+    const bool small = (int64_t)grid.x * grid.y < 1024 && nb > 16;
+    if (small)
+        hipLaunchKernelGGL((reduce_scatter_kernel<F, 16, MAP>), grid, dim3(1024), 0, st, ws, stride, nb, map, rpos,
+                           cpos, out, p, mirror, live);
+    else
+        hipLaunchKernelGGL((reduce_scatter_kernel<F, 4, MAP>), grid, dim3(256), 0, st, ws, stride, nb, map, rpos,
+                           cpos, out, p, mirror, live);
+    TM_LAUNCH_CHECK();
+    return TM_OK;
+}
+
 __global__ void fill_i32_kernel(int32_t *p, int64_t n, int32_t v);
 __global__ void scatter_iota_i32_kernel(int32_t *map, const int32_t *cols, int64_t n_cols);
 
diff --git a/tabmat_amd/csrc/sparse_blocks.hip b/tabmat_amd/csrc/sparse_blocks.hip
--- a/tabmat_amd/csrc/sparse_blocks.hip
+++ b/tabmat_amd/csrc/sparse_blocks.hip
@@ -18,6 +18,19 @@
     const int part = I * (I + 1) / 2 + J;
     out[(int64_t)i * n_out + j] = tiles[(int64_t)part * KB_TS * KB_TS + (hi % KB_TS) * KB_TS + (lo % KB_TS)];
 }
+
+struct BlocksTileMap {
+    int64_t m;
+    __device__ bool operator()(int part, int64_t e, int64_t &hi, int64_t &lo) const {
+        int I = 0;
+        while ((I + 1) * (I + 2) / 2 <= part) ++I;
+        const int J = part - I * (I + 1) / 2;
+        const int64_t h = e / KB_TS, l = e % KB_TS;
+        hi = (int64_t)I * KB_TS + h;
+        lo = (int64_t)J * KB_TS + l;
+        return hi < m && lo < m && (I != J || l <= h);
+    }
+};
 
 constexpr int KB_FLAG_REP_A = 1 << 16;
 constexpr int KB_FLAG_REP_B = 1 << 17;
@@ -202,8 +215,14 @@
 template <typename F, bool U8 = false, bool D12 = false>
 static int run_sparse_sandwich_blocks(const F *data, const int32_t *ind, const int32_t *cptr, int64_t n,
                                       int64_t m, int64_t nnz, const int32_t *blocks, const int32_t *wg_tab,
-                                      int n_wg, int max_nb, const F *d, F *out, hipStream_t st) {
+                                      int n_wg, int max_nb, const F *d, F *out, hipStream_t st,
+                                      double *pp = nullptr, int64_t p = 0, const int64_t *pos = nullptr,
+                                      const uint8_t *slot_live = nullptr) {
     if (m == 0) return TM_OK;
+    if (pp != nullptr && (n == 0 || nnz == 0 || n_wg == 0)) {
+        set_error("sparse_sandwich_blocks_into: needs a non-empty block");
+        return TM_EINVAL;
+    }
     if (n == 0 || nnz == 0 || n_wg == 0) {
         TM_HIP(hipMemsetAsync(out, 0, sizeof(F) * (size_t)(m * m), st));
         return TM_OK;
@@ -222,7 +241,7 @@
     if (rc) return rc;
     F *tmp = reinterpret_cast<F *>(wsv);
     F *ws = reinterpret_cast<F *>(reinterpret_cast<char *>(wsv) + tmp_bytes);
-    TM_HIP(hipMemsetAsync(ws, 0, ws_bytes, st));
+    if (pp == nullptr || slot_live == nullptr) TM_HIP(hipMemsetAsync(ws, 0, ws_bytes, st));
     auto kern = &sparse_sandwich_blocks_kernel<F, U8, D12>;
     TM_HIP(hipFuncSetAttribute(reinterpret_cast<const void *>(kern),
                                hipFuncAttributeMaxDynamicSharedMemorySize, (int)lds));
@@ -233,6 +252,9 @@
                        max_nb, ws, wg_log_ptr());
     prof_end(st);
     TM_LAUNCH_CHECK();
+    if (pp != nullptr)
+        return launch_reduce_scatter<F>(ws, (int64_t)TS * TS, max_nb, n_parts, BlocksTileMap{m}, pos, pos, pp, p, 1,
+                                        st, slot_live);
     rc = launch_reduce_partials<F>(ws, (int64_t)TS * TS, max_nb, n_parts, tmp, (int64_t)n_parts * TS * TS,
                                    false, st);
     if (rc) return rc;
@@ -295,4 +317,18 @@
                                                                tmh::as_stream(stream));
 }
 
-}
+int tm_sparse_sandwich_blocks_p12_into_f64(const double *cm_data, const uint8_t *cm_col8, const int32_t *cptr,
+                                           int64_t n, int64_t m, int64_t nnz, const int32_t *blocks12,
+                                           const int32_t *wg_tab, int n_wg, int max_nb, const double *d, double *out,
+                                           int64_t p, const int64_t *pos, const uint8_t *slot_live,
+                                           void *stream) {
+    if (out == nullptr || pos == nullptr) {
+        tmh::set_error("tm_sparse_sandwich_blocks_p12_into_f64: out and pos are required");
+        return TM_EINVAL;
+    }
+    return tmh::run_sparse_sandwich_blocks<double, true, true>(cm_data, reinterpret_cast<const int32_t *>(cm_col8), cptr,
+                                                               n, m, nnz, blocks12, wg_tab, n_wg, max_nb, d, nullptr,
+                                                               tmh::as_stream(stream), out, p, pos, slot_live);
+}
+
+}
diff --git a/tabmat_amd/csrc/sparse_ent.hip b/tabmat_amd/csrc/sparse_ent.hip
--- a/tabmat_amd/csrc/sparse_ent.hip
+++ b/tabmat_amd/csrc/sparse_ent.hip
@@ -358,9 +358,20 @@
     csum[c] = (F)a;
 }
 
+struct EnMap {
+    int64_t nB;
+    __device__ bool operator()(int part, int64_t e, int64_t &i, int64_t &j) const {
+        i = e / EN_W;
+        j = (int64_t)part * EN_W + e % EN_W;
+        return j < nB;
+    }
+};
+
 template <typename F>
 static int run_csr_dense_ent(const F *vals, const uint16_t *meta, const uint32_t *bstart, int64_t n, int64_t m,
-                             const F *B, int64_t r, const F *d, F *out, F *colsum, hipStream_t st) {
+                             const F *B, int64_t r, const F *d, F *out, F *colsum, hipStream_t st,
+                             double *pp = nullptr, int64_t p = 0, const int64_t *rpos = nullptr,
+                             const int64_t *cpos = nullptr) {
     const int64_t nB = r;
     const int64_t total = m * nB;
     if (total == 0) return TM_OK;
@@ -378,6 +389,10 @@
         return TM_EUNSUPPORTED;
     }
     const int64_t n_slabs = ceil_div(n, EN_R);
+    if (pp != nullptr && (n_slabs == 0 || colsum != nullptr)) {
+        set_error("tm_csr_dense_sandwich_ent_into: needs n > 0 and takes no column sums");
+        return TM_EINVAL;
+    }
     const int n_groups = (int)(m / EN_C);
     const int n_parts = (int)ceil_div(nB, EN_W);
     const int nz = (int)ceil_div(n_groups, EN_NW);
@@ -411,6 +426,8 @@
                        reinterpret_cast<long long *>((uintptr_t)tune("ent_prof", 0)));
     prof_end(st);
     TM_LAUNCH_CHECK();
+    if (pp != nullptr)
+        return launch_reduce_scatter<F>(ws, stride, (int)nblk, n_parts, EnMap{nB}, rpos, cpos, pp, p, 1, st);
     rc = launch_reduce_partials<F>(ws, stride, (int)nblk, n_parts, tmp, n_parts * stride, false, st);
     if (rc) return rc;
     hipLaunchKernelGGL((en_untile_kernel<F>), dim3((unsigned)ceil_div(total, 256)), dim3(256), 0, st, tmp, m,
@@ -441,4 +458,14 @@
                                   double *colsum, void *stream) {
     return tmh::run_csr_dense_ent<double>(vals, meta, bstart, n, m, B, r, d, out, colsum, tmh::as_stream(stream));
 }
-}
+int tm_csr_dense_sandwich_ent_into_f64(const double *vals, const uint16_t *meta, const uint32_t *bstart, int64_t n,
+                                       int64_t m, const double *B, int64_t r, const double *d, double *out,
+                                       int64_t p, const int64_t *rpos, const int64_t *cpos, void *stream) {
+    if (out == nullptr || rpos == nullptr || cpos == nullptr) {
+        tmh::set_error("tm_csr_dense_sandwich_ent_into_f64: out, rpos and cpos are required");
+        return TM_EINVAL;
+    }
+    return tmh::run_csr_dense_ent<double>(vals, meta, bstart, n, m, B, r, d, nullptr, nullptr,
+                                          tmh::as_stream(stream), out, p, rpos, cpos);
+}
+}
diff --git a/tabmat_amd/ext/sparse.py b/tabmat_amd/ext/sparse.py
--- a/tabmat_amd/ext/sparse.py
+++ b/tabmat_amd/ext/sparse.py
@@ -161,6 +161,13 @@
     return (out[A.inv], cs[A.inv]) if want_colsum else out[A.inv]
 
 
+def csr_dense_sandwich_ent_into(A: SlabEnt, B: DenseDev, d, out, rpos, cpos):
+    assert B.n == A.n and ell_supported(B) and A.n > 0 and A.m > 0 and B.m > 0
+    D.same_float("csr_dense_sandwich_ent_into", A.vals, B.buf, d)
+    call("tm_csr_dense_sandwich_ent_into_f64", D.p(A.vals), D.p(A.meta), D.p(A.bstart), A.n, A.mk, D.p(B.buf),
+         B.m, D.p(d), D.p(out), int(out.shape[0]), D.p(rpos), D.p(cpos), D.stream_ptr())
+
+
 def _row_table(A: CsrDev, rows, d, as_set: bool):
     import weakref
 
@@ -265,6 +272,28 @@
     return out
 
 
+def sparse_sandwich_blocks_into(A: CsrDev, d, out, pos) -> bool:
+    import torch
+
+    if A.m == 0 or A.n == 0 or A.dtype != torch.float64 or not K2B_U8:
+        return False
+    cm_data, cm_c8, cptr = A.chunk_major()
+    blocks, wg_tab, max_nb = A.pair_blocks(d12=None)
+    if int(blocks.shape[1]) != 3 or cm_data.numel() == 0 or int(wg_tab.shape[0]) == 0:
+        return False
+    D.same_float("sparse_sandwich_blocks_into", A.data, d)
+    hit = getattr(A, "_k2b_live", None)
+    if hit is None or hit[0] is not wg_tab:
+        nch = -(-A.m // 128)
+        live = torch.zeros((nch * (nch + 1) // 2) * int(max_nb), dtype=torch.uint8, device=wg_tab.device)
+        live[wg_tab[:, 0].to(torch.int64) * int(max_nb) + wg_tab[:, 1].to(torch.int64)] = 1
+        hit = A._k2b_live = (wg_tab, live)
+    call("tm_sparse_sandwich_blocks_p12_into_f64", D.p(cm_data), D.p(cm_c8), D.p(cptr), A.n, A.m,
+         int(cm_data.numel()), D.p(blocks), D.p(wg_tab), int(wg_tab.shape[0]), int(max_nb), D.p(d),
+         D.p(out), int(out.shape[0]), D.p(pos), D.p(hit[1]), D.stream_ptr())
+    return True
+
+
 def sparse_sandwich_pairs(A: CsrDev, d):
     if A.m == 0 or A.n == 0:
         return D.zeros((A.m, A.m), A.dtype)
diff --git a/tabmat_amd/ext/split.py b/tabmat_amd/ext/split.py
--- a/tabmat_amd/ext/split.py
+++ b/tabmat_amd/ext/split.py
@@ -368,6 +368,23 @@
     return res
 
 
+def multi_cat_dense_sandwich_into(cats, d, mat_j: DenseDev, out, rpos, cpos):
+    assert mat_j.n > 0 and mat_j.m > 0 and multi_cat_dense_wide_ok(cats, mat_j)
+    codes, ncols, drop, n = _cat_args(cats)
+    D.same_float("multi_cat_dense_sandwich_into", mat_j.buf, d)
+    call("tm_multi_cat_dense_sandwich_into_f64", codes, ncols, drop, n, mat_j.n, D.p(d), D.p(mat_j.buf), mat_j.m,
+         D.p(out), int(out.shape[0]), D.p(rpos), D.p(cpos), D.stream_ptr())
+
+
+def multi_cat_sparse_sandwich_ent_into(cats, d, E, out, rpos, cpos, packed=None):
+    assert E.n > 0 and E.m > 0
+    codes, ncols, drop, n = _cat_args(cats)
+    D.same_float("multi_cat_sparse_sandwich_ent_into", E.vals, d)
+    call("tm_multi_cat_sparse_sandwich_ent_into_f64", codes, ncols, drop, n, E.n, D.p(d), D.p(E.vals), D.p(E.meta),
+         D.p(E.bstart), E.n_slots(), E.mk, D.p(packed), D.p(out), int(out.shape[0]), D.p(rpos), D.p(cpos),
+         D.stream_ptr())
+
+
 def multi_cat_sparse_sandwich(cats, d, S: SlabCsc):
     total = sum(int(c[1]) for c in cats)
     if total == 0 or S.m == 0 or S.n == 0:
diff --git a/tabmat_amd/sparse_matrix.py b/tabmat_amd/sparse_matrix.py
--- a/tabmat_amd/sparse_matrix.py
+++ b/tabmat_amd/sparse_matrix.py
@@ -335,6 +335,29 @@
             return res
         return xs.sparse_sandwich(A, d, rows, cols)
 
+    def _sandwich_into(self, d, rows, out, pos) -> bool:
+        from . import categorical_matrix as _cm
+
+        if (self.dtype != np.float64 or d.dtype != torch.float64 or self.shape[0] == 0 or self.shape[1] == 0
+                or self._row_parts() is not None or _cm.DETERMINISTIC):
+            return False
+        A = self._dev()
+        if not (0 < A.data.numel() < 2**31 and self.shape[1] <= 128 * 32):
+            return False
+        if getattr(self, "_direct_pays", None) is None:
+            self._direct_pays = xs.direct_sandwich_pays(A)
+        pp = getattr(self, "_pairs_pay", None)
+        if pp is None:
+            pp = self._pairs_pay = xs.pairs_sandwich_pays(A)
+        if (pp and (rows is None or D.nlen(rows) > 0.3 * self.shape[0])) or self._direct_pays:
+            return False
+        if rows is not None and 0 < D.nlen(rows) <= ROW_LIST_FRACTION * self.shape[0]:
+            return False
+        bl = getattr(self, "_blocks_pay", None)
+        if bl is None:
+            bl = self._blocks_pay = xs.blocks_sandwich_pays(A)
+        return bool(bl) and xs.sparse_sandwich_blocks_into(A, D.masked_d(d, rows, as_set=True), out, pos)
+
     def _ent_det(self):
         ent = self._ent()
         if ent is None:
@@ -389,6 +412,39 @@
         res = self._sandwich_dev(D.to_dev(d), D.idx_dev(normalize_index(rows, self.shape[0])),
                                  D.idx_dev(normalize_index(cols, self.shape[1])))
         return res if on_dev else D.to_host(res)
+
+    def _cross_sandwich_into(self, other, d, rows, out, pos_self, pos_other) -> bool:
+        from .dense_matrix import DenseMatrix
+
+        if (not isinstance(other, DenseMatrix) or self.dtype != np.float64 or other.dtype != np.float64
+                or d.dtype != torch.float64 or self.shape[0] == 0 or self.shape[1] == 0 or other.shape[1] == 0):
+            return False
+        Bd = other._dev_c()
+        A = self._dev()
+        if A.data.numel() == 0:
+            return False
+        if rows is not None and (
+                (0 < D.nlen(rows) <= ROW_LIST_FRACTION_K3 * self.shape[0]
+                 and A.data.numel() < 2**31 and self.shape[1] <= 128 * 32) or not self._values_finite()):
+            return False
+        if A.data.numel() <= SORTED_K3_NNZ_PER_ROW * self.shape[0] and self.shape[1] >= 1024 and xs.ell_supported(Bd):
+            return False
+        if not (Bd.m > 64 and xs.ell_supported(Bd)):
+            return False
+        ent = self._ent()
+        if ent is None:
+            return False
+        xs.csr_dense_sandwich_ent_into(ent, Bd, D.masked_d(d, rows), out, self._ent_pos(ent, pos_self), pos_other)
+        return True
+
+    def _ent_pos(self, ent, pos):
+        key = (pos.data_ptr(), int(pos.numel()), ent.mk, id(ent))
+        hit = self.__dict__.get("_ent_pos_cache")
+        if hit is None or hit[0] != key:
+            kpos = torch.full((ent.mk,), -1, dtype=torch.int64, device=pos.device)
+            kpos[ent.inv] = pos
+            hit = self.__dict__["_ent_pos_cache"] = (key, kpos, pos)
+        return hit[1]
 
     def _cross_sandwich_dev(self, other, d, rows, L_cols, R_cols, colsum_box=None):
         from .categorical_matrix import CategoricalMatrix
diff --git a/tabmat_amd/split_matrix.py b/tabmat_amd/split_matrix.py
--- a/tabmat_amd/split_matrix.py
+++ b/tabmat_amd/split_matrix.py
@@ -28,6 +28,7 @@
 )
 
 
+FINISH_INTO = True
 ROW_LIST_FRACTION_CATSPARSE = 0.04
 DIAG_FROM_PAIRS = True
 CAT_PAIRS_FUSED = os.environ.get("TABMAT_AMD_CAT_PAIRS", "1") != "0"
@@ -419,6 +420,35 @@
             return xsplit.multi_cat_sparse_sandwich(cats, d_eff, mw._slab())
         return None
 
+    def _fused_cats_into(self, mw, cats, cat_ids, d_eff, rows, total, budget, out, gpos, wpos) -> bool:
+        if self.dtype != np.float64 or d_eff.dtype != torch.float64 or total == 0 or mw.shape[1] == 0:
+            return False
+        if isinstance(mw, DenseMatrix):
+            Md = mw._dev_c()
+            if (Md.n == 0 or not xsplit.multi_cat_dense_wide_ok(cats, Md)
+                    or (rows is not None and D.nlen(rows) <= 0.5 * self.shape[0])):
+                return False
+            xsplit.multi_cat_dense_sandwich_into(cats, d_eff, Md, out, gpos, wpos)
+            return True
+        if not isinstance(mw, SparseMatrix) or total * 33 > budget or mw._dev().data.numel() == 0:
+            return False
+        if rows is not None and (
+                (0 < D.nlen(rows) <= ROW_LIST_FRACTION_CATSPARSE * self.shape[0]
+                 and mw._dev().data.numel() < 2**31) or not mw._values_finite()):
+            return False
+        if not (len(cats) <= 8 and (getattr(mw, "_entblk", None) or any(
+                isinstance(mo, DenseMatrix) and mo.shape[1] > 64 and mo.dtype == mw.dtype for mo in self.matrices))):
+            return False
+        ent = mw._ent()
+        if ent is None or ent.n == 0:
+            return False
+        pk_cache = self.__dict__.setdefault("_packed_codes", {})
+        key = tuple(cat_ids)
+        if key not in pk_cache:
+            pk_cache[key] = xsplit.pack_codes(cats)
+        xsplit.multi_cat_sparse_sandwich_ent_into(cats, d_eff, ent, out, gpos, mw._ent_pos(ent, wpos), pk_cache[key])
+        return True
+
     def _parts(self):
         parts = self.__dict__.get("_row_parts", False)
         if parts is False:
@@ -662,15 +692,20 @@
             for w, mw in enumerate(mats):
                 if empty[w] or mw.dtype != self.dtype or d.dtype != D.torch_dtype(self.dtype):
                     continue
-                stacked = self._fused_cats(mw, cats, grp, d_eff, rows, total, budget, d)
-                if stacked is None:
-                    continue
                 whole = cols_host is None and len(grp) > 1
                 if whole:
                     cache = self.__dict__.setdefault("_group_pos", {})
                     gpos = cache.get(tuple(grp))
                     if gpos is None:
                         gpos = cache[tuple(grp)] = torch.cat([pos_d[i] for i in grp])
+                    if FINISH_INTO and colsum is None and self._fused_cats_into(
+                            mw, cats, grp, d_eff, rows, total, budget, out, gpos, pos_d[w]):
+                        done.update((min(i, w), max(i, w)) for i in grp)
+                        continue
+                stacked = self._fused_cats(mw, cats, grp, d_eff, rows, total, budget, d)
+                if stacked is None:
+                    continue
+                if whole:
                     xsplit.scatter_block(stacked.contiguous(), gpos, pos_d[w], out, mirror=True)
                 for ci, i in enumerate(grp):
                     res = stacked[int(offs[ci]):int(offs[ci + 1])]
@@ -758,6 +793,9 @@
                 if cen_i is not None:
                     center.cs_centered.add(i)
                 xsplit.scatter_block(res, pos_d[i], pos_d[i], out)
+            elif (FINISH_INTO and isinstance(mi, SparseMatrix) and colsum is None and sub_d[i] is None
+                  and mi._sandwich_into(d, rows, out, pos_d[i])):
+                pass
             elif isinstance(mi, DenseMatrix) and center is not None and center.get(i) is not None:
                 res = mi._sandwich_dev(d, rows, sub_d[i], center=center.get(i))
                 xsplit.scatter_block(res, pos_d[i], pos_d[i], out)
@@ -771,8 +809,13 @@
                 if empty[j] or (i, j) in done:
                     continue
                 si, di = (i, j) if isinstance(mi, SparseMatrix) else (j, i)
-                if (colsum is not None and colsum[si] is None and isinstance(mats[si], SparseMatrix)
-                        and isinstance(mats[di], DenseMatrix)):
+                want_cs = (colsum is not None and colsum[si] is None and isinstance(mats[si], SparseMatrix)
+                           and isinstance(mats[di], DenseMatrix))
+                if (FINISH_INTO and not want_cs and sub_d[i] is None and sub_d[j] is None
+                        and isinstance(mats[si], SparseMatrix)
+                        and mats[si]._cross_sandwich_into(mats[di], d, rows, out, pos_d[si], pos_d[di])):
+                    continue
+                if want_cs:
                     box = []
                     res = mats[si]._cross_sandwich_dev(mats[di], d, rows, sub_d[si], sub_d[di],
                                                        colsum_box=box)
```

Result: no change. 1020 GB/s (median of 6 runs) (+0.3%).
